# liulisixin/MLI-NeRF

Measured on AMD Instinct MI355X. Metric: rays/sec + PSNR, syn_hotdog 4096 rays x128 samples, 1/2/4/8 MI355X, higher is better.
Workload: dtype fp16; 1 GPU; syn_hotdog_b stage-b train step; rays_per_gpu=4096, samples_per_ray=128, global_rays=4096, parallelism=dp1, pipeline=geometry prefetch on a side stream, gate heads, 2 batch(es) ahead, output_layer_dw=forward partials (pq), tail=fused, reductions=ordered

## Files before the change

### include/mli_hip.h

```cpp
#ifndef MLI_HIP_H
#define MLI_HIP_H

#include <stdint.h>

#ifdef __cplusplus
extern "C" {
#endif

typedef struct ihipStream_t* mli_stream_t;

#define MLI_ABI_VERSION 18
#define MLI_HIDDEN 256
#define MLI_LEVELS 16
#define MLI_LEVEL_FEAT 8
#define MLI_HEAD_K0 304

typedef struct {
  float scale[MLI_LEVELS];
  uint32_t res[MLI_LEVELS];
  uint32_t size[MLI_LEVELS];
  uint32_t offset[MLI_LEVELS];
  uint64_t modmagic[MLI_LEVELS];
} mli_grid_levels;

int mli_abi_version(void);
const char* mli_error_string(int code);

typedef struct {
  const float* intr;
  const float* pose;
  const float* pose_light;
  const int64_t* ray_idx;
  int64_t first_pixel;
  int R, W;
  int bounding;
  float aabb[6];
  float* center;
  float* ray_unit;
  float* ray_norm;
  float* pts_light;
  float* near_;
  float* far_;
  uint8_t* outside;
} mli_rays_args;
int mli_rays(const mli_rays_args* a, mli_stream_t s);

typedef struct {
  const float* x01;
  const uint16_t* table;
  mli_grid_levels levels;
  int n;
  float* out;
} mli_hashgrid_args;
int mli_hashgrid_fwd(const mli_hashgrid_args* a, mli_stream_t s);

#define MLI_SDF_MODE_SDF 0
#define MLI_SDF_MODE_FIELD 1
#define MLI_SDF_MODE_SDF_LISTED 2
typedef struct {
  int mode;
  int R, n_per_ray;
  const float* center;
  const float* ray_unit;
  const float* dists;
  const uint8_t* outside;
  const uint16_t* table;
  mli_grid_levels levels;
  const void* wsdf;
  float eps;
  float grad_den;
  float hess_den;
  float outside_val;
  int with_hessian;
  float* sdf;
  float* grad;
  float* hess;
  uint16_t* h0;
  uint16_t* enc;
  int active_levels;
  const int32_t* inside_list;
  const int32_t* n_inside;
} mli_sdf_args;
int mli_sdf(const mli_sdf_args* a, mli_stream_t s);
int mli_sdf_workspace(const mli_sdf_args* a, int64_t* bytes);

struct mli_inside_list_args_s {
  int R, N;
  int n_pad;
  const uint8_t* outside;
  int32_t* inside_list;
  int32_t* n_inside;
  float outside_val;
  float* sdf;
  float* grad;
  float* hess;
  const float* near_;
  const float* far_;
  float* dists;
};
typedef struct mli_inside_list_args_s mli_inside_list_args;
int mli_inside_list(const mli_inside_list_args* a, mli_stream_t s);

typedef struct {
  const float* near_; const float* far_;
  const float* u;
  int R, Nc;
  float* dists;
} mli_sample_coarse_args;
int mli_sample_coarse(const mli_sample_coarse_args* a, mli_stream_t s);

typedef struct {
  int R;
  const float* dists_a; const float* sdf_a; int Na;
  const float* dists_b; const float* sdf_b; int Nb;
  float* dists_out; float* sdf_out;
  int Nf;
  float inv_s;
  const float* u_fine;
  float* fine_out;
  const int32_t* inside_list;
  const int32_t* n_inside;
} mli_sample_fine_args;
int mli_sample_fine(const mli_sample_fine_args* a, mli_stream_t s);

typedef struct {
  int R, N;
  const float* center; const float* ray_unit; const float* pts_light;
  const float* dists;
  const float* grad;
  const uint16_t* h0;
  const void* wfwd;
  float* y;
  uint16_t* feat_frag;
  uint16_t* xT;
  uint32_t* masks;
  int n_heads;
  const float* weights;
  float* q4;
  const int32_t* tile_list;
  const int32_t* n_live_tiles;
} mli_rgb_fwd_args;
#define MLI_Q4_SCALE 65536.0f
#define MLI_Q4_SEGS(N) ((256 % (N)) == 0 ? 256 / (N) : ((N) % 256 == 0 ? 1 : 256 / (N) + 2))
int mli_rgb_fwd(const mli_rgb_fwd_args* a, mli_stream_t s);
int mli_rgb_fwd_workspace(const mli_rgb_fwd_args* a, int64_t* bytes);

typedef struct {
  int R, N;
  const float* dists; const float* far_; const float* ray_unit; const float* ray_norm;
  const float* sdf; const float* grad; const float* y;
  const float* s_var;
  float anneal;
  int white_bg;
  float* weights;
  float* rgb; float* o_r; float* o_s; float* o_re;
  float* opacity; float* gradient; float* depth;
  float* blend_dist;
} mli_composite_args;
int mli_composite_fwd(const mli_composite_args* a, mli_stream_t s);

typedef struct {
  int R, N;
  const float* weights; const float* y;
  const float* o_r; const float* o_s;
  const float* d_rgb; const float* d_o_r; const float* d_o_s; const float* d_o_re;
  float grad_scale;
  float* dz4;
  float* dray;
} mli_composite_bwd_args;
int mli_composite_bwd(const mli_composite_bwd_args* a, mli_stream_t s);

typedef struct {
  int R, N;
  const float* dz4;
  const void* wbwd;
  const uint32_t* masks;
  uint16_t* dzT;
  uint16_t* dz4T;
  int skip_dz3;
  const int32_t* tile_list;
  const int32_t* n_live_tiles;
} mli_rgb_bwd_args;
int mli_rgb_bwd(const mli_rgb_bwd_args* a, mli_stream_t s);
int mli_rgb_bwd_workspace(const mli_rgb_bwd_args* a, int64_t* bytes);

typedef struct {
  const uint16_t* a_rows;
  const uint16_t* b_rows;
  int M, K;
  float* dw;
  float* db;
  int ldw;
  int a_tiled, b_tiled;
  int a_kst, b_kst;
  const uint16_t* b2_rows;
  int b2_q, b2_kst;
  const float* rb_dz4;
  const uint32_t* rb_mask;
  const void* rb_w4;
  int rb_col, rb_cnt;
  int rb_R, rb_N;
} mli_wgrad_job;
#define MLI_WGRAD_LAYOUT_ROWS 0
#define MLI_WGRAD_LAYOUT_TILED 1
#define MLI_WGRAD_LAYOUT_FRAG_ACC 2
#define MLI_WGRAD_LAYOUT_FRAG_NAT 3
#define MLI_WGRAD_BIG 1
#define MLI_WGRAD_WIDE 2
#define MLI_WGRAD_THIN 4
typedef struct {
  int S;
  int n_jobs;
  const mli_wgrad_job* jobs;
  int classes;
  int deterministic;
  float* workspace;
  const int32_t* tile_rank;
  const int32_t* tile_list;
  const int32_t* wtile_rank;
  const int32_t* wtile_list;
} mli_wgrad_args;
int mli_wgrad(const mli_wgrad_args* a, mli_stream_t s);
int mli_wgrad_workspace(const mli_wgrad_args* a, int64_t* bytes);

typedef struct {
  int R, N, n_heads;
  const float* q4;
  const float* dray;
  float scale;
  float* dw[3];
  float* db[3];
  int k_out[3];
  float* workspace;
  const int32_t* tile_rank;
} mli_dw4_args;
int mli_dw4(const mli_dw4_args* a, mli_stream_t s);
int mli_dw4_workspace(const mli_dw4_args* a, int64_t* bytes);

struct mli_live_rays_args_s {
  int R, N;
  const float* weights;
  float* y;
  int32_t* flags;
  int32_t* tile_list; int32_t* tile_rank; int32_t* n_live_tiles;
};
typedef struct mli_live_rays_args_s mli_live_rays_args;
int mli_live_rays(const mli_live_rays_args* a, mli_stream_t s);

struct mli_live_tiles_args_s {
  mli_composite_args comp;
  float* y;
  int32_t* flags;
  int32_t* tile_list; int32_t* tile_rank; int32_t* n_live_tiles;
  int32_t* wtile_list; int32_t* wtile_rank;
  int32_t* ticket;
  int scan_launch;
};
typedef struct mli_live_tiles_args_s mli_live_tiles_args;
int mli_live_tiles(const mli_live_tiles_args* a, mli_stream_t s);


typedef struct {
  int R, N;
  const float* dists; const float* far_; const float* ray_unit;
  const float* sdf; const float* grad; const float* y;
  const float* s_var;
  float anneal;
  int white_bg;
  const float* d_rgb;
  float grad_scale;
  float* dz4;
  float* d_sdf;
  float* d_grad;
  float* d_inv_s_part;
  float* d_s_var;
} mli_composite_bwd_geo_args;
int mli_composite_bwd_geo(const mli_composite_bwd_geo_args* a, mli_stream_t s);
int mli_composite_bwd_geo_workspace(const mli_composite_bwd_geo_args* a, int64_t* bytes);

typedef struct {
  int R, N;
  const float* dz4;
  const void* wgeo;
  const uint32_t* masks;
  const uint16_t* feat_frag;
  uint16_t* dzT;
  uint16_t* dz4T;
  float* d_nrm;
  uint16_t* dz1T;
  uint16_t* dh0_frag;
} mli_geo_bwd_args;
int mli_geo_bwd(const mli_geo_bwd_args* a, mli_stream_t s);
int mli_geo_bwd_workspace(const mli_geo_bwd_args* a, int64_t* bytes);

typedef struct {
  int R, N;
  const float* center; const float* ray_unit; const float* dists;
  const uint8_t* outside;
  const float* grad; const float* hess;
  const float* d_sdf; const float* d_grad;
  const float* d_nrm;
  const uint16_t* dh0_frag;
  const uint16_t* enc;
  const void* wsdf;
  const void* wsdf_t;
  float eps, grad_den, hess_den;
  float w_eikonal, w_curvature;
  float grad_scale;
  float* d_enc;
  uint16_t* dz0_frag;
  uint16_t* p_frag;
  float* dw_sdf;
  float* db_sdf;
  const float* d_grad_ext;
  const float* d_hess_ext;
  float* partials;
} mli_sdf_bwd_args;
int mli_sdf_bwd(const mli_sdf_bwd_args* a, mli_stream_t s);
int mli_sdf_bwd_workspace(const mli_sdf_bwd_args* a, int64_t* bytes);

typedef struct {
  const float* v0; const float* g0;
  uint8_t* dst;
} mli_pack_sdf_t_args;
#define MLI_SDF_T_PACK_BYTES 65536
int mli_pack_sdf_t(const mli_pack_sdf_t_args* a, mli_stream_t s);

typedef struct {
  int R, N;
  const float* center; const float* ray_unit; const float* dists;
  const float* d_enc;
  mli_grid_levels levels;
  float eps;
  int active_levels;
  float* d_table;
  int deterministic;
  int64_t* workspace;
  int64_t n_params;
} mli_hash_bwd_args;
int mli_hash_bwd(const mli_hash_bwd_args* a, mli_stream_t s);
int mli_hash_bwd_workspace(const mli_hash_bwd_args* a, int64_t* bytes);

typedef struct {
  const uint16_t* src;
  int64_t tile_stride;
  int tiles, k_steps, order;
  uint16_t* dst;
  int64_t ld;
  int64_t col0;
  int row0;
} mli_frag_rows_args;
int mli_frag_rows(const mli_frag_rows_args* a, mli_stream_t s);

typedef struct {
  int R;
  const float* center; const float* ray_unit; const float* pts_light;
  const float* near_; const float* far_;
  const float* blend_dist;
  const float* gradient;
  int camera_ray_type, iters;
  int vis_box;
  float vis_r2; float aabb[6];
  float gamma;
  const uint16_t* table; mli_grid_levels levels; int active_levels; const void* wsdf;
  float* light_unit; float* near_l; float* far_t; uint8_t* inside;
  float* inter_dist; uint8_t* inter_mask; float* inter_pts;
  uint8_t* visibility; float* normal_x_light; float* pseudo_shading;
} mli_light_visibility_args;
int mli_light_visibility(const mli_light_visibility_args* a, mli_stream_t s);
int mli_light_visibility_workspace(const mli_light_visibility_args* a, int64_t* bytes);

typedef struct {
  uint64_t seed;
  int64_t n_pixels;
  int R;
  const float* image;
  const float* ref;
  const float* sha;
  const float* cert;
  int64_t* ray_idx;
  float* image_sampled;
  float* ref_sampled;
  float* sha_sampled;
  float* cert_sampled;
} mli_ray_batch_args;
int mli_ray_batch(const mli_ray_batch_args* a, mli_stream_t s);

typedef struct {
  int R, N;
  const float* rgb; const float* o_r; const float* o_s; const float* o_re;
  const float* gt;
  const float* ref; const float* sha; const float* cert;
  const uint8_t* outside;
  const float* grad; const float* hess;
  float w_render, w_eikonal, w_curvature, w_intrinsic, w_re;
  float range_sha_lo, range_sha_hi, range_vis_lo, range_vis_hi, f_ref, f_sha;
  float f_neg, f_pos, e_pos;
  float* d_rgb; float* d_o_r; float* d_o_s; float* d_o_re;
  float* losses;
  float* scratch;
} mli_loss_args;
int mli_stage_b_loss(const mli_loss_args* a, mli_stream_t s);
int mli_stage_b_loss_workspace(const mli_loss_args* a, int64_t* bytes);

typedef struct {
  mli_composite_args comp;
  mli_loss_args loss;
  float grad_scale;
  float* dz4;
  int defer_finalize;
  float* dray;
} mli_composite_loss_args;
int mli_composite_loss(const mli_composite_loss_args* a, mli_stream_t s);
int mli_composite_loss_finalize(const mli_composite_loss_args* a, mli_stream_t s);
int mli_composite_loss_workspace(const mli_composite_loss_args* a, int64_t* bytes);

typedef struct {
  const float* v; const float* g; const float* bias;
  int n_out, k_ref;
  int transpose;
  int n_tiles, k_steps;
  const int16_t* kmap;
  const uint8_t* kmode;
  int64_t dst_offset;
  int chunk_stride;
  const int16_t* nmap;
} mli_pack_layer;
typedef struct {
  int n_layers;
  const mli_pack_layer* layers;
  uint8_t* dst;
  float* row_scale;
} mli_pack_args;
int mli_pack(const mli_pack_args* a, mli_stream_t s);
int mli_pack_workspace(const mli_pack_args* a, int64_t* bytes);

typedef struct {
  const float* v0; const float* g0; const float* b0;
  const float* w_sdf; const float* b_sdf;
  uint8_t* dst;
} mli_pack_sdf_args;
#define MLI_SDF_PACK_BYTES (65536 + 5 * 1024 + 16)
int mli_pack_sdf(const mli_pack_sdf_args* a, mli_stream_t s);

typedef struct {
  const float* dw; const float* db;
  const float* v; const float* g;
  int n_out, k_ref, k_pack;
  const int16_t* kinv;
  float* grad_v; float* grad_g; float* grad_b;
  const float* extra_db;
  int plain;
} mli_assemble_layer;
typedef struct {
  int n_layers;
  const mli_assemble_layer* layers;
  float inv_scale;
  int zero_dw;
} mli_assemble_args;
int mli_grad_assemble(const mli_assemble_args* a, mli_stream_t s);

typedef struct {
  float* p; float* g; float* m; float* v;
  int64_t n;
  double lr, beta1, beta2, eps, weight_decay;
  int step;
  uint16_t* p16;
  int zero_grad;
} mli_adamw_args;
int mli_adamw(const mli_adamw_args* a, mli_stream_t s);

typedef struct { const float* src; uint16_t* dst; int64_t n; } mli_cast_args;
int mli_cast_f16(const mli_cast_args* a, mli_stream_t s);

const char* mli_source_hash(void);

#ifdef __cplusplus
}
#endif
#endif
```

### mli_nerf_amd/_lib.py

```python
import ctypes as C
import os

HERE = os.path.dirname(os.path.abspath(__file__))
LIB_PATH = os.environ.get("MLI_HIP_LIB") or os.path.join(HERE, "libmli_hip.so")

P = C.c_void_p
I32 = C.c_int
I64 = C.c_int64
F32 = C.c_float
F64 = C.c_double


class GridLevels(C.Structure):
    _fields_ = [("scale", F32 * 16), ("res", C.c_uint32 * 16), ("size", C.c_uint32 * 16),
                ("offset", C.c_uint32 * 16), ("modmagic", C.c_uint64 * 16)]


class RaysArgs(C.Structure):
    _fields_ = [("intr", P), ("pose", P), ("pose_light", P), ("ray_idx", P), ("first_pixel", I64),
                ("R", I32), ("W", I32), ("bounding", I32), ("aabb", F32 * 6),
                ("center", P), ("ray_unit", P), ("ray_norm", P), ("pts_light", P),
                ("near_", P), ("far_", P), ("outside", P)]


class HashgridArgs(C.Structure):
    _fields_ = [("x01", P), ("table", P), ("levels", GridLevels), ("n", I32), ("out", P)]


class SdfArgs(C.Structure):
    _fields_ = [("mode", I32), ("R", I32), ("n_per_ray", I32), ("center", P), ("ray_unit", P),
                ("dists", P), ("outside", P), ("table", P), ("levels", GridLevels), ("wsdf", P),
                ("eps", F32), ("grad_den", F32), ("hess_den", F32), ("outside_val", F32),
                ("with_hessian", I32), ("sdf", P), ("grad", P), ("hess", P), ("h0", P),
                ("enc", P), ("active_levels", I32), ("inside_list", P), ("n_inside", P)]


class InsideListArgs(C.Structure):
    _fields_ = [("R", I32), ("N", I32), ("n_pad", I32), ("outside", P), ("inside_list", P), ("n_inside", P),
                ("outside_val", F32), ("sdf", P), ("grad", P), ("hess", P), ("near_", P), ("far_", P),
                ("dists", P)]


class SampleCoarseArgs(C.Structure):
    _fields_ = [("near_", P), ("far_", P), ("u", P), ("R", I32), ("Nc", I32), ("dists", P)]


class SampleFineArgs(C.Structure):
    _fields_ = [("R", I32), ("dists_a", P), ("sdf_a", P), ("Na", I32), ("dists_b", P), ("sdf_b", P),
                ("Nb", I32), ("dists_out", P), ("sdf_out", P), ("Nf", I32), ("inv_s", F32),
                ("u_fine", P), ("fine_out", P), ("inside_list", P), ("n_inside", P)]


class RgbFwdArgs(C.Structure):
    _fields_ = [("R", I32), ("N", I32), ("center", P), ("ray_unit", P), ("pts_light", P),
                ("dists", P), ("grad", P), ("h0", P), ("wfwd", P), ("y", P), ("feat_frag", P),
                ("xT", P), ("masks", P), ("n_heads", I32), ("weights", P), ("q4", P),
                ("tile_list", P), ("n_live_tiles", P)]


class CompositeArgs(C.Structure):
    _fields_ = [("R", I32), ("N", I32), ("dists", P), ("far_", P), ("ray_unit", P), ("ray_norm", P),
                ("sdf", P), ("grad", P), ("y", P), ("s_var", P), ("anneal", F32), ("white_bg", I32),
                ("weights", P), ("rgb", P), ("o_r", P), ("o_s", P), ("o_re", P), ("opacity", P),
                ("gradient", P), ("depth", P), ("blend_dist", P)]


class CompositeBwdArgs(C.Structure):
    _fields_ = [("R", I32), ("N", I32), ("weights", P), ("y", P), ("o_r", P), ("o_s", P),
                ("d_rgb", P), ("d_o_r", P), ("d_o_s", P), ("d_o_re", P), ("grad_scale", F32),
                ("dz4", P), ("dray", P)]


class RgbBwdArgs(C.Structure):
    _fields_ = [("R", I32), ("N", I32), ("dz4", P), ("wbwd", P), ("masks", P), ("dzT", P),
                ("dz4T", P), ("skip_dz3", I32), ("tile_list", P), ("n_live_tiles", P)]


class WgradJob(C.Structure):
    _fields_ = [("a_rows", P), ("b_rows", P), ("M", I32), ("K", I32), ("dw", P), ("db", P), ("ldw", I32),
                ("a_tiled", I32), ("b_tiled", I32), ("a_kst", I32), ("b_kst", I32), ("b2_rows", P),
                ("b2_q", I32), ("b2_kst", I32), ("rb_dz4", P), ("rb_mask", P), ("rb_w4", P), ("rb_col", I32),
                ("rb_cnt", I32), ("rb_R", I32), ("rb_N", I32)]


ROWS, TILED, FRAG_ACC, FRAG_NAT = 0, 1, 2, 3


def frag_job(a, b, M, K, dw, db, ldw, a_kst, b_kst, order=FRAG_ACC, b_order=None, b2=None, b2_q=0, b2_kst=0):
    return WgradJob(a, b, M, K, dw, db, ldw, order, order if b_order is None else b_order, a_kst, b_kst,
                    b2, b2_q, b2_kst)


class WgradArgs(C.Structure):
    _fields_ = [("S", I32), ("n_jobs", I32), ("jobs", P), ("classes", I32), ("deterministic", I32),
                ("workspace", P), ("tile_rank", P), ("tile_list", P), ("wtile_rank", P), ("wtile_list", P)]


class Dw4Args(C.Structure):
    _fields_ = [("R", I32), ("N", I32), ("n_heads", I32), ("q4", P), ("dray", P), ("scale", F32),
                ("dw", P * 3), ("db", P * 3), ("k_out", I32 * 3), ("workspace", P),
                ("tile_rank", P)]


class LiveRaysArgs(C.Structure):
    _fields_ = [("R", I32), ("N", I32), ("weights", P), ("y", P), ("flags", P), ("tile_list", P),
                ("tile_rank", P), ("n_live_tiles", P)]


class LiveTilesArgs(C.Structure):
    _fields_ = [("comp", CompositeArgs), ("y", P), ("flags", P), ("tile_list", P), ("tile_rank", P),
                ("n_live_tiles", P), ("wtile_list", P), ("wtile_rank", P), ("ticket", P), ("scan_launch", I32)]


Q4_SCALE = 65536.0


class LossArgs(C.Structure):
    _fields_ = [("R", I32), ("N", I32), ("rgb", P), ("o_r", P), ("o_s", P), ("o_re", P), ("gt", P),
                ("ref", P), ("sha", P), ("cert", P), ("outside", P), ("grad", P), ("hess", P),
                ("w_render", F32), ("w_eikonal", F32), ("w_curvature", F32), ("w_intrinsic", F32),
                ("w_re", F32), ("range_sha_lo", F32), ("range_sha_hi", F32), ("range_vis_lo", F32),
                ("range_vis_hi", F32), ("f_ref", F32), ("f_sha", F32), ("f_neg", F32), ("f_pos", F32),
                ("e_pos", F32), ("d_rgb", P), ("d_o_r", P), ("d_o_s", P), ("d_o_re", P), ("losses", P),
                ("scratch", P)]



class CompositeLossArgs(C.Structure):
    _fields_ = [("comp", CompositeArgs), ("loss", LossArgs), ("grad_scale", F32), ("dz4", P),
                ("defer_finalize", I32), ("dray", P)]

class PackLayer(C.Structure):
    _fields_ = [("v", P), ("g", P), ("bias", P), ("n_out", I32), ("k_ref", I32), ("transpose", I32),
                ("n_tiles", I32), ("k_steps", I32), ("kmap", P), ("kmode", P), ("dst_offset", I64),
                ("chunk_stride", I32), ("nmap", P)]


class PackArgs(C.Structure):
    _fields_ = [("n_layers", I32), ("layers", P), ("dst", P), ("row_scale", P)]


class PackSdfArgs(C.Structure):
    _fields_ = [("v0", P), ("g0", P), ("b0", P), ("w_sdf", P), ("b_sdf", P), ("dst", P)]


class AssembleLayer(C.Structure):
    _fields_ = [("dw", P), ("db", P), ("v", P), ("g", P), ("n_out", I32), ("k_ref", I32),
                ("k_pack", I32), ("kinv", P), ("grad_v", P), ("grad_g", P), ("grad_b", P),
                ("extra_db", P), ("plain", I32)]


class AssembleArgs(C.Structure):
    _fields_ = [("n_layers", I32), ("layers", P), ("inv_scale", F32), ("zero_dw", I32)]


class AdamwArgs(C.Structure):
    _fields_ = [("p", P), ("g", P), ("m", P), ("v", P), ("n", I64), ("lr", F64), ("beta1", F64),
                ("beta2", F64), ("eps", F64), ("weight_decay", F64), ("step", I32), ("p16", P),
                ("zero_grad", I32)]


class CastArgs(C.Structure):
    _fields_ = [("src", P), ("dst", P), ("n", I64)]


class CompositeBwdGeoArgs(C.Structure):
    _fields_ = [("R", I32), ("N", I32), ("dists", P), ("far_", P), ("ray_unit", P), ("sdf", P), ("grad", P),
                ("y", P), ("s_var", P), ("anneal", F32), ("white_bg", I32), ("d_rgb", P), ("grad_scale", F32),
                ("dz4", P), ("d_sdf", P), ("d_grad", P), ("d_inv_s_part", P), ("d_s_var", P)]


class GeoBwdArgs(C.Structure):
    _fields_ = [("R", I32), ("N", I32), ("dz4", P), ("wgeo", P), ("masks", P), ("feat_frag", P), ("dzT", P),
                ("dz4T", P), ("d_nrm", P), ("dz1T", P), ("dh0_frag", P)]


class SdfBwdArgs(C.Structure):
    _fields_ = [("R", I32), ("N", I32), ("center", P), ("ray_unit", P), ("dists", P), ("outside", P),
                ("grad", P), ("hess", P), ("d_sdf", P), ("d_grad", P), ("d_nrm", P), ("dh0_frag", P), ("enc", P),
                ("wsdf", P), ("wsdf_t", P), ("eps", F32), ("grad_den", F32), ("hess_den", F32),
                ("w_eikonal", F32), ("w_curvature", F32), ("grad_scale", F32), ("d_enc", P), ("dz0_frag", P),
                ("p_frag", P), ("dw_sdf", P), ("db_sdf", P), ("d_grad_ext", P), ("d_hess_ext", P),
                ("partials", P)]


class PackSdfTArgs(C.Structure):
    _fields_ = [("v0", P), ("g0", P), ("dst", P)]


class HashBwdArgs(C.Structure):
    _fields_ = [("R", I32), ("N", I32), ("center", P), ("ray_unit", P), ("dists", P), ("d_enc", P),
                ("levels", GridLevels), ("eps", F32), ("active_levels", I32), ("d_table", P),
                ("deterministic", I32), ("workspace", P), ("n_params", I64)]


class LightVisibilityArgs(C.Structure):
    _fields_ = [("R", I32), ("center", P), ("ray_unit", P), ("pts_light", P), ("near_", P), ("far_", P),
                ("blend_dist", P), ("gradient", P), ("camera_ray_type", I32), ("iters", I32), ("vis_box", I32),
                ("vis_r2", F32), ("aabb", F32 * 6), ("gamma", F32), ("table", P), ("levels", GridLevels),
                ("active_levels", I32), ("wsdf", P), ("light_unit", P), ("near_l", P), ("far_t", P),
                ("inside", P), ("inter_dist", P), ("inter_mask", P), ("inter_pts", P), ("visibility", P),
                ("normal_x_light", P), ("pseudo_shading", P)]


class RayBatchArgs(C.Structure):
    _fields_ = [("seed", C.c_uint64), ("n_pixels", I64), ("R", I32), ("image", P), ("ref", P), ("sha", P),
                ("cert", P), ("ray_idx", P), ("image_sampled", P), ("ref_sampled", P), ("sha_sampled", P),
                ("cert_sampled", P)]


class FragRowsArgs(C.Structure):
    _fields_ = [("src", P), ("tile_stride", I64), ("tiles", I32), ("k_steps", I32), ("order", I32), ("dst", P),
                ("ld", I64), ("col0", I64), ("row0", I32)]


ABI_VERSION = 18

ENTRY_POINTS = {
    "mli_rays": RaysArgs, "mli_hashgrid_fwd": HashgridArgs, "mli_sdf": SdfArgs,
    "mli_sample_coarse": SampleCoarseArgs, "mli_sample_fine": SampleFineArgs,
    "mli_rgb_fwd": RgbFwdArgs, "mli_composite_fwd": CompositeArgs,
    "mli_composite_bwd": CompositeBwdArgs, "mli_rgb_bwd": RgbBwdArgs,
    "mli_wgrad": WgradArgs, "mli_dw4": Dw4Args, "mli_live_rays": LiveRaysArgs,
    "mli_live_tiles": LiveTilesArgs, "mli_inside_list": InsideListArgs,
    "mli_pack": PackArgs, "mli_pack_sdf": PackSdfArgs, "mli_grad_assemble": AssembleArgs,
    "mli_adamw": AdamwArgs, "mli_cast_f16": CastArgs, "mli_stage_b_loss": LossArgs,
    "mli_composite_bwd_geo": CompositeBwdGeoArgs, "mli_geo_bwd": GeoBwdArgs, "mli_sdf_bwd": SdfBwdArgs,
    "mli_pack_sdf_t": PackSdfTArgs, "mli_hash_bwd": HashBwdArgs, "mli_frag_rows": FragRowsArgs,
    "mli_light_visibility": LightVisibilityArgs, "mli_ray_batch": RayBatchArgs,
    "mli_composite_loss": CompositeLossArgs, "mli_composite_loss_finalize": CompositeLossArgs,
}

WORKSPACE = {
    "mli_sdf": 1, "mli_rgb_fwd": 6, "mli_rgb_bwd": 2, "mli_wgrad": 1, "mli_composite_bwd_geo": 4,
    "mli_geo_bwd": 6, "mli_sdf_bwd": 4, "mli_hash_bwd": 1, "mli_light_visibility": 5, "mli_stage_b_loss": 5,
    "mli_pack": 1, "mli_dw4": 1, "mli_composite_loss": 2,
}


class McArgs(C.Structure):
    _fields_ = [("sdf", P), ("nx", I32), ("ny", I32), ("nz", I32), ("sx", I64), ("sy", I64), ("sz", I64),
                ("iso", F32), ("origin", F32 * 3), ("spacing", F32), ("off_x", I32), ("off_y", I32),
                ("off_z", I32), ("gx", I32), ("gy", I32), ("gz", I32), ("chunk_base", P), ("counts", P),
                ("edge_slot", P), ("max_vertices", I32), ("max_triangles", I32), ("verts", P),
                ("vert_keys", P), ("faces", P), ("face_keys", P)]


MESH_ABI_VERSION = 1
MC_CHUNK = 256

MESH_ENTRY_POINTS = {"mli_mc_count": McArgs, "mli_mc_emit": McArgs}
MESH_WORKSPACE = {"mli_mc_count": 2, "mli_mc_emit": 1}

class LabelMorphArgs(C.Structure):
    _fields_ = [("B", I32), ("H", I32), ("W", I32), ("erode_radius", I32), ("edge_step", I32),
                ("visibility", P), ("eroded", P), ("certainty", P), ("tile_max", P), ("normal_x_light", P),
                ("inter_mask", P), ("inv_gamma", F32), ("shading", P), ("shading_gamma", P)]


class LabelKmeansArgs(C.Structure):
    _fields_ = [("L", I32), ("K", I32), ("n_pixels", I32), ("max_iter", I32), ("image", P), ("labels", P),
                ("centers", P), ("passes", P)]


class LabelBestRefArgs(C.Structure):
    _fields_ = [("L", I32), ("K", I32), ("n_pixels", I32), ("threshold", F32), ("threshold_wrt_max", F32),
                ("image", P), ("shading", P), ("shading_gamma", P), ("labels", P), ("average_ref", P),
                ("keep_count", P), ("any_mask", P)]


class LabelFillArgs(C.Structure):
    _fields_ = [("H", I32), ("W", I32), ("K", I32), ("n_holes", I32), ("n_donors", I32), ("slices", I32),
                ("normal", P), ("centers", P), ("hole_idx", P), ("donor_idx", P), ("ref", P), ("hole_feat", P),
                ("donor_feat", P), ("partial", P)]


LABELS_ABI_VERSION = 1
LABELS_MAX_RADIUS = 15
LABELS_MAX_K = 4
LABELS_TILE = (32, 8)
LABELS_DONOR_TILE = 256
LABELS_MAX_SLICES = 64

LABELS_ENTRY_POINTS = {"mli_label_morph": LabelMorphArgs, "mli_label_kmeans": LabelKmeansArgs,
                       "mli_label_best_ref": LabelBestRefArgs, "mli_label_fill": LabelFillArgs}
LABELS_WORKSPACE = {"mli_label_morph": 1, "mli_label_fill": 3}

class MeshCcArgs(C.Structure):
    _fields_ = [("faces", P), ("n_faces", I64), ("verts", P), ("n_verts", C.c_int32), ("label", P), ("changed", P),
                ("max_rounds", C.c_int32), ("round", C.c_int32), ("comp_faces", P), ("comp_area", P), ("max_q", P),
                ("inv_unit", F64)]


MESH_CC_ABI_VERSION = 1
MESH_CC_MAX_ROUNDS = 4096

MESH_CC_ENTRY_POINTS = {"mli_cc_init": MeshCcArgs, "mli_cc_round": MeshCcArgs, "mli_cc_stats": MeshCcArgs}
MESH_CC_WORKSPACE = {"mli_cc_init": 4}

class MetricsArgs(C.Structure):
    _fields_ = [("B", I32), ("C", I32), ("H", I32), ("W", I32), ("quantize", I32), ("mask_pred", I32),
                ("gamma_target", I32), ("inv_gamma", F64), ("pred_f32", P), ("pred_u8", P), ("target_f32", P),
                ("target_u8", P), ("alpha_f32", P), ("alpha_u8", P), ("mse", P), ("psnr", P), ("ssim", P),
                ("ssim_channels", P), ("prep_pred", P), ("prep_target", P), ("partial", P)]


METRICS_ABI_VERSION = 1
METRICS_MAX_SIDE = 16384
METRICS_MAX_IMAGES = 16383
METRICS_MAX_CHANNELS = 4
METRICS_WINDOW = 7
METRICS_TILE = (32, 8)

METRICS_ENTRY_POINTS = {"mli_image_metrics": MetricsArgs}
METRICS_WORKSPACE = {"mli_image_metrics": 1}

class LightPointsArgs(C.Structure):
    _fields_ = [("L", I32), ("R", I32), ("pose_lights", P), ("pts_light", P)]


class CameraHitArgs(C.Structure):
    _fields_ = [("R", I32), ("center", P), ("ray_unit", P), ("near_", P), ("far_", P), ("blend_dist", P),
                ("camera_ray_type", I32), ("iters", I32), ("table", P), ("levels", GridLevels),
                ("active_levels", I32), ("wsdf", P), ("inter_dist", P), ("inter_mask", P), ("inter_pts", P)]


class LightShadowsArgs(C.Structure):
    _fields_ = [("L", I32), ("R", I32), ("pts_light", P), ("inter_pts", P), ("gradient", P), ("vis_box", I32),
                ("vis_r2", F32), ("aabb", F32 * 6), ("gamma", F32), ("iters", I32), ("table", P),
                ("levels", GridLevels), ("active_levels", I32), ("wsdf", P), ("visibility", P),
                ("normal_x_light", P), ("pseudo_shading", P)]


RELIGHT_ABI_VERSION = 1

RELIGHT_ENTRY_POINTS = {"mli_light_points": LightPointsArgs, "mli_camera_hit": CameraHitArgs,
                        "mli_light_shadows": LightShadowsArgs}
RELIGHT_WORKSPACE = {}

_lib = None


def lib():
    global _lib
    if _lib is None:
        if not os.path.exists(LIB_PATH):
            raise ImportError("libmli_hip.so is not built (%s); run mli_nerf_amd.build.build() -- "
                              "there is no CPU fallback for the hot path" % LIB_PATH)
        _lib = C.CDLL(LIB_PATH)
        for name, st in list(ENTRY_POINTS.items()) + list(MESH_ENTRY_POINTS.items()) + list(
                LABELS_ENTRY_POINTS.items()) + list(MESH_CC_ENTRY_POINTS.items()) + list(
                METRICS_ENTRY_POINTS.items()) + list(RELIGHT_ENTRY_POINTS.items()):
            fn = getattr(_lib, name)
            fn.argtypes = [C.POINTER(st), P]
            fn.restype = I32
        for table, points in ((WORKSPACE, ENTRY_POINTS), (MESH_WORKSPACE, MESH_ENTRY_POINTS),
                              (LABELS_WORKSPACE, LABELS_ENTRY_POINTS), (MESH_CC_WORKSPACE, MESH_CC_ENTRY_POINTS),
                              (METRICS_WORKSPACE, METRICS_ENTRY_POINTS)):
            for name in table:
                fn = getattr(_lib, name + "_workspace")
                fn.argtypes = [C.POINTER(points[name]), C.POINTER(I64)]
                fn.restype = I32
        _lib.mli_mesh_abi_version.restype = I32
        _lib.mli_labels_abi_version.restype = I32
        _lib.mli_mesh_cc_abi_version.restype = I32
        _lib.mli_metrics_abi_version.restype = I32
        _lib.mli_relight_abi_version.restype = I32
        _lib.mli_abi_version.restype = I32
        _lib.mli_error_string.restype = C.c_char_p
        _lib.mli_error_string.argtypes = [I32]
        _lib.mli_source_hash.restype = C.c_char_p
        if (_lib.mli_abi_version() != ABI_VERSION or _lib.mli_mesh_abi_version() != MESH_ABI_VERSION
                or _lib.mli_labels_abi_version() != LABELS_ABI_VERSION
                or _lib.mli_mesh_cc_abi_version() != MESH_CC_ABI_VERSION
                or _lib.mli_metrics_abi_version() != METRICS_ABI_VERSION
                or _lib.mli_relight_abi_version() != RELIGHT_ABI_VERSION):
            raise ImportError("libmli_hip.so ABI mismatch")
        from . import build as _build
        if all(os.path.exists(d) for d in _build._deps()):
            want, got = _build.source_hash(), _lib.mli_source_hash().decode()
            in_tree = os.path.realpath(LIB_PATH) == os.path.realpath(_build.OUT)
            if got != want and in_tree:
                raise ImportError("libmli_hip.so is stale (built from sources %s, the tree is %s); rebuild with "
                                  "mli_nerf_amd.build.build()" % (got, want))
            if got != want:
                import warnings
                warnings.warn("MLI_HIP_LIB=%s was built from sources %s, not this tree's %s (experiment build)"
                              % (LIB_PATH, got, want))
    return _lib


def _variant(name, args):
    if name == "mli_sdf":
        return ":field" if args.mode == 1 else ":sdf"
    if name == "mli_wgrad":
        return {1: ":big", 2: ":wide", 4: ":thin"}.get(args.classes, "")
    return ""


def workspace(name, args):
    out = (I64 * 8)()
    rc = getattr(lib(), name + "_workspace")(C.byref(args), out)
    if rc != 0:
        raise RuntimeError("%s_workspace failed: %s (%d)" % (name, lib().mli_error_string(rc).decode(), rc))
    return [int(out[i]) for i in range(WORKSPACE.get(name) or MESH_WORKSPACE.get(name) or LABELS_WORKSPACE.get(name)
                                         or MESH_CC_WORKSPACE.get(name) or METRICS_WORKSPACE[name])]


def ptr(t):
    return None if t is None else t.data_ptr()


PROFILE = None
PROFILE_NAMES = None
# ... 17 lines not shown
```

### mli_nerf_amd/csrc/mlp_bwd.hip

```cpp
#include "mlp_core.h"

namespace {

template <bool NODZ3>
__global__ __launch_bounds__(GBwd::THREADS) void rgb_bwd_kernel(mli_rgb_bwd_args a) {
  extern __shared__ __attribute__((aligned(16))) uint8_t lds[];
  if (a.n_live_tiles && (int)(blockIdx.x * GBwd::NW) >= *a.n_live_tiles) return;
  if (__builtin_amdgcn_readfirstlane(threadIdx.x >> 6) >= GBwd::NW / 2) rgb_bwd_body<GBwd, STORE, NODZ3>(a, lds);
  else rgb_bwd_body<GBwd, DMA, NODZ3>(a, lds);
}


}

extern "C" int mli_rgb_bwd(const mli_rgb_bwd_args* a, mli_stream_t s) {
  const int S = a->R * a->N;
  if (S % 256 != 0) return (int)hipErrorInvalidValue;
  if ((a->tile_list != nullptr) != (a->n_live_tiles != nullptr)) return (int)hipErrorInvalidValue;
  if (a->tile_list && (a->N <= 0 || 256 % a->N != 0 || a->N % 32 != 0)) return (int)hipErrorInvalidValue;
  if (a->skip_dz3)
    hipLaunchKernelGGL(rgb_bwd_kernel<true>, dim3(S / GBwd::SAMPLES), dim3(GBwd::THREADS), GBwd::LDS_BWD,
                       (hipStream_t)s, *a);
  else
    hipLaunchKernelGGL(rgb_bwd_kernel<false>, dim3(S / GBwd::SAMPLES), dim3(GBwd::THREADS), GBwd::LDS_BWD,
                       (hipStream_t)s, *a);
  MLI_LAUNCH_CHECK();
}

extern "C" int mli_rgb_bwd_workspace(const mli_rgb_bwd_args* a, int64_t* bytes) {
  const int64_t S = (int64_t)a->R * a->N;
  if (S <= 0 || S % 256 != 0) return (int)hipErrorInvalidValue;
  bytes[0] = 3 * 4 * 256 * S * 2;
  bytes[1] = 3 * S * 16 * 2;
  return 0;
}
```

### mli_nerf_amd/csrc/mlp_core.h

```cpp
#pragma once
#include "common.h"

#include <type_traits>

namespace {

constexpr int CH(int ks) { return ks * 1024 + 128; }
constexpr int FRAG_KS = 512;
constexpr int FRAG_TILE = 16 * FRAG_KS;
constexpr int X0_KS = MLI_HEAD_K0 / 16;
constexpr int X0_TILE = X0_KS * FRAG_KS;
constexpr int Q4_SLOT = 257 * 16;
constexpr int DIST = 2;
#ifndef MLI_HEADS_PAIR
#define MLI_HEADS_PAIR 1
#endif
constexpr bool HEADS_PAIR = MLI_HEADS_PAIR;
constexpr int NSLOT = HEADS_PAIR ? 4 : DIST + 1;

enum Role { ALL = 0, DMA = 1, STORE = 2 };

template <int NW_, int MAXP, bool SPLIT_, int PF_ = 0>
struct Geo {
  static constexpr int NW = NW_;
// ... 12 lines not shown
  static constexpr int QP_OFF = RING;
  static constexpr int PQ_WAVE = 2048 + 256;
  static constexpr int PQW_OFF = QP_OFF + (HEADS_PAIR ? 0 : NW * Q4_SLOT);
  static constexpr int LDS_FWD_PQ = PQW_OFF + NW * PQ_WAVE;
  static constexpr int FEAT_KS = 6;
  static_assert(FEAT_KS % 2 == 0, "whole 32-feature tiles of feat in LDS");
  static constexpr int LDS_FWD_PQF = LDS_FWD_PQ + NW * FEAT_KS * 1024;
  static constexpr int FEAT_KS_EVAL = 8;
  static_assert(FEAT_KS_EVAL % 2 == 0, "whole 32-feature tiles of feat in LDS");
  static constexpr int LDS_FWD_F = LDS_FWD + NW * FEAT_KS_EVAL * 1024;
  template <int ROLE> static constexpr int ring_ops() { return ROLE == STORE ? 0 : RND; }
};

struct Ring {
  const uint8_t* src;
  const uint8_t* last;
  int next, n, cur;
};

template <class G, int ROLE>
MLI_FI void ring_pieces(const uint8_t* s, int nb, uint8_t* slot) {
  const int wave = threadIdx.x >> 6, lane = threadIdx.x & 63;
  if (ROLE != STORE) {
#pragma unroll
    for (int u = 0; u < G::RND; ++u)
      glds16(s + min((u * G::ND + wave) * 1024 + lane * 16, nb - 16), slot + (u * G::ND + wave) * 1024);
  }
}

template <class G, int ROLE, class Bytes>
MLI_FI void ring_issue(Ring& r, uint8_t* lds, Bytes&& bytes) {
  const bool real = r.next < r.n;
  const int nb = bytes(real ? r.next : r.n - 1);
  ring_pieces<G, ROLE>(real ? r.src : r.last, nb, lds + (r.next % NSLOT) * G::SLOT);
  if (real) r.src += nb;
  r.next++;
}

struct ChunkAt {
  const uint8_t* image;
  int head_bytes;
  int first;
  MLI_FI const uint8_t* src(int c) const { return image + (size_t)(c >> 3) * head_bytes + first + (c & 7) * CH(16); }
  MLI_FI int operator()(int) const { return CH(16); }
};

template <class G, int ROLE>
MLI_FI void ring_issue(Ring& r, uint8_t* lds, ChunkAt& at) {
  ring_pieces<G, ROLE>(at.src(min(r.next, r.n - 1)), CH(16), lds + (r.next % NSLOT) * G::SLOT);
  r.next++;
}

template <class Bytes>
MLI_FI void ring_start(Ring& r, const void* base, int n, Bytes&& bytes) {
  r.src = reinterpret_cast<const uint8_t*>(base);
  size_t total = 0;
  for (int c = 0; c + 1 < n; ++c) total += bytes(c);
  r.last = r.src + total;
  r.next = 0;
  r.n = n;
  r.cur = 0;
}

MLI_FI void frag_store2(uint16_t* tile_img, int t, half8 f0, half8 f1, int lane) {
  half8* d = reinterpret_cast<half8*>(tile_img) + (2 * t) * 64 + lane;
  gstore_nt(d, f0);
  gstore_nt(d + 64, f1);
}

MLI_FI float relu1(float x) {
  return __builtin_bit_cast(float, max(__builtin_bit_cast(int, x), 0));
}
MLI_FI int f32_bits(float x) { return __builtin_bit_cast(int, x); }
MLI_FI uint32_t relu_bits16(const f32x16& r) {
  uint32_t b = 0;
#pragma unroll
  for (int i = 15; i >= 0; --i)
    asm("v_cmp_lt_i32 vcc, 0, %1\n\tv_addc_co_u32 %0, vcc, %0, %0, vcc" : "+v"(b) : "v"(f32_bits(r[i])) : "vcc");
  return b;
}
template <int KS, int PF = 0>
MLI_FI f32x16 chunk_mma(const uint8_t* chunk, const half8* X, int lane) {
  const int h = lane >> 5;
  f32x16 acc;
  const f32x4* bias = reinterpret_cast<const f32x4*>(chunk + KS * 1024 + h * 64);
#pragma unroll
  for (int u = 0; u < 4; ++u) {
    const f32x4 b = bias[u];
    acc[4 * u] = b[0]; acc[4 * u + 1] = b[1]; acc[4 * u + 2] = b[2]; acc[4 * u + 3] = b[3];
  }
  const half8* w = reinterpret_cast<const half8*>(chunk) + lane;
  if constexpr (PF == 0) {
#pragma unroll
    for (int q = 0; q < KS; ++q) acc = mfma32(w[q * 64], X[q], acc);
  } else {
    constexpr int D = PF < KS ? PF : KS;
    half8 wr[D];
#pragma unroll
    for (int q = 0; q < D; ++q) wr[q] = w[q * 64];
#pragma unroll
    for (int q = 0; q < KS; ++q) {
      acc = mfma32(wr[q % D], X[q], acc);
      if (q + D < KS) wr[q % D] = w[(q + D) * 64];
    }
#pragma unroll
    for (int q = 0; q < D; ++q) __builtin_amdgcn_sched_group_barrier(0x100, 1, 0);
#pragma unroll
    for (int q = 0; q < KS; ++q) {
      __builtin_amdgcn_sched_group_barrier(0x008, 1, 0);
      if (q + D < KS) __builtin_amdgcn_sched_group_barrier(0x100, 1, 0);
    }
  }
  return acc;
}

template <class G, int ROLE, int KS, int NT, int EPI, bool MASKED, class Bytes, class Pre, class Epi>
MLI_FI void run_layer(Ring& rg, uint8_t* lds, const half8* X, int lane, Bytes&& bytes, Pre&& pre, Epi&& epi) {
  auto stores = [](int t) MLI_LAMBDA_FI { return EPI + ((MASKED && t == NT - 1) ? 1 : 0); };
#pragma unroll
  for (int t = 0; t < NT; ++t) {
    pre.issue(t);
    ring_issue<G, ROLE>(rg, lds, bytes);
    const f32x16 acc = chunk_mma<KS, G::PF>(lds + (rg.cur % NSLOT) * G::SLOT, X, lane);
    epi(t, acc);
    if (ROLE != STORE) {
      int n = (DIST - 1) * G::template ring_ops<ROLE>() + pre.count(t) + stores(t);
#pragma unroll
      for (int b = 1; b < DIST; ++b) {
        if (t - b < 0) break;
        n += stores(t - b) + (b < DIST - 1 ? pre.count(t - b) : 0);
      }
      vm_wait(n);
    }
    block_sync();
    rg.cur++;
  }
}

struct NoPre {
  MLI_FI int count(int) const { return 0; }
  MLI_FI void issue(int) const {}
};

template <class G, int ROLE, int KS, int NT, int EPI, int MASKN, int PREVN, bool DEFER, int LASTN = 0, class Bytes,
          class Pre, class Prev, class Epi>
MLI_FI void run_layer_d(Ring& rg, uint8_t* lds, const half8* X, int lane, Bytes&& bytes, Pre&& pre, Prev&& prev,
                        Epi&& epi, f32x16& pacc) {
  static_assert(ROLE != ALL, "split wave roles only");
  auto stores = [](int t) MLI_LAMBDA_FI {
    if (t < 0) return LASTN;
    const int pv = t == 0 ? PREVN : 0;
    if (DEFER) return pv + (t >= 1 ? EPI : 0);
    return pv + EPI + (t == NT - 1 ? MASKN : 0);
  };
#pragma unroll
  for (int t = 0; t < NT; ++t) {
    pre.issue(t);
    ring_issue<G, ROLE>(rg, lds, bytes);
    if (t == 0) prev(pacc);
    const f32x16 acc = chunk_mma<KS, G::PF>(lds + (rg.cur % NSLOT) * G::SLOT, X, lane);
    if (DEFER) {
      if (t > 0) epi(t - 1, pacc);
      pacc = acc;
    } else {
      epi(t, acc);
    }
    if (ROLE != STORE) vm_wait((DIST - 1) * G::template ring_ops<ROLE>() + pre.count(t) + stores(t) + stores(t - 1));
    block_sync();
    rg.cur++;
  }
}

template <class G, int ROLE, int KS, int NT, int EPI, int MASKN, int PREVN, bool DEFER, int NEXTN, class Bytes,
          class Pre, class Prev, class Epi>
MLI_FI void run_layer_p(Ring& rg, uint8_t* lds, const half8* X, int lane, Bytes&& bytes, Pre&& pre, Prev&& prev,
                        Epi&& epi, f32x16& pacc) {
  static_assert(ROLE != ALL, "split wave roles only");
  static_assert(NSLOT == 4, "two segments of two chunks in the ring");
  auto stores = [](int t) MLI_LAMBDA_FI {
    const int pv = t == 0 ? PREVN : 0;
    if (DEFER) return pv + (t >= 1 ? EPI : 0);
    return pv + EPI + (t == NT - 1 ? MASKN : 0);
  };
#pragma unroll
  for (int s = 0; s < NT; s += 2) {
    const int n_this = NT - s < 2 ? NT - s : 2;
    const int n_next = s + 2 < NT ? (NT - s - 2 < 2 ? NT - s - 2 : 2) : NEXTN;
#pragma unroll
    for (int t = s; t < s + n_this; ++t) pre.issue(t);
#pragma unroll
    for (int k = 0; k < n_next; ++k) ring_issue<G, ROLE>(rg, lds, bytes);
    int n = 0;
#pragma unroll
    for (int t = s; t < s + n_this; ++t) {
      if (t == 0) prev(pacc);
      const f32x16 acc = chunk_mma<KS, G::PF>(lds + (rg.cur % NSLOT) * G::SLOT, X, lane);
      if (DEFER) {
        if (t > 0) epi(t - 1, pacc);
        pacc = acc;
      } else {
        epi(t, acc);
      }
      n += stores(t);
      rg.cur++;
    }
    if (ROLE != STORE) vm_wait(n);
    block_sync();
  }
}

template <class G, int ROLE, int KS, int NT, int EPI, int MASKN, int PREVN, bool DEFER, int LASTN, int NEXTN,
          class Bytes, class Pre, class Prev, class Epi>
MLI_FI void heads_layer(Ring& rg, uint8_t* lds, const half8* X, int lane, Bytes&& bytes, Pre&& pre, Prev&& prev,
                        Epi&& epi, f32x16& pacc) {
  if constexpr (HEADS_PAIR)
    run_layer_p<G, ROLE, KS, NT, EPI, MASKN, PREVN, DEFER, NEXTN>(rg, lds, X, lane, bytes, pre, prev, epi, pacc);
  else
    run_layer_d<G, ROLE, KS, NT, EPI, MASKN, PREVN, DEFER, LASTN>(rg, lds, X, lane, bytes, pre, prev, epi, pacc);
}

constexpr int PROLOGUE_CHUNKS = HEADS_PAIR ? 2 : DIST;

constexpr bool HEADS_DEFER = true;

constexpr float Q4_SCALE = MLI_Q4_SCALE;

template <class G, int ROLE>
MLI_FI void q4_tile(const mli_rgb_fwd_args& a, uint8_t* lds, const half8 (&X)[19], const float (&gq)[3], int hd,
                   int lane, const Ring& rg) {
  const int wave = threadIdx.x >> 6, c = lane & 31, h = lane >> 5;
  uint8_t* xr = lds + G::PQW_OFF + wave * G::PQ_WAVE;
  uint8_t* gr = xr + 2048;
  auto q4_park = [&](int w) MLI_LAMBDA_FI {
    if constexpr (HEADS_PAIR) {
      static_assert(4 * Q4_SLOT <= G::SLOT && G::NW == 8, "Q park in two ring slots");
      const int slot = (rg.cur - (w < 4 ? 2 : 1)) % NSLOT;
      return lds + slot * G::SLOT + (w & 3) * Q4_SLOT;
    } else {
      return lds + G::QP_OFF + w * Q4_SLOT;
    }
  };
  uint8_t* qs = q4_park(wave);
  if (h == 0) {
#pragma unroll
    for (int i = 0; i < 4; ++i)
      ds_write_u16(lds_addr(gr + i * 64 + c * 2), __builtin_bit_cast(uint16_t, (f16)(i < 3 ? gq[i] : 0.f)));
  }
  asm volatile("" ::: "memory");
  half8 gf[2];
  {
    const int gi = min(c, 3);
#pragma unroll
    for (int ks = 0; ks < 2; ++ks) gf[ks] = *reinterpret_cast<const half8*>(gr + gi * 64 + (16 * ks + 8 * h) * 2);
  }
  const int g16 = (lane >> 4) & 3, q = (lane & 15) >> 2, p = lane & 3;
  const int chunk = 4 * (g16 & 1) + p;
#pragma unroll
  for (int b = 0; b < 8; ++b) {
#pragma unroll
    for (int u = 0; u < 2; ++u) {
      const u32x4 w = __builtin_bit_cast(u32x4, X[2 * b + u]);
#pragma unroll
      for (int jj = 0; jj < 2; ++jj) {
        const int ch = (4 * u + 2 * jj + h) ^ ((c >> 1) & 7);
        ds_write_u64(lds_addr(xr + c * 64 + ch * 8), u32x2{w[2 * jj], w[2 * jj + 1]});
      }
    }
    f32x16 acc;
#pragma unroll
    for (int e = 0; e < 16; ++e) acc[e] = 0.f;
    half8 xf[2];
#pragma unroll
    for (int ks = 0; ks < 2; ++ks) {
      const int s0 = 16 * ks + 8 * h + q, s1 = s0 + 4;
      const half4 lo = ds_tr16_at<0>(lds_addr(xr + s0 * 64 + (chunk ^ ((s0 >> 1) & 7)) * 8));
      const half4 hi = ds_tr16_at<0>(lds_addr(xr + s1 * 64 + (chunk ^ ((s1 >> 1) & 7)) * 8));
      xf[ks] = half8{lo[0], lo[1], lo[2], lo[3], hi[0], hi[1], hi[2], hi[3]};
    }
    lgkm_wait<0>();
    tie(xf[0]);
    tie(xf[1]);
#pragma unroll
    for (int ks = 0; ks < 2; ++ks) acc = mfma32(gf[ks], xf[ks], acc);
    if (h == 0) ds_write_f128(lds_addr(qs + (32 * b + c) * 16), f32x4{acc[0], acc[1], acc[2], acc[3]});
  }
  float sb[3];
#pragma unroll
  for (int i = 0; i < 3; ++i) {
    float v = gq[i];
#pragma unroll
    for (int o = 32; o > 0; o >>= 1) v += __shfl_xor(v, o);
    sb[i] = v;
  }
  if (lane == 0) ds_write_f128(lds_addr(qs + 256 * 16), f32x4{sb[0], sb[1], sb[2], 0.f});
  block_sync();
  if (ROLE != DMA) {
    const int N = a.N, t0 = blockIdx.x * G::NW;
    const int r_first = t0 * 32 / N;
    const int nseg = ((t0 + G::NW) * 32 - 1) / N - r_first + 1;
    const int segs = MLI_Q4_SEGS(N);
    const int nthr = ROLE == STORE ? G::THREADS / 2 : G::THREADS;
    const int tid = ROLE == STORE ? threadIdx.x - G::THREADS / 2 : threadIdx.x;
    f32x4* qb = reinterpret_cast<f32x4*>(a.q4);
    for (int it = tid; it < nseg * 257; it += nthr) {
      const int seg = it / 257, row = it - seg * 257;
      size_t item = (size_t)blockIdx.x * segs + seg;
      if (a.tile_list) item = (size_t)(a.tile_list[t0 + seg * (N / 32)] * 32 / N);
      f32x4* qo = qb + item * a.n_heads * 257;
      f32x4 v = {0.f, 0.f, 0.f, 0.f};
#pragma unroll
      for (int w = 0; w < G::NW; ++w)
        if ((t0 + w) * 32 / N - r_first == seg) v += *reinterpret_cast<const f32x4*>(q4_park(w) + row * 16);
      gstore_nt(qo + (size_t)hd * 257 + row, v);
    }
  }
  block_sync();
}

MLI_FI int fwd_bytes(int c) { return (c >= 8 && (c - 8) % 33 < 8) ? CH(19) : CH(16); }

template <class G, bool TRAIN, bool PQ, int ROLE>
MLI_FI void rgb_fwd_body(const mli_rgb_fwd_args& a, uint8_t* lds) {
  const int lane = threadIdx.x & 63, wave = threadIdx.x >> 6;
  const int c = lane & 31, h = lane >> 5;
  const int S = a.R * a.N;
  const int tile = blockIdx.x * G::NW + wave;
  const int tile_o = (PQ && a.tile_list) ? __builtin_amdgcn_readfirstlane(a.tile_list[tile]) : tile;
  const int m = tile_o * 32 + c;
  const int r = m / a.N, k = m - r * a.N;
  const size_t slot = (size_t)k * a.R + r;
  auto bytes = [](int cc) MLI_LAMBDA_FI { return fwd_bytes(cc); };
  constexpr int XL = PQ ? 3 : 4;
  constexpr int FKS = PQ ? G::FEAT_KS : (!TRAIN ? G::FEAT_KS_EVAL : 0);
  constexpr int FOFF = PQ ? G::LDS_FWD_PQ : G::LDS_FWD;
  const float wgt = PQ ? a.weights[slot] : 0.f;

  Ring rg;
  ring_start(rg, a.wfwd, 8 + a.n_heads * 33, bytes);

  half8 A[16], B[19];
  {
    const half8* src = reinterpret_cast<const half8*>(a.h0 + (size_t)tile_o * FRAG_TILE) + lane;
#pragma unroll
    for (int q = 0; q < 16; ++q) B[q] = gload16(src + q * 64);
  }
  half8 xe[3];
  {
    const float d = a.dists[slot];
    const float* cr = a.center + 3 * r;
    const float* vr = a.ray_unit + 3 * r;
    float p[3], nrm[3], g[3];
#pragma unroll
    for (int i = 0; i < 3; ++i) {
      p[i] = __fadd_rn(cr[i], __fmul_rn(vr[i], d));
      g[i] = a.grad[3 * slot + i];
    }
    const float gn = fmaxf(sqrtf((g[0] * g[0] + g[1] * g[1]) + g[2] * g[2]), 1e-12f);
#pragma unroll
    for (int i = 0; i < 3; ++i) nrm[i] = g[i] / gn;
    float shl[16], shv[16];
    sh16(a.pts_light[3 * r], a.pts_light[3 * r + 1], a.pts_light[3 * r + 2], shl);
    sh16(vr[0], vr[1], vr[2], shv);
    const float e16[8] = {p[0], p[1], p[2], nrm[0], nrm[1], nrm[2], 0.f, 0.f};
    const uint32_t hm = opaque_v(h) ? ~0u : 0u;
#pragma unroll
    for (int j = 0; j < 8; ++j) {
      const float v16 = sel_mask(hm, 0.f, e16[j]);
      const float v17 = sel_mask(hm, shl[8 + j], shl[j]);
      const float v18 = sel_mask(hm, shv[8 + j], shv[j]);
      B[16][j] = (f16)v16;
      B[17][j] = (f16)v17;
      B[18][j] = (f16)v18;
      if (TRAIN) {
        const int lo = j < 4 ? j : 4 + j, hi = j < 4 ? 4 + j : 8 + j;
        xe[0][j] = (f16)sel_mask(hm, hi < 8 ? e16[hi & 7] : 0.f, lo < 8 ? e16[lo & 7] : 0.f);
        xe[1][j] = (f16)sel_mask(hm, shl[hi], shl[lo]);
        xe[2][j] = (f16)sel_mask(hm, shv[hi], shv[lo]);
      }
    }
  }
  uint16_t* ftile = a.feat_frag + (size_t)tile * X0_TILE;
#pragma unroll
  for (int d = 0; d < PROLOGUE_CHUNKS; ++d) ring_issue<G, ROLE>(rg, lds, bytes);
  if (TRAIN) {
    half8* xd = reinterpret_cast<half8*>(ftile + 16 * FRAG_KS) + lane;
#pragma unroll
    for (int i = 0; i < 3; ++i) gstore_nt(xd + i * 64, xe[i]);
  }
  vm_wait((HEADS_PAIR || ROLE == STORE ? 0 : (DIST - 1) * G::template ring_ops<ROLE>()) + (TRAIN ? 3 : 0));
#pragma unroll
  for (int q = 0; q < 16; ++q) tie(B[q]);
  block_sync();

  f32x16 pacc;
  auto none = [](f32x16&) MLI_LAMBDA_FI {};
  auto feat_epi = [&](int t, const f32x16& acc) MLI_LAMBDA_FI {
    f32x16 v;
#pragma unroll
    for (int i = 0; i < 16; i += 2) {
      const f32x2 sp = softplus100x2((f32x2){acc[i], acc[i + 1]});
      v[i] = sp.x;
      v[i + 1] = sp.y;
    }
    A[2 * t] = acc_to_frag(v, 0);
    A[2 * t + 1] = acc_to_frag(v, 1);
    half8* dst = reinterpret_cast<half8*>(ftile) + (2 * t) * 64 + lane;
    gstore(dst, A[2 * t]);
    gstore(dst + 64, A[2 * t + 1]);
    if (2 * t + 1 < FKS) {
      half8* fl = reinterpret_cast<half8*>(lds + FOFF + wave * FKS * 1024) + (2 * t) * 64 + lane;
      fl[0] = A[2 * t];
      fl[64] = A[2 * t + 1];
    }
  };
  heads_layer<G, ROLE, 16, 8, 2, 0, 0, HEADS_DEFER, TRAIN ? 3 : 0, 2>(rg, lds, B, lane, bytes, NoPre{}, none, feat_epi,
                                                                      pacc);
  if (HEADS_DEFER) feat_epi(7, pacc);

  for (int hd = 0; hd < a.n_heads; ++hd) {
    const int S = opaque_s(a.R * a.N);
    if (hd == 0) {
#pragma unroll
      for (int q = 0; q < 16; ++q) B[q] = A[q];
    } else {
      const half8* src = reinterpret_cast<const half8*>(ftile) + opaque_v(lane);
      const half8* fl = reinterpret_cast<const half8*>(lds + FOFF + wave * (FKS > 0 ? FKS : 1) * 1024) + lane;
#pragma unroll
      for (int q = 0; q < 16; ++q) B[q] = q < FKS ? fl[q * 64] : gload16(src + q * 64);
    }
    auto l0_wait = [&](f32x16&) MLI_LAMBDA_FI {
      if (hd > 0) {
        vm_wait((HEADS_PAIR ? 2 : 1) * G::template ring_ops<ROLE>());
#pragma unroll
        for (int q = FKS; q < 16; ++q) tie(B[q]);
      }
    };
    uint32_t mbits[4];
    auto relu_epi = [&](half8* out, int layer, bool stg) MLI_LAMBDA_FI {
      return [&, out, layer, stg](int t, const f32x16& acc) MLI_LAMBDA_FI {
        f32x16 v;
#pragma unroll
        for (int i = 0; i < 16; ++i) v[i] = relu1(acc[i]);
        out[2 * t] = acc_to_frag(v, 0);
        out[2 * t + 1] = acc_to_frag(v, 1);
        if (TRAIN) {
          const uint32_t bits = relu_bits16(v);
          if (t & 1) mbits[t >> 1] |= bits << 16; else mbits[t >> 1] = bits;
          if (stg) frag_store2(a.xT + ((size_t)(hd * XL + layer) * (S / 32) + tile) * FRAG_TILE, t, out[2 * t],
                               out[2 * t + 1], lane);
          if (t == 7) {
            u32x4* mp = reinterpret_cast<u32x4*>(a.masks) +
                        ((size_t)(hd * 4 + layer) * (S / 32) + tile) * 64 + lane;
            gstore_nt(mp, u32x4{mbits[0], mbits[1], mbits[2], mbits[3]});
          }
        }
      };
    };
    auto e0 = relu_epi(A, 0, true);
    auto e1 = relu_epi(B, 1, true);
    auto e2 = relu_epi(A, 2, true);
    auto e3 = relu_epi(B, 3, !PQ);
    auto fin = [&](auto& e) MLI_LAMBDA_FI {
      return [&](f32x16& p) MLI_LAMBDA_FI {
        if (HEADS_DEFER) e(7, p);
      };
    };
    constexpr int MN = TRAIN ? 1 : 0, PN = TRAIN && HEADS_DEFER ? 1 : 0;
    constexpr int X = TRAIN ? 2 : 0, X3 = PQ ? 0 : X;
    constexpr int LN = HEADS_DEFER ? X : X + MN;
    heads_layer<G, ROLE, 19, 8, X, MN, 0, HEADS_DEFER, 0, 2>(rg, lds, B, lane, bytes, NoPre{}, l0_wait, e0, pacc);
    heads_layer<G, ROLE, 16, 8, X, MN, PN + X, HEADS_DEFER, LN, 2>(rg, lds, A, lane, bytes, NoPre{}, fin(e0), e1, pacc);
    heads_layer<G, ROLE, 16, 8, X, MN, PN + X, HEADS_DEFER, LN, 2>(rg, lds, B, lane, bytes, NoPre{}, fin(e1), e2, pacc);
    heads_layer<G, ROLE, 16, 8, X3, MN, PN + X, HEADS_DEFER, LN, 1>(rg, lds, A, lane, bytes, NoPre{}, fin(e2), e3,
                                                                    pacc);
    const int no = hd == 2 ? 1 : 3;
    const int off = hd * 3;
    float gq[3] = {0.f, 0.f, 0.f};
    heads_layer<G, ROLE, 16, 1, 0, 0, PN + X3, false, HEADS_DEFER ? X3 : X3 + MN, 2>(rg, lds, B, lane, bytes, NoPre{},
                                                                                fin(e3),
                                          [&](int, const f32x16& acc) MLI_LAMBDA_FI {
      if (h == 0) {
#pragma unroll
        for (int i = 0; i < 3; ++i)
          if (i < no) {
            const float y = sigmoidf_acc(acc[i]);
            gstore_f32(a.y + 8 * slot + off + i, y);
            if (PQ) gq[i] = Q4_SCALE * wgt * (y * (1.0f - y));
          }
      }
    }, pacc);
    if (PQ) q4_tile<G, ROLE>(a, lds, B, gq, hd, lane, rg);
  }
  vm_wait(0);
}

#ifndef MLI_HEADS_PF
#define MLI_HEADS_PF 4
#endif
constexpr int HEADS_PF = MLI_HEADS_PF;
typedef Geo<8, 20, true, HEADS_PF> GFwd;
typedef Geo<8, 20, true, HEADS_PF> GFwdT;
typedef Geo<8, 17, true, HEADS_PF> GBwd;

template <bool TRAIN, bool PQ>
__global__ __launch_bounds__(GFwd::THREADS) void rgb_fwd_kernel(mli_rgb_fwd_args a) {
  extern __shared__ __attribute__((aligned(16))) uint8_t lds[];
  typedef typename std::conditional<TRAIN, GFwdT, GFwd>::type G;
  if (PQ && a.n_live_tiles && (int)(blockIdx.x * G::NW) >= *a.n_live_tiles) return;
  if (__builtin_amdgcn_readfirstlane(threadIdx.x >> 6) >= G::NW / 2) rgb_fwd_body<G, TRAIN, PQ, STORE>(a, lds);
  else rgb_fwd_body<G, TRAIN, PQ, DMA>(a, lds);
}

MLI_FI int bwd_bytes(int c) { return (c % 32) < 8 ? CH(1) : CH(16); }
constexpr int BWD_CHUNKS = 3 * 32;

template <class G, int ROLE, bool NODZ3 = false>
MLI_FI void rgb_bwd_body(const mli_rgb_bwd_args& a, uint8_t* lds) {
  const int lane = threadIdx.x & 63, wave = threadIdx.x >> 6;
  const int c = lane & 31, h = lane >> 5;
  const int S = a.R * a.N;
  const int tiles = S / 32;
  const int tile = blockIdx.x * G::NW + wave;
  const int tile_o = a.tile_list ? __builtin_amdgcn_readfirstlane(a.tile_list[tile]) : tile;
  const int m = tile_o * 32 + c;
  const int r = m / a.N, k = m - r * a.N;
  const size_t slot = (size_t)k * a.R + r;
  auto bytes = [](int cc) MLI_LAMBDA_FI { return bwd_bytes(cc); };
  constexpr int MASK_OPS = ROLE == DMA ? 2 : ROLE == ALL ? 1 : 0;
  auto mask_dma = [&](int L) MLI_LAMBDA_FI {
    const int Lc = min(L, 11);
    const int hd = Lc >> 2, ml = 3 - (Lc & 3);
    const uint8_t* src = reinterpret_cast<const uint8_t*>(a.masks) +
                         (((size_t)(hd * 4 + ml) * tiles + (size_t)blockIdx.x * G::NW) * 64) * 16;
#pragma unroll
    for (int u = 0; u < MASK_OPS; ++u)
      glds16(src + u * (G::MASKB / 2) + threadIdx.x * 16,
             lds + G::MASK_OFF + (L & 1) * G::MASKB + u * (G::MASKB / 2) + wave * 1024);
  };

  f32x4 dzv0, dzv1;
  {
    const f32x4* p = reinterpret_cast<const f32x4*>(a.dz4 + 8 * slot);
    dzv0 = p[0];
    dzv1 = p[1];
  }
  Ring rg;
  ring_start(rg, a.wbwd, BWD_CHUNKS, bytes);
  mask_dma(0);
#pragma unroll
  for (int d = 0; d < PROLOGUE_CHUNKS; ++d) ring_issue<G, ROLE>(rg, lds, bytes);
  if (ROLE != STORE) vm_wait(HEADS_PAIR ? 0 : (DIST - 1) * G::template ring_ops<ROLE>());
  block_sync();

  half8 A[16], B[16];
  for (int hd = 0; hd < 3; ++hd) {
    const int S = opaque_s(a.R * a.N);
    const int no = hd == 2 ? 1 : 3;
    half8 z4;
    {
      const float d0 = hd == 0 ? dzv0[0] : hd == 1 ? dzv0[3] : dzv1[2];
      const float d1 = hd == 0 ? dzv0[1] : dzv1[0];
      const float d2 = hd == 0 ? dzv0[2] : dzv1[1];
#pragma unroll
      for (int j = 0; j < 8; ++j) z4[j] = (f16)0.f;
      if (h == 0) {
        z4[0] = (f16)d0;
        if (no > 1) {
          z4[1] = (f16)d1;
          z4[2] = (f16)d2;
        }
      }
      if (a.dz4T)
        gstore_nt(reinterpret_cast<half8*>(a.dz4T + ((size_t)hd * (S / 32) + tile) * FRAG_KS) + lane, z4);
    }
    struct MaskPre {
      decltype(mask_dma)& dma;
      int next_layer;
      MLI_FI int count(int t) const { return t == 8 - DIST ? MASK_OPS : 0; }
      MLI_FI void issue(int t) const {
        if (t == 8 - DIST) dma(next_layer);
      }
    };
    auto pre = [&](int li) MLI_LAMBDA_FI { return MaskPre{mask_dma, hd * 4 + li + 1}; };
    auto mask_epi = [&](half8* out, int layer , int li, auto stc ) MLI_LAMBDA_FI {
      return [&, out, layer, li, stc](int t, const f32x16& acc) MLI_LAMBDA_FI {
        const u32x4 mv =
            *reinterpret_cast<const u32x4*>(lds + G::MASK_OFF + (li & 1) * G::MASKB + wave * 1024 + lane * 16);
        const int wi = t >> 1;
        const uint32_t word = wi == 0 ? mv[0] : wi == 1 ? mv[1] : wi == 2 ? mv[2] : mv[3];
        f32x16 v;
#pragma unroll
        for (int i = 0; i < 16; ++i) v[i] = mask_bit(acc[i], word, (t & 1) * 16 + i);
        out[2 * t] = acc_to_frag(v, 0);
        out[2 * t + 1] = acc_to_frag(v, 1);
        if (decltype(stc)::value)
          frag_store2(a.dzT + ((size_t)(hd * 4 + layer) * (S / 32) + tile) * FRAG_TILE, t, out[2 * t],
                      out[2 * t + 1], lane);
      };
    };
    const std::true_type store{};
    auto e3 = mask_epi(A, 3, 0, std::integral_constant<bool, !NODZ3>{});
    auto e2 = mask_epi(B, 2, 1, store);
    auto e1 = mask_epi(A, 1, 2, store);
    auto e0 = mask_epi(B, 0, 3, store);
    auto none = [](f32x16&) MLI_LAMBDA_FI {};
    auto fin = [&](auto& e) MLI_LAMBDA_FI {
      return [&](f32x16& p) MLI_LAMBDA_FI {
        if (HEADS_DEFER) e(7, p);
      };
    };
    f32x16 pacc;
    constexpr int X = 2, LN = X, X3 = NODZ3 ? 0 : X;
    heads_layer<G, ROLE, 1, 8, X3, 0, 0, HEADS_DEFER, 0, 2>(rg, lds, &z4, lane, bytes, pre(0), none, e3, pacc);
    heads_layer<G, ROLE, 16, 8, X, 0, X3, HEADS_DEFER, X3, 2>(rg, lds, A, lane, bytes, pre(1), fin(e3), e2, pacc);
    heads_layer<G, ROLE, 16, 8, X, 0, X, HEADS_DEFER, LN, 2>(rg, lds, B, lane, bytes, pre(2), fin(e2), e1, pacc);
    heads_layer<G, ROLE, 16, 8, X, 0, X, HEADS_DEFER, LN, 2>(rg, lds, A, lane, bytes, pre(3), fin(e1), e0, pacc);
    if (HEADS_DEFER) e0(7, pacc);
  }
  vm_wait(0);
}

}

__attribute__((visibility("hidden"))) int mli_launch_rgb_fwd_pq(const mli_rgb_fwd_args* a, hipStream_t s);
__attribute__((visibility("hidden"))) int mli_launch_rgb_fwd_train(const mli_rgb_fwd_args* a, hipStream_t s);
```

### mli_nerf_amd/csrc/mlp_fwd.hip

```cpp
#include "mlp_core.h"

extern "C" int mli_rgb_fwd(const mli_rgb_fwd_args* a, mli_stream_t s) {
  const int S = a->R * a->N;
  if (S % 256 != 0) return (int)hipErrorInvalidValue;
  const bool train = a->xT != nullptr;
  if (a->feat_frag == nullptr || (train && a->masks == nullptr)) return (int)hipErrorInvalidValue;
  if (a->n_heads != 1 && a->n_heads != 3) return (int)hipErrorInvalidValue;
  const bool pq = a->weights != nullptr;
  if (pq && (!train || a->q4 == nullptr || a->N % 32 != 0)) return (int)hipErrorInvalidValue;
  if (!pq && a->q4 != nullptr) return (int)hipErrorInvalidValue;
  if ((a->tile_list != nullptr) != (a->n_live_tiles != nullptr)) return (int)hipErrorInvalidValue;
  if (a->tile_list && (!pq || 256 % a->N != 0)) return (int)hipErrorInvalidValue;
  const dim3 grid(S / GFwd::SAMPLES), block(GFwd::THREADS);
  if (pq) return mli_launch_rgb_fwd_pq(a, (hipStream_t)s);
  if (train) return mli_launch_rgb_fwd_train(a, (hipStream_t)s);
  static_assert(GFwd::LDS_FWD_F <= 163840, "LDS per workgroup");
  hipLaunchKernelGGL((rgb_fwd_kernel<false, false>), grid, block, GFwd::LDS_FWD_F, (hipStream_t)s, *a);
  MLI_LAUNCH_CHECK();
}

extern "C" int mli_rgb_fwd_workspace(const mli_rgb_fwd_args* a, int64_t* bytes) {
  const int64_t S = (int64_t)a->R * a->N;
  if (S <= 0 || S % 256 != 0 || (a->n_heads != 1 && a->n_heads != 3)) return (int)hipErrorInvalidValue;
  const bool pq = a->weights != nullptr;
  if (pq && a->N % 32 != 0) return (int)hipErrorInvalidValue;
  bytes[0] = S * 8 * 4;
  bytes[1] = (int64_t)MLI_HEAD_K0 * S * 2;
  bytes[2] = 0;
  bytes[3] = (int64_t)a->n_heads * (pq ? 3 : 4) * 256 * S * 2;
  bytes[4] = (int64_t)a->n_heads * 4 * (S / 32) * 64 * 16;
  bytes[5] = pq ? (S / 256) * MLI_Q4_SEGS(a->N) * a->n_heads * 257 * 4 * 4 : 0;
  return 0;
}
```

### mli_nerf_amd/csrc/rays.hip

```cpp
#include "common.h"
#include "loss.h"
#include "mli_relight.h"

namespace {

MLI_FI float light_pos(const float* Q, int i) {
  return -((Q[4 * 0 + i] * Q[3] + Q[4 * 1 + i] * Q[7]) + Q[4 * 2 + i] * Q[11]);
}

__global__ __launch_bounds__(256) void rays_kernel(mli_rays_args a) {
  const int r = blockIdx.x * blockDim.x + threadIdx.x;
  if (r >= a.R) return;
  const int64_t pix = a.ray_idx ? a.ray_idx[r] : a.first_pixel + r;
  const float py = (float)(pix / a.W) + 0.5f;
  const float px = (float)(pix % a.W) + 0.5f;
  float K[9], T[12], TL[3];
  {
    const float* M = a.intr;
    const float c00 = M[4] * M[8] - M[5] * M[7], c01 = M[5] * M[6] - M[3] * M[8], c02 = M[3] * M[7] - M[4] * M[6];
    const float det = (M[0] * c00 + M[1] * c01) + M[2] * c02;
    const float id = 1.0f / det;
    K[0] = c00 * id; K[1] = (M[2] * M[7] - M[1] * M[8]) * id; K[2] = (M[1] * M[5] - M[2] * M[4]) * id;
    K[3] = c01 * id; K[4] = (M[0] * M[8] - M[2] * M[6]) * id; K[5] = (M[2] * M[3] - M[0] * M[5]) * id;
    K[6] = c02 * id; K[7] = (M[1] * M[6] - M[0] * M[7]) * id; K[8] = (M[0] * M[4] - M[1] * M[3]) * id;
// ... 610 lines not shown
  return (L << lb) | Rr;
}

__global__ __launch_bounds__(256) void ray_batch_kernel(mli_ray_batch_args a) {
  const int r = blockIdx.x * blockDim.x + threadIdx.x;
  if (r >= a.R) return;
  int bits = 1;
  while ((1ll << bits) < a.n_pixels) ++bits;
  uint64_t x = (uint64_t)r;
  do {
    x = feistel(x, bits, a.seed);
  } while (x >= (uint64_t)a.n_pixels);
  const int64_t p = (int64_t)x, n = a.n_pixels;
  a.ray_idx[r] = p;
  if (a.image)
    for (int c = 0; c < 3; ++c) a.image_sampled[3 * r + c] = a.image[c * n + p];
  if (a.ref)
    for (int c = 0; c < 3; ++c) a.ref_sampled[3 * r + c] = a.ref[c * n + p];
  if (a.sha) a.sha_sampled[r] = a.sha[p];
  if (a.cert) a.cert_sampled[r] = a.cert[p];
}

}

extern "C" int mli_rays(const mli_rays_args* a, mli_stream_t s) {
  if (a->R <= 0) return 0;
  hipLaunchKernelGGL(rays_kernel, dim3((a->R + 255) / 256), dim3(256), 0, (hipStream_t)s, *a);
  MLI_LAUNCH_CHECK();
}

extern "C" int mli_light_points(const mli_light_points_args* a, mli_stream_t s) {
  if (a->L <= 0 || a->R <= 0) return 0;
  if (!a->pose_lights || !a->pts_light) return (int)hipErrorInvalidValue;
  if ((int64_t)a->L * a->R > INT32_MAX) return (int)hipErrorInvalidValue;
  const int64_t n = (int64_t)a->L * a->R * 3;
  hipLaunchKernelGGL(light_points_kernel, dim3((unsigned)((n + 255) / 256)), dim3(256), 0, (hipStream_t)s, *a);
  MLI_LAUNCH_CHECK();
}

extern "C" int mli_sample_coarse(const mli_sample_coarse_args* a, mli_stream_t s) {
  const int n = a->R * a->Nc;
  if (n <= 0) return 0;
  hipLaunchKernelGGL(sample_coarse_kernel, dim3((n + 255) / 256), dim3(256), 0, (hipStream_t)s, *a);
  MLI_LAUNCH_CHECK();
}

extern "C" int mli_sample_fine(const mli_sample_fine_args* a, mli_stream_t s) {
  if (a->R <= 0) return 0;
  if (a->Nf > FBMAX || a->Nb > FBMAX || a->Na < 1 || a->Na + a->Nb > FMAX) return (int)hipErrorInvalidValue;
  if (a->Nf > 0 && a->sdf_out == nullptr) return (int)hipErrorInvalidValue;
  if ((a->inside_list == nullptr) != (a->n_inside == nullptr)) return (int)hipErrorInvalidValue;
  FineArgs fa;
  fa.a = *a;
  for (int j = 0; j < 64; ++j) fa.u[j] = (j < a->Nf && a->u_fine) ? a->u_fine[j] : 2.0f;
  hipLaunchKernelGGL(sample_fine_kernel, dim3((a->R + FW - 1) / FW), dim3(FW * 64), 0, (hipStream_t)s, fa);
  MLI_LAUNCH_CHECK();
}

extern "C" int mli_composite_fwd(const mli_composite_args* a, mli_stream_t s) {
  if (a->R <= 0) return 0;
  if (a->N > 256) return (int)hipErrorInvalidValue;
  if (a->N <= 32 * CE)
    hipLaunchKernelGGL(composite_fwd_kernel<32>, dim3((a->R + 2 * CW - 1) / (2 * CW)), dim3(CW * 64), 0,
                       (hipStream_t)s, *a);
  else
    hipLaunchKernelGGL(composite_fwd_kernel<64>, dim3((a->R + CW - 1) / CW), dim3(CW * 64), 0, (hipStream_t)s, *a);
  MLI_LAUNCH_CHECK();
}

extern "C" int mli_composite_bwd(const mli_composite_bwd_args* a, mli_stream_t s) {
  if (a->R <= 0) return 0;
  const size_t S = (size_t)a->R * a->N;
  hipLaunchKernelGGL(composite_bwd_kernel, dim3((unsigned)((S + 255) / 256)), dim3(256), 0, (hipStream_t)s, *a);
  MLI_LAUNCH_CHECK();
}

extern "C" int mli_composite_bwd_geo(const mli_composite_bwd_geo_args* a, mli_stream_t s) {
  if (a->R <= 0) return 0;
  if (a->N > 256) return (int)hipErrorInvalidValue;
  if (a->d_inv_s_part == nullptr) return (int)hipErrorInvalidValue;
  hipLaunchKernelGGL(composite_bwd_geo_kernel, dim3((a->R + CW - 1) / CW), dim3(CW * 64), 0, (hipStream_t)s, *a);
  hipLaunchKernelGGL(svar_grad_kernel, dim3(1), dim3(256), 0, (hipStream_t)s, *a);
  MLI_LAUNCH_CHECK();
}

extern "C" int mli_composite_bwd_geo_workspace(const mli_composite_bwd_geo_args* a, int64_t* bytes) {
  if (a->R <= 0 || a->N <= 0) return (int)hipErrorInvalidValue;
  const int64_t S = (int64_t)a->R * a->N;
  bytes[0] = S * 8 * 4;
  bytes[1] = S * 4;
  bytes[2] = S * 3 * 4;
  bytes[3] = (int64_t)a->R * 4;
  return 0;
}

extern "C" int mli_ray_batch(const mli_ray_batch_args* a, mli_stream_t s) {
  if (a->R <= 0) return 0;
  if (a->n_pixels < a->R || a->n_pixels > (1ll << 40) || !a->ray_idx) return (int)hipErrorInvalidValue;
  hipLaunchKernelGGL(ray_batch_kernel, dim3((a->R + 255) / 256), dim3(256), 0, (hipStream_t)s, *a);
  MLI_LAUNCH_CHECK();
}

struct CLGeo {
  int rpb, nb;
};
static CLGeo cl_geo(int R, int N) {
  const int rpb = N <= 32 * CE ? 2 * CW : CW;
  return CLGeo{rpb, (R + rpb - 1) / rpb};
}
static bool cl_valid(const mli_composite_loss_args* a) {
  const mli_composite_args& c = a->comp;
  const mli_loss_args& l = a->loss;
  if (c.R <= 0 || c.N <= 0 || c.N > 256 || l.R != c.R || l.N != c.N) return false;
  if (!c.weights || !c.rgb || !c.o_r || !c.o_s || !c.o_re || !a->dz4 || !l.scratch || !l.losses || !l.gt ||
      !l.outside || !c.y)
    return false;
  return !(l.w_intrinsic != 0.f && (l.sha == nullptr || l.cert == nullptr || l.ref == nullptr));
}

extern "C" int mli_composite_loss(const mli_composite_loss_args* a, mli_stream_t s) {
  if (!cl_valid(a)) return (int)hipErrorInvalidValue;
  const CLGeo g = cl_geo(a->comp.R, a->comp.N);
  if (g.rpb == 2 * CW)
    hipLaunchKernelGGL(composite_loss_kernel<32>, dim3(g.nb), dim3(CW * 64), 0, (hipStream_t)s, *a);
  else
    hipLaunchKernelGGL(composite_loss_kernel<64>, dim3(g.nb), dim3(CW * 64), 0, (hipStream_t)s, *a);
  if (!a->defer_finalize)
    hipLaunchKernelGGL(composite_loss_finalize, dim3(1), dim3(256), 0, (hipStream_t)s, a->loss, g.nb);
  MLI_LAUNCH_CHECK();
}

extern "C" int mli_composite_loss_finalize(const mli_composite_loss_args* a, mli_stream_t s) {
  if (!cl_valid(a)) return (int)hipErrorInvalidValue;
  hipLaunchKernelGGL(composite_loss_finalize, dim3(1), dim3(256), 0, (hipStream_t)s, a->loss,
                     cl_geo(a->comp.R, a->comp.N).nb);
  MLI_LAUNCH_CHECK();
}

extern "C" int mli_composite_loss_workspace(const mli_composite_loss_args* a, int64_t* bytes) {
  const int R = a->comp.R;
  if (R <= 0 || a->comp.N <= 0) return (int)hipErrorInvalidValue;
  bytes[0] = (int64_t)mli_loss::ACC_N * cl_geo(R, a->comp.N).nb * 4;
  bytes[1] = (int64_t)R * a->comp.N * 8 * 4;
  return 0;
}

namespace {

constexpr int LR_RAYS = 64, LR_SCAN = 1024;

__global__ __launch_bounds__(4 * LR_RAYS) void live_flags_kernel(mli_live_rays_args a) {
  __shared__ int any[4][LR_RAYS];
  const int rl = threadIdx.x % LR_RAYS, j = threadIdx.x / LR_RAYS;
  const int r = blockIdx.x * LR_RAYS + rl;
  int live = 0;
  if (r < a.R)
    for (int k = j; k < a.N; k += 4)
      live |= (__builtin_bit_cast(uint32_t, a.weights[(size_t)k * a.R + r]) & 0x7fffffffu) != 0;
  any[j][rl] = live;
  __syncthreads();
  live = any[0][rl] | any[1][rl] | any[2][rl] | any[3][rl];
  if (r >= a.R) return;
  if (j == 0) a.flags[r] = live;
  if (!live && a.y != nullptr) {
    const f32x4 z = {0.f, 0.f, 0.f, 0.f};
    for (int k = j; k < a.N; k += 4) {
      f32x4* row = reinterpret_cast<f32x4*>(a.y + ((size_t)k * a.R + r) * 8);
      row[0] = z;
      row[1] = z;
    }
  }
}

template <bool TILES, class Flag, class Emit>
MLI_FI void compact_scan(int n, Flag flag, Emit emit, int& kept, int& bits) {
  __shared__ int sums[1 + TILES][LR_SCAN];
  const int t = threadIdx.x;
  const int per = (n + LR_SCAN - 1) / LR_SCAN;
  const int r0 = min(t * per, n), r1 = min(r0 + per, n);
  int cnt = 0, wcnt = 0;
  for (int r = r0; r < r1; ++r) {
    const uint32_t f = flag(r);
    cnt += f != 0;
    if (TILES) wcnt += __popc(f);
  }
  sums[0][t] = cnt;
  if (TILES) sums[TILES][t] = wcnt;
  __syncthreads();
  for (int o = 1; o < LR_SCAN; o <<= 1) {
    const int v = t >= o ? sums[0][t - o] : 0, wv = TILES && t >= o ? sums[TILES][t - o] : 0;
    __syncthreads();
    sums[0][t] += v;
    if (TILES) sums[TILES][t] += wv;
    __syncthreads();
  }
  kept = sums[0][LR_SCAN - 1];
  bits = TILES ? sums[TILES][LR_SCAN - 1] : 0;
  int before = sums[0][t] - cnt;
  int wbefore = TILES ? sums[TILES][t] - wcnt : 0;
  for (int r = r0; r < r1; ++r) {
    const uint32_t f = flag(r);
    emit(r, f, f != 0 ? before : kept + (r - before), before, wbefore);
    before += f != 0;
    if (TILES) wbefore += __popc(f);
  }
}

__global__ __launch_bounds__(LR_SCAN) void live_scan_kernel(mli_live_rays_args a) {
  const int T = a.N / 32, G = 256 / a.N;
  int L, none;
  compact_scan<false>(
      a.R, [&](int r) MLI_LAMBDA_FI { return (uint32_t)a.flags[r]; },
      [&](int r, uint32_t live, int pos, int before, int) MLI_LAMBDA_FI {
        for (int i = 0; i < T; ++i) {
          a.tile_list[pos * T + i] = r * T + i;
          a.tile_rank[r * T + i] = before * T + (live ? i : 0);
        }
      },
      L, none);
  if (threadIdx.x == 0) {
    a.tile_rank[a.R * T] = L * T;
    a.n_live_tiles[0] = (L + G - 1) / G * G * T;
  }
}

}

extern "C" int mli_live_rays(const mli_live_rays_args* a, mli_stream_t s) {
  if (a->R <= 0 || a->N <= 0 || a->N % 32 != 0 || 256 % a->N != 0 || a->R % (256 / a->N) != 0)
    return (int)hipErrorInvalidValue;
  if (!a->weights || !a->flags || !a->tile_list || !a->tile_rank || !a->n_live_tiles) return (int)hipErrorInvalidValue;
  hipLaunchKernelGGL(live_flags_kernel, dim3((a->R + LR_RAYS - 1) / LR_RAYS), dim3(4 * LR_RAYS), 0, (hipStream_t)s, *a);
  hipLaunchKernelGGL(live_scan_kernel, dim3(1), dim3(LR_SCAN), 0, (hipStream_t)s, *a);
  MLI_LAUNCH_CHECK();
}

namespace {

__global__ __launch_bounds__(LR_SCAN) void inside_list_kernel(mli_inside_list_args a, int fill_blocks) {
  const int t = threadIdx.x;
  if ((int)blockIdx.x < fill_blocks) {
    const size_t i = (size_t)blockIdx.x * LR_SCAN + t;
    if (i >= (size_t)a.R * a.N) return;
    const int r = (int)(i % a.R);
    if (!a.outside[r]) return;
    if (a.dists != nullptr) {
      const float near = a.near_[r], far = a.far_[r];
      const float d = near + (((float)(i / a.R) + 0.5f) / (float)a.N) * (far - near);
      a.dists[i] = fminf(fmaxf(d, near), far);
    }
    if (a.sdf == nullptr) return;
    a.sdf[i] = a.outside_val;
    a.grad[3 * i] = 0.0f;
    a.grad[3 * i + 1] = 0.0f;
    a.grad[3 * i + 2] = 0.0f;
    if (a.hess != nullptr) {
      a.hess[3 * i] = 0.0f;
      a.hess[3 * i + 1] = 0.0f;
      a.hess[3 * i + 2] = 0.0f;
    }
    return;
  }
  int n_in, none;
  compact_scan<false>(
      a.R, [&](int r) MLI_LAMBDA_FI { return (uint32_t)(a.outside[r] == 0); },
      [&](int r, uint32_t, int pos, int, int) MLI_LAMBDA_FI { a.inside_list[pos] = r; }, n_in, none);
  if (t == 0) a.n_inside[0] = min(n_in + a.n_pad, a.R);
}

}

extern "C" int mli_inside_list(const mli_inside_list_args* a, mli_stream_t s) {
  if (a->R <= 0 || a->N <= 0 || a->n_pad < 0 || !a->outside || !a->inside_list || !a->n_inside)
    return (int)hipErrorInvalidValue;
  if ((a->sdf == nullptr) != (a->grad == nullptr) || (a->hess != nullptr && a->sdf == nullptr))
    return (int)hipErrorInvalidValue;
  if ((a->dists == nullptr) != (a->near_ == nullptr) || (a->dists == nullptr) != (a->far_ == nullptr))
    return (int)hipErrorInvalidValue;
  const int64_t S = (int64_t)a->R * a->N;
  const int fill_blocks = (a->sdf || a->dists) ? (int)((S + LR_SCAN - 1) / LR_SCAN) : 0;
  hipLaunchKernelGGL(inside_list_kernel, dim3(fill_blocks + 1), dim3(LR_SCAN), 0, (hipStream_t)s, *a, fill_blocks);
  MLI_LAUNCH_CHECK();
}

namespace {

constexpr int LT_WAVES = LR_SCAN / 64;

MLI_FI void live_tiles_scan(const mli_live_tiles_args& a) {
  const int R = a.comp.R, N = a.comp.N;
  const int T = N / 32, G = 256 / N;
  int L, W;
  compact_scan<true>(
      R,
      [&](int r) MLI_LAMBDA_FI {
        return (uint32_t)__hip_atomic_load(a.flags + r, __ATOMIC_RELAXED, __HIP_MEMORY_SCOPE_AGENT);
      },
      [&](int r, uint32_t f, int pos, int before, int wbefore) MLI_LAMBDA_FI {
        for (int i = 0; i < T; ++i) {
          const int below = wbefore + __popc(f & ((1u << i) - 1u));
          a.tile_list[pos * T + i] = r * T + i;
          a.tile_rank[r * T + i] = before * T + (f != 0 ? i : 0);
          a.wtile_rank[pos * T + i] = f != 0 ? below : W;
          if ((f >> i) & 1u) a.wtile_list[below] = pos * T + i;
        }
      },
      L, W);
  if (threadIdx.x == 0) {
    a.tile_rank[R * T] = L * T;
    a.wtile_rank[R * T] = W;
    a.n_live_tiles[0] = (L + G - 1) / G * G * T;
  }
}

template <int L>
__global__ __launch_bounds__(LR_SCAN) void live_tiles_kernel(mli_live_tiles_args a) {
  __shared__ int last;
  const int lane = threadIdx.x & 63, w = threadIdx.x >> 6;
  const int sub = lane % L;
  const int r = (blockIdx.x * LT_WAVES + w) * (64 / L) + lane / L;
  const int R = a.comp.R, N = a.comp.N;
  if (r < R) {
    float wv[CE], yk[CE][7], acc[12];
    composite_ray<L>(a.comp, r, sub, wv, yk, acc);
    int nz = 0;
#pragma unroll
    for (int e = 0; e < CE; ++e)
      if (CE * sub + e < N) nz |= (__builtin_bit_cast(uint32_t, wv[e]) & 0x7fffffffu) != 0;
    const uint64_t seg = __ballot(nz) >> (lane / L * L);
    uint32_t f = 0;
#pragma unroll
    for (int j = 0; j < L * CE / 32; ++j)
      if (j * 32 < N && ((seg >> (j * (32 / CE))) & ((1u << (32 / CE)) - 1u)) != 0) f |= 1u << j;
    if (sub == 0) a.flags[r] = (int)f;
    if (f == 0 && a.y != nullptr) {
      const f32x4 z = {0.f, 0.f, 0.f, 0.f};
#pragma unroll
      for (int e = 0; e < CE; ++e) {
        const int k = CE * sub + e;
        if (k < N) {
          f32x4* row = reinterpret_cast<f32x4*>(a.y + ((size_t)k * R + r) * 8);
          row[0] = z;
          row[1] = z;
        }
      }
    }
  }
  if (a.scan_launch) return;
  __threadfence();
  __syncthreads();
  if (threadIdx.x == 0) last = atomicAdd(a.ticket, 1) == (int)gridDim.x - 1;
  __syncthreads();
  if (!last) return;
  __threadfence();
  live_tiles_scan(a);
  if (threadIdx.x == 0) atomicExch(a.ticket, 0);
}

__global__ __launch_bounds__(LR_SCAN) void live_tiles_scan_kernel(mli_live_tiles_args a) { live_tiles_scan(a); }

}

extern "C" int mli_live_tiles(const mli_live_tiles_args* a, mli_stream_t s) {
  const int R = a->comp.R, N = a->comp.N;
  if (R <= 0 || N <= 0 || N % 32 != 0 || 256 % N != 0 || R % (256 / N) != 0) return (int)hipErrorInvalidValue;
  if (a->comp.y != nullptr || !a->comp.weights || !a->flags || !a->tile_list || !a->tile_rank || !a->n_live_tiles ||
      !a->wtile_list || !a->wtile_rank || (!a->scan_launch && !a->ticket))
    return (int)hipErrorInvalidValue;
  if (N <= 32 * CE) {
    const int rpb = 2 * LT_WAVES;
    hipLaunchKernelGGL(live_tiles_kernel<32>, dim3((R + rpb - 1) / rpb), dim3(LR_SCAN), 0, (hipStream_t)s, *a);
  } else {
    hipLaunchKernelGGL(live_tiles_kernel<64>, dim3((R + LT_WAVES - 1) / LT_WAVES), dim3(LR_SCAN), 0, (hipStream_t)s, *a);
  }
  if (a->scan_launch) hipLaunchKernelGGL(live_tiles_scan_kernel, dim3(1), dim3(LR_SCAN), 0, (hipStream_t)s, *a);
  MLI_LAUNCH_CHECK();
}
```

### mli_nerf_amd/csrc/wgrad.hip

```cpp
#include "common.h"

#include <algorithm>

namespace {

constexpr int MAXJOBS = 16;
constexpr int BK = 64;
constexpr int ROWB = BK * 2 + 16;

struct Job {
  const uint16_t* a; const uint16_t* b;
  int M, K, ldw;
  float* dw; float* db;
  int tiles_n, tile_base;
  int a_tiled, b_tiled;
  int a_kst, b_kst;
  const uint16_t* b2;
  int b2_q, b2_kst;
  const float* rb_dz4; const uint8_t* rb_mask; const uint8_t* rb_w4;
  int rb_col, rb_cnt, rb_R, rb_N;
};

MLI_FI const uint16_t* operand_at(const uint16_t* base, bool tiled, int n_rows, int row, size_t S, int k) {
  return tiled ? base + (size_t)(k >> 8) * n_rows * 256 + (size_t)row * 256 + (k & 255) : base + (size_t)row * S + k;
// ... 372 lines not shown
    tstride[u] = kst * 1024;
    sbase[u] = reinterpret_cast<const uint8_t*>(in_a ? J.a : sec ? J.b2 : J.b) + (size_t)tl * tstride[u] +
               (sec ? qg - J.b2_q : qg) * 1024;
    odd[u] = (q & 1) << 7;
  }
  const uint32_t voff = (32 * (lane >> 5) + ((lane & 31) ^ ((lane >> 5) << 2))) * 16;
  auto tile_of = [&](int s) MLI_LAMBDA_FI {
    const int sc = min(s, n_st - 1);
    return wl != nullptr ? sload_i32(wl + to_sgpr(sc)) : t0 + sc * TPS;
  };
  auto issue = [&](auto RBc, int s, int buf) MLI_LAMBDA_FI {
    constexpr int U0 = decltype(RBc)::value ? A_PPW : 0;
    const int tile = tile_of(s);
#pragma unroll
    for (int u = U0; u < PPW; ++u) {
      const uint8_t* sp = sbase[u] + (size_t)tile * tstride[u];
      glds16(sp + (voff ^ (uint32_t)odd[u]), lds + buf * STAGE + piece_of(u) * 1024);
    }
  };
  const bool a_nat = J.a_tiled == 3, b_nat = J.b_tiled == 3;
  uint32_t ba[2][2], bb[2][2];
  {
    const uint32_t l0 = lds_addr(lds);
#pragma unroll
    for (int hf = 0; hf < 2; ++hf)
#pragma unroll
      for (int r = 0; r < 2; ++r) {
        ba[hf][r] = l0 + 2 * wm * TM * 1024 + frag_read_off(lane, hf, r, a_nat);
        bb[hf][r] = l0 + B_OFF + 2 * wn * TN * 1024 + frag_read_off(lane, hf, r, b_nat);
      }
  }

  f32x16 acc[TM][TN];
#pragma unroll
  for (int i = 0; i < TM; ++i)
#pragma unroll
    for (int j = 0; j < TN; ++j)
#pragma unroll
      for (int e = 0; e < 16; ++e) acc[i][j][e] = 0.f;
  const bool do_bias = (J.db != nullptr) && tn == 0 && wn == 0;
  float bsum[TM];
#pragma unroll
  for (int i = 0; i < TM; ++i) bsum[i] = 0.f;
  const half2 ones = {(f16)1.f, (f16)1.f};

  auto consume = [&](int st) MLI_LAMBDA_FI {
    const uint32_t so = (st % NBUF) * STAGE;
    auto read_a = [&](auto KSc, half8 (&ra)[TM]) MLI_LAMBDA_FI {
      constexpr int ks = decltype(KSc)::value, tl = ks >> 1, hf = ks & 1;
      static_for<TM>([&](auto Ic) MLI_LAMBDA_FI {
        constexpr int o = (tl * KA + 2 * decltype(Ic)::value) * 1024;
        const half4 lo = ds_tr16_at<o>(ba[hf][0] + so), hi = ds_tr16_at<o>(ba[hf][1] + so);
        ra[decltype(Ic)::value] = half8{lo[0], lo[1], lo[2], lo[3], hi[0], hi[1], hi[2], hi[3]};
      });
    };
    auto read_b = [&](auto KSc, auto Jc, half8& rb) MLI_LAMBDA_FI {
      constexpr int ks = decltype(KSc)::value, tl = ks >> 1, hf = ks & 1;
      constexpr int o = (tl * KB + 2 * decltype(Jc)::value) * 1024;
      const half4 lo = ds_tr16_at<o>(bb[hf][0] + so), hi = ds_tr16_at<o>(bb[hf][1] + so);
      rb = half8{lo[0], lo[1], lo[2], lo[3], hi[0], hi[1], hi[2], hi[3]};
    };
    half8 fa[2][TM], fb[TN];
    read_a(std::integral_constant<int, 0>{}, fa[0]);
    static_for<TN>([&](auto Jc) MLI_LAMBDA_FI { read_b(std::integral_constant<int, 0>{}, Jc, fb[decltype(Jc)::value]); });
    static_for<2 * TPS>([&](auto KSc) MLI_LAMBDA_FI {
      constexpr int ks = decltype(KSc)::value, cb = ks & 1;
      constexpr bool next = ks + 1 < 2 * TPS;
      if constexpr (next) read_a(std::integral_constant<int, ks + 1>{}, fa[cb ^ 1]);
      static_for<TN>([&](auto Jc) MLI_LAMBDA_FI {
        constexpr int j = decltype(Jc)::value;
        lgkm_wait<next ? 2 * (TN - 1 + TM) : 2 * (TN - 1 - j)>();
        if constexpr (j == 0) {
#pragma unroll
          for (int i = 0; i < TM; ++i) tie(fa[cb][i]);
        }
        tie(fb[j]);
#pragma unroll
        for (int i = 0; i < TM; ++i) acc[i][j] = mfma32(fa[cb][i], fb[j], acc[i][j]);
        if constexpr (next) read_b(std::integral_constant<int, ks + 1>{}, Jc, fb[j]);
      });
      if (do_bias) {
#pragma unroll
        for (int i = 0; i < TM; ++i)
#pragma unroll
          for (int e = 0; e < 8; e += 2)
            bsum[i] = __builtin_amdgcn_fdot2(half2{fa[cb][i][e], fa[cb][i][e + 1]}, ones, bsum[i], false);
      }
    });
  };
  auto stream = [&]() MLI_LAMBDA_FI {
    const std::false_type img{};
#pragma unroll
    for (int d = 0; d < NBUF - 1; ++d) issue(img, d, d);
    for (int st = 0; st < n_st; ++st) {
      vm_wait((NBUF - 2) * PPW);
      block_sync();
      issue(img, st + NBUF - 1, (st + NBUF - 1) % NBUF);
      consume(st);
    }
  };
  if (n_st <= 0) {
  } else if constexpr (CAN_RB) {
    if (J.rb_dz4 != nullptr) {
      const std::true_type rb{};
      constexpr int B_PPW = PPW - A_PPW;
      const int c = lane & 31;
      const uint32_t l0 = lds_addr(lds);
      const uint8_t* wc = J.rb_w4 + wv * W4_CHUNK;
      half8 wf = *reinterpret_cast<const half8*>(wc + lane * 16);
      f32x16 bias;
#pragma unroll
      for (int u = 0; u < 4; ++u) {
        const f32x4 b = *reinterpret_cast<const f32x4*>(wc + 1024 + h * 64 + u * 16);
        bias[4 * u] = b[0]; bias[4 * u + 1] = b[1]; bias[4 * u + 2] = b[2]; bias[4 * u + 3] = b[3];
      }
      tie(wf);
      tie(bias);
      auto issue_e = [&](int s) MLI_LAMBDA_FI {
        if (wv < 2) {
          const int tile = tile_of(s);
          const uint8_t* p;
          if (wv == 0) {
            const int m = (ka.tile_list ? sload_i32(ka.tile_list + tile) : tile) * 32 + c;
            const int r = m / J.rb_N, k = m - r * J.rb_N;
            p = reinterpret_cast<const uint8_t*>(J.rb_dz4) + ((size_t)k * J.rb_R + r) * 32 + h * 16;
          } else {
            p = J.rb_mask + (size_t)tile * 1024 + lane * 16;
          }
          glds16(p, lds + E_OFF + (s % NBUF) * E_SLOT + wv * 1024);
        }
      };
      auto rebuild = [&](int s) MLI_LAMBDA_FI {
        const uint32_t e = l0 + E_OFF + (s % NBUF) * E_SLOT;
        uint32_t d[3];
#pragma unroll
        for (int i = 0; i < 3; ++i) {
          const int f = min(J.rb_col + i, 7);
          d[i] = ds_read_u32(e + ((f >> 2) * 32 + c) * 16 + (f & 3) * 4);
        }
        uint32_t word = ds_read_u32(e + 1024 + lane * 16 + (wv >> 1) * 4);
        lgkm_wait<0>();
#pragma unroll
        for (int i = 0; i < 3; ++i) tie(d[i]);
        tie(word);
        half8 z4;
#pragma unroll
        for (int j = 0; j < 8; ++j) z4[j] = (f16)0.f;
        if (h == 0) {
          z4[0] = (f16)__builtin_bit_cast(float, d[0]);
          if (J.rb_cnt > 1) {
            z4[1] = (f16)__builtin_bit_cast(float, d[1]);
            z4[2] = (f16)__builtin_bit_cast(float, d[2]);
          }
        }
        const f32x16 a = mfma32(wf, z4, bias);
        f32x16 v;
#pragma unroll
        for (int i = 0; i < 16; ++i) v[i] = mask_bit(a[i], word, (wv & 1) * 16 + i);
        const uint32_t dst = l0 + (s % NBUF) * STAGE + 2 * wv * 1024;
        ds_write_f128(dst + frag_chunk(c, h, 0) * 16, __builtin_bit_cast(f32x4, acc_to_frag(v, 0)));
        ds_write_f128(dst + 1024 + frag_chunk(c, h, 1) * 16, __builtin_bit_cast(f32x4, acc_to_frag(v, 1)));
      };
      issue_e(0);
#pragma unroll
      for (int d = 0; d < NBUF - 1; ++d) {
        issue_e(d + 1);
        issue(rb, d, d);
      }
      if (wv < 2) vm_wait((NBUF - 1) * (B_PPW + 1));
      block_sync();
      rebuild(0);
      for (int st = 0; st < n_st; ++st) {
        if (wv < 2) vm_wait((NBUF - 2) * (B_PPW + 1));
        else vm_wait((NBUF - 2) * B_PPW);
        block_sync();
        issue_e(st + NBUF);
        issue(rb, st + NBUF - 1, (st + NBUF - 1) % NBUF);
        consume(st);
        rebuild(st + 1);
      }
    } else {
      stream();
    }
  } else {
    stream();
  }
  vm_wait(0);
  float* slab = nullptr;
  if (ka.part != nullptr) {
    int jx = 0;
#pragma unroll
    for (int j = 1; j < MAXJOBS; ++j)
      if (j < ka.n_jobs && bid >= ka.jobs[j].tile_base) jx = j;
    slab = ka.part + ka.part_base[jx] + (int64_t)split * ((int64_t)J.M * J.K + J.M);
  }
#pragma unroll
  for (int i = 0; i < TM; ++i)
#pragma unroll
    for (int j = 0; j < TN; ++j)
#pragma unroll
      for (int e = 0; e < 16; ++e) {
        const int row = tm * BM + wm * TM * 32 + i * 32 + acc_row(e, h);
        const int col = tn * BN + wn * TN * 32 + j * 32 + rl;
        if (row < J.M && col < J.K) {
          if (slab) slab[(size_t)row * J.K + col] = acc[i][j][e];
          else atomicAdd(J.dw + (size_t)row * J.ldw + col, acc[i][j][e]);
        }
      }
  if (do_bias) {
#pragma unroll
    for (int i = 0; i < TM; ++i) {
      const float v = bsum[i] + __shfl_xor(bsum[i], 32);
      const int row = tm * BM + wm * TM * 32 + i * 32 + rl;
      if (h == 0 && row < J.M) {
        if (slab) slab[(size_t)J.M * J.K + row] = v;
        else atomicAdd(J.db + row, v);
      }
    }
  }
}

struct RArgs {
  const float* part;
  int64_t base[MAXJOBS], first[MAXJOBS + 1];
  float* dw[MAXJOBS];
  float* db[MAXJOBS];
  int M[MAXJOBS], K[MAXJOBS], ldw[MAXJOBS];
  int n_jobs, n_split;
};

__global__ __launch_bounds__(256) void wgrad_reduce_kernel(RArgs r) {
  const int64_t e = (int64_t)blockIdx.x * 256 + threadIdx.x;
  if (e >= r.first[r.n_jobs]) return;
  int j = 0;
#pragma unroll
  for (int q = 1; q < MAXJOBS; ++q)
    if (q < r.n_jobs && e >= r.first[q]) j = q;
  const int64_t loc = e - r.first[j];
  const int64_t MK = (int64_t)r.M[j] * r.K[j], stride = MK + r.M[j];
  if (loc >= MK && r.db[j] == nullptr) return;
  const float* p = r.part + r.base[j] + loc;
  float acc = 0.f;
  int sp = 0;
  for (; sp + 16 <= r.n_split; sp += 16) {
    float v[16];
#pragma unroll
    for (int q = 0; q < 16; ++q) v[q] = p[(int64_t)(sp + q) * stride];
#pragma unroll
    for (int q = 0; q < 16; ++q) acc += v[q];
  }
  for (; sp < r.n_split; ++sp) acc += p[(int64_t)sp * stride];
  if (loc < MK) {
    const int row = (int)(loc / r.K[j]), col = (int)(loc - (int64_t)row * r.K[j]);
    r.dw[j][(size_t)row * r.ldw[j] + col] = acc;
  } else {
    r.db[j][loc - MK] = acc;
  }
}


constexpr int FR_ROW = 256 * 2 + 16;
__global__ __launch_bounds__(512) void frag_rows_kernel(mli_frag_rows_args a) {
  __shared__ __attribute__((aligned(16))) uint8_t st[16 * FR_ROW];
  const int lane = threadIdx.x & 63, wave = threadIdx.x >> 6, tid = threadIdx.x;
  const int c = lane & 31, h = lane >> 5;
  const int tile = blockIdx.x * 8 + wave;
  const bool have = tile < a.tiles;
  const half8* src = reinterpret_cast<const half8*>(a.src + (size_t)(have ? tile : 0) * a.tile_stride) + lane;
  for (int q = 0; q < a.k_steps; ++q) {
    half8 v = src[q * 64];
#pragma unroll
    for (int j = 0; j < 8; ++j) {
      const int kk = a.order ? (8 * (j >> 2) + 4 * h + (j & 3)) : (8 * h + j);
      *reinterpret_cast<f16*>(st + kk * FR_ROW + (wave * 32 + c) * 2) = v[j];
    }
    __syncthreads();
    const int row = tid >> 5, col = (tid & 31) * 8;
    const int64_t s0 = (int64_t)blockIdx.x * 256 + col;
    if (s0 < (int64_t)a.tiles * 32) {
      const u32x4 x = *reinterpret_cast<const u32x4*>(st + row * FR_ROW + col * 2);
      __builtin_nontemporal_store(x, reinterpret_cast<u32x4*>(a.dst + (a.row0 + 16 * q + row) * a.ld + a.col0 + s0));
    }
    __syncthreads();
  }
}

constexpr int DW4_SLICES = 256;

__global__ __launch_bounds__(256) void dw4_partial_kernel(mli_dw4_args a) {
  const int N = a.N, nh = a.n_heads, segs = MLI_Q4_SEGS(N);
  const int wgs = a.R * N / 256;
  const int g0 = (int)((int64_t)wgs * blockIdx.x / gridDim.x);
  const int g1 = (int)((int64_t)wgs * (blockIdx.x + 1) / gridDim.x);
  const int f = threadIdx.x;
  f32x4 acc[3], accb[3];
#pragma unroll
  for (int h = 0; h < 3; ++h) acc[h] = accb[h] = f32x4{0.f, 0.f, 0.f, 0.f};
  for (int g = g0; g < g1; ++g) {
    const int r0 = g * 256 / N, nseg = (g * 256 + 255) / N - r0 + 1;
    for (int sg = 0; sg < nseg; ++sg) {
      if (a.tile_rank != nullptr && a.tile_rank[(r0 + sg + 1) * (N / 32)] == a.tile_rank[(r0 + sg) * (N / 32)]) continue;
      const float* d = a.dray + 8 * (r0 + sg);
      const f32x4* q = reinterpret_cast<const f32x4*>(a.q4) + ((size_t)g * segs + sg) * nh * 257;
#pragma unroll
      for (int h = 0; h < 3; ++h) {
        if (h >= nh) break;
        f32x4 dv;
#pragma unroll
        for (int c = 0; c < 4; ++c) dv[c] = c < a.k_out[h] ? d[3 * h + c] : 0.f;
        acc[h] += dv * __builtin_nontemporal_load(q + h * 257 + f);
        if (f == 0) accb[h] += dv * __builtin_nontemporal_load(q + h * 257 + 256);
      }
    }
  }
  f32x4* ws = reinterpret_cast<f32x4*>(a.workspace) + (size_t)blockIdx.x * nh * 257;
#pragma unroll
  for (int h = 0; h < 3; ++h) {
    if (h >= nh) break;
    ws[h * 257 + f] = acc[h];
    if (f == 0) ws[h * 257 + 256] = accb[h];
  }
}

__global__ __launch_bounds__(256) void dw4_reduce_kernel(mli_dw4_args a, int slices) {
  __shared__ f32x4 red[256];
  const int nh = a.n_heads, e = blockIdx.x;
  const int h = e / 257, row = e - h * 257, j = threadIdx.x;
  const f32x4* ws = reinterpret_cast<const f32x4*>(a.workspace);
  red[j] = j < slices ? ws[(size_t)j * nh * 257 + e] : f32x4{0.f, 0.f, 0.f, 0.f};
  __syncthreads();
  for (int o = 128; o > 0; o >>= 1) {
    if (j < o) red[j] += red[j + o];
    __syncthreads();
  }
  if (j < a.k_out[h]) {
    const float s = red[0][j] * a.scale;
    if (row < 256) a.dw[h][j * 256 + row] = s;
    else a.db[h][j] = s;
  }
}

enum { CLS_BIG = 1, CLS_WIDE = 2, CLS_THIN = 4 };

constexpr bool WIDE_SHARE = true;
constexpr int WIDE_DMA = 2, WIDE_BKD = 64;
constexpr int BIG_DMA = 2;
#ifndef MLI_FRAG_TPS
#define MLI_FRAG_TPS 1
#endif
#ifndef MLI_FRAG_NBUF
#define MLI_FRAG_NBUF 4
#endif
constexpr int FRAG_TPS = MLI_FRAG_TPS, FRAG_NBUF = MLI_FRAG_NBUF;

inline int job_class(const mli_wgrad_job& j) {
  return j.M <= 32 ? CLS_THIN : (j.K <= 256 ? CLS_BIG : CLS_WIDE);
}

inline bool is_frag(int layout) { return layout == MLI_WGRAD_LAYOUT_FRAG_ACC || layout == MLI_WGRAD_LAYOUT_FRAG_NAT; }

inline bool job_valid(const mli_wgrad_job& j, int S) {
  if (j.a_tiled < 0 || j.a_tiled > 3 || j.b_tiled < 0 || j.b_tiled > 3) return false;
  const bool fa = is_frag(j.a_tiled), fb = is_frag(j.b_tiled);
  if (fa != fb) return false;
  if (j.b2_rows && (!fb || j.b2_q <= 0 || j.b2_q > j.b_kst || j.b2_kst <= 0 ||
                    j.b2_q + j.b2_kst < (j.K + 15) / 16))
    return false;
  if (fa && (j.a_kst < (j.M + 15) / 16 || (!j.b2_rows && j.b_kst < (j.K + 15) / 16))) return false;
  if ((j.a_tiled == MLI_WGRAD_LAYOUT_TILED || j.b_tiled == MLI_WGRAD_LAYOUT_TILED) && S % 256 != 0) return false;
  if (j.rb_dz4 && (!fa || j.M != 256 || job_class(j) != CLS_BIG || !j.rb_mask || !j.rb_w4 ||
                   (j.rb_cnt != 1 && j.rb_cnt != 3) || j.rb_col < 0 || j.rb_col + j.rb_cnt > 8 || j.rb_N <= 0 ||
                   (int64_t)j.rb_R * j.rb_N != S))
    return false;
  return true;
}

template <int BM, int BN, int OCC, bool SHARE = false>
int64_t plan(const mli_wgrad_args* a, int cls, bool frag, KArgs& ka) {
  ka.S = a->S;
  int n = 0, tiles = 0;
  for (int i = 0; i < a->n_jobs; ++i) {
    const mli_wgrad_job& j = a->jobs[i];
    if (!job_valid(j, a->S)) return -1;
    if (job_class(j) != cls || is_frag(j.a_tiled) != frag) continue;
    if (n == MAXJOBS || j.ldw < j.K || j.M <= 0 || j.K <= 0) return -1;
    Job& J = ka.jobs[n++];
    J.a = j.a_rows; J.b = j.b_rows; J.M = j.M; J.K = j.K; J.ldw = j.ldw; J.dw = j.dw; J.db = j.db;
    J.a_tiled = j.a_tiled; J.b_tiled = j.b_tiled;
    J.a_kst = j.a_kst; J.b_kst = j.b_kst;
    J.b2 = j.b2_rows; J.b2_q = j.b2_q; J.b2_kst = j.b2_kst;
    J.rb_dz4 = j.rb_dz4;
    J.rb_mask = reinterpret_cast<const uint8_t*>(j.rb_mask);
    J.rb_w4 = reinterpret_cast<const uint8_t*>(j.rb_w4);
    J.rb_col = j.rb_col; J.rb_cnt = j.rb_cnt; J.rb_R = j.rb_R; J.rb_N = j.rb_N;
    J.tiles_n = (j.K + BN - 1) / BN;
    tiles += ((j.M + BM - 1) / BM) * J.tiles_n;
  }
  ka.n_jobs = n;
  ka.part = nullptr;
  ka.tile_rank = ka.tile_list = ka.wtile_rank = ka.wtile_list = nullptr;
  if (n == 0) return 0;
  ka.share = 0;
  if (SHARE) {
    bool ok = n > 1;
    for (int i = 0; ok && i < n; ++i) ok = ka.jobs[i].b == ka.jobs[0].b && ka.jobs[i].M <= BM && ka.jobs[i].tiles_n == 1;
    ka.share = ok ? 1 : 0;
  }
  const int want = ka.share ? 8 * std::max(1, 32 * OCC / n) : std::max(1, 256 * OCC / tiles);
  const int steps = a->S / BK;
  ka.k_split = ((steps + want - 1) / want) * BK;
  ka.n_split = (a->S + ka.k_split - 1) / ka.k_split;
  int base = 0;
  int64_t floats = 0;
  for (int i = 0; i < n; ++i) {
    ka.jobs[i].tile_base = base;
    base += ((ka.jobs[i].M + BM - 1) / BM) * ka.jobs[i].tiles_n * ka.n_split;
    ka.part_base[i] = floats;
    floats += (int64_t)ka.n_split * ((int64_t)ka.jobs[i].M * ka.jobs[i].K + ka.jobs[i].M);
  }
  return floats;
}

template <int BM, int BN, int WM, int WN, int OCC, int DEPTH, bool SHARE_B = false, int DMA_NBUF = 0, int DMA_BKD = 32>
int launch(const mli_wgrad_args* a, int cls, bool frag, hipStream_t s) {
  KArgs ka;
  const int64_t floats = plan<BM, BN, OCC, SHARE_B>(a, cls, frag, ka);
  if (floats < 0) return (int)hipErrorInvalidValue;
  if (ka.n_jobs == 0) return 0;
  if (a->deterministic) {
    if (a->workspace == nullptr) return (int)hipErrorInvalidValue;
    ka.part = a->workspace;
  }
  int grid = 0;
  for (int i = 0; i < ka.n_jobs; ++i) grid += ((ka.jobs[i].M + BM - 1) / BM) * ka.jobs[i].tiles_n * ka.n_split;
  if (a->tile_rank != nullptr) {
    if (!frag || FRAG_TPS != 1 || a->tile_list == nullptr) return (int)hipErrorInvalidValue;
    ka.tile_rank = a->tile_rank;
    ka.tile_list = a->tile_list;
  }
  if (a->wtile_rank != nullptr || a->wtile_list != nullptr) {
    if (a->tile_rank == nullptr || a->wtile_rank == nullptr || a->wtile_list == nullptr) return (int)hipErrorInvalidValue;
    ka.wtile_rank = a->wtile_rank;
    ka.wtile_list = a->wtile_list;
  }
  if (frag) {
    constexpr int LDS = FRAG_NBUF * FRAG_TPS * (BM / 16 + BN / 16) * 1024;
    constexpr int LDS_RB = rebuild_ok(BM, BN, false, FRAG_TPS) ? FRAG_NBUF * E_SLOT : 0;
    static_assert(LDS + LDS_RB <= 160 * 1024, "LDS");
    bool any_rb = false;
    for (int i = 0; i < ka.n_jobs; ++i) any_rb = any_rb || ka.jobs[i].rb_dz4 != nullptr;
    if (SHARE_B && ka.share)
      hipLaunchKernelGGL((wgrad_frag_kernel<BM, BN, WM, WN, FRAG_NBUF, SHARE_B, FRAG_TPS>),
                         dim3(8 * ka.n_jobs * ((ka.n_split + 7) / 8)), dim3(512), LDS, s, ka);
    else
      hipLaunchKernelGGL((wgrad_frag_kernel<BM, BN, WM, WN, FRAG_NBUF, false, FRAG_TPS>), dim3(grid), dim3(512),
                         LDS + (any_rb ? LDS_RB : 0), s, ka);
  } else if (SHARE_B && ka.share) {
    grid = 8 * ka.n_jobs * ((ka.n_split + 7) / 8);
    if constexpr (SHARE_B && DMA_NBUF > 0)
      hipLaunchKernelGGL((wgrad_dma_kernel<BM, BN, WM, WN, DMA_NBUF, true, DMA_BKD>), dim3(grid), dim3(512),
                         DMA_NBUF * (BM + BN) * DMA_BKD * 2, s, ka);
    else if constexpr (SHARE_B)
      hipLaunchKernelGGL((wgrad_kernel<BM, BN, WM, WN, DEPTH, true>), dim3(grid), dim3(512), (BM + BN) * ROWB, s, ka);
  } else if constexpr (DMA_NBUF > 0) {
    hipLaunchKernelGGL((wgrad_dma_kernel<BM, BN, WM, WN, DMA_NBUF, false, DMA_BKD>), dim3(grid), dim3(512),
                       DMA_NBUF * (BM + BN) * DMA_BKD * 2, s, ka);
  } else {
    hipLaunchKernelGGL((wgrad_kernel<BM, BN, WM, WN, DEPTH>), dim3(grid), dim3(512), (BM + BN) * ROWB, s, ka);
  }
  if (!a->deterministic) return (int)hipGetLastError();
  RArgs r;
  r.part = a->workspace;
  r.n_jobs = ka.n_jobs;
  r.n_split = ka.n_split;
  int64_t first = 0;
  for (int i = 0; i < ka.n_jobs; ++i) {
    const Job& J = ka.jobs[i];
    r.base[i] = ka.part_base[i];
    r.first[i] = first;
    r.dw[i] = J.dw; r.db[i] = J.db; r.M[i] = J.M; r.K[i] = J.K; r.ldw[i] = J.ldw;
    first += (int64_t)J.M * J.K + J.M;
  }
  r.first[ka.n_jobs] = first;
  hipLaunchKernelGGL(wgrad_reduce_kernel, dim3((unsigned)((first + 255) / 256)), dim3(256), 0, s, r);
  return (int)hipGetLastError();
}

}

extern "C" int mli_wgrad(const mli_wgrad_args* a, mli_stream_t s) {
  if (a->S <= 0 || a->S % BK != 0) return (int)hipErrorInvalidValue;
  int e = 0;
  for (int frag = 0; frag < 2 && !e; ++frag) {
    if (a->classes & CLS_BIG) e = launch<256, 256, 4, 2, 1, 2, false, BIG_DMA, 64>(a, CLS_BIG, frag, (hipStream_t)s);
    if (!e && (a->classes & CLS_WIDE))
      e = launch<256, 320, 4, 2, 1, 1, WIDE_SHARE, WIDE_DMA, WIDE_BKD>(a, CLS_WIDE, frag, (hipStream_t)s);
    if (!e && (a->classes & CLS_THIN)) e = launch<32, 256, 1, 8, 2, 2>(a, CLS_THIN, frag, (hipStream_t)s);
  }
  return e;
}

extern "C" int mli_wgrad_workspace(const mli_wgrad_args* a, int64_t* bytes) {
  bytes[0] = 0;
  if (a->S <= 0 || a->S % BK != 0) return (int)hipErrorInvalidValue;
  if (!a->deterministic) return 0;
  KArgs ka;
  int64_t mx = 0, f;
  for (int frag = 0; frag < 2; ++frag) {
    if (a->classes & CLS_BIG) { if ((f = plan<256, 256, 1>(a, CLS_BIG, frag, ka)) < 0) return (int)hipErrorInvalidValue; mx = std::max(mx, f); }
    if (a->classes & CLS_WIDE) { if ((f = plan<256, 320, 1, WIDE_SHARE>(a, CLS_WIDE, frag, ka)) < 0) return (int)hipErrorInvalidValue; mx = std::max(mx, f); }
    if (a->classes & CLS_THIN) { if ((f = plan<32, 256, 2>(a, CLS_THIN, frag, ka)) < 0) return (int)hipErrorInvalidValue; mx = std::max(mx, f); }
  }
  bytes[0] = mx * 4;
  return 0;
}

extern "C" int mli_frag_rows(const mli_frag_rows_args* a, mli_stream_t s) {
  if (a->tiles <= 0 || a->k_steps <= 0) return 0;
  if (a->tiles % 8 != 0 || (a->ld % 8) != 0 || (a->col0 % 8) != 0) return (int)hipErrorInvalidValue;
  hipLaunchKernelGGL(frag_rows_kernel, dim3(a->tiles / 8), dim3(512), 0, (hipStream_t)s, *a);
  MLI_LAUNCH_CHECK();
}

static bool dw4_valid(const mli_dw4_args* a) {
  if (a->R <= 0 || a->N <= 0 || a->N % 32 != 0 || (int64_t)a->R * a->N % 256 != 0 || a->n_heads < 1 ||
      a->n_heads > 3)
    return false;
  for (int h = 0; h < a->n_heads; ++h)
    if (a->k_out[h] < 1 || a->k_out[h] > 3 || 3 * h + a->k_out[h] > 8) return false;
  return true;
}

static int dw4_slices(const mli_dw4_args* a) { return std::min(DW4_SLICES, a->R * a->N / 256); }

extern "C" int mli_dw4(const mli_dw4_args* a, mli_stream_t s) {
  if (!dw4_valid(a) || !a->q4 || !a->dray || !a->workspace) return (int)hipErrorInvalidValue;
  if (a->tile_rank && 256 % a->N != 0) return (int)hipErrorInvalidValue;
  for (int h = 0; h < a->n_heads; ++h)
    if (!a->dw[h] || !a->db[h]) return (int)hipErrorInvalidValue;
  const int slices = dw4_slices(a);
  hipLaunchKernelGGL(dw4_partial_kernel, dim3(slices), dim3(256), 0, (hipStream_t)s, *a);
  hipLaunchKernelGGL(dw4_reduce_kernel, dim3(a->n_heads * 257), dim3(256), 0, (hipStream_t)s, *a, slices);
  MLI_LAUNCH_CHECK();
}

extern "C" int mli_dw4_workspace(const mli_dw4_args* a, int64_t* bytes) {
  if (!dw4_valid(a)) return (int)hipErrorInvalidValue;
  bytes[0] = (int64_t)dw4_slices(a) * a->n_heads * 257 * 4 * 4;
  return 0;
}
```

### mli_nerf_amd/engine.py

```python
import contextlib
import ctypes as C
import math
import os
import types

import numpy as np
import torch

from . import _lib as L
from . import layout
from .hashgrid import level_table, normal_eps


class PathConfig:

    def __init__(self, n_coarse=64, n_fine=16, n_hier=4, white_bg=True, bounding="sphere",
                 aabb=(-1, -1, -1, 1, 1, 1), outside_val=1000.0, anneal_end=0.1, log2T=22,
                 levels=16, min_logres=5, max_logres=11, light_visibility=None, scale_rule="fp32"):
        self.n_coarse, self.n_fine, self.n_hier = n_coarse, n_fine, n_hier
        self.scale_rule = scale_rule
        self.white_bg, self.bounding, self.aabb = white_bg, bounding, tuple(float(x) for x in aabb)
        self.outside_val, self.anneal_end = outside_val, anneal_end
        self.log2T, self.levels, self.min_logres, self.max_logres = log2T, levels, min_logres, max_logres
        self.light_visibility = light_visibility

    @property
    def n_samples(self):
        return self.n_coarse + self.n_fine * self.n_hier


def _grid_levels(cfg):
    table, total = level_table(cfg.levels, cfg.log2T, cfg.min_logres, cfg.max_logres, cfg.scale_rule)
    g = L.GridLevels()
    for i, (scale, res, size, off) in enumerate(table):
        g.scale[i], g.res[i], g.size[i], g.offset[i] = scale, res, size, off
        g.modmagic[i] = layout.fastmod_magic(size)
    return g, total


GEOMETRY_BUFS = frozenset(["center", "ray_unit", "ray_norm", "pts_light", "near", "far", "outside",
                           "d_coarse", "s_coarse", "d_m0", "d_m1", "s_m0", "s_m1", "d_f0", "d_f1", "s_f0",
                           "s_f1", "dists", "sdf", "grad", "hess", "h0", "enc5", "inside_list", "n_inside"])


class _Lane:

    def __init__(self, shared=None):
        self.own = {}
        self.step = self.own if shared is None else shared

    def of(self, name):
        return self.own if name in GEOMETRY_BUFS else self.step


class _Lanes:

    def __init__(self):
        self._lanes = {0: _Lane()}
        self._lane = self._lanes[0]
        self._shared_step = {}

    def _lane_named(self, lane, geometry_only):
        if lane not in self._lanes:
            self._lanes[lane] = _Lane(self._shared_step if geometry_only else None)
        found = self._lanes[lane]
        if geometry_only != (found.step is not found.own):
            raise RuntimeError("engine lane %r was created with geometry_only=%s" % (lane, not geometry_only))
        return found

    def use_lane(self, lane, geometry_only=False):
        self._lane = self._lane_named(lane, geometry_only)

    @contextlib.contextmanager
    def lane(self, lane, geometry_only=False):
        prev = self._lane
        self._lane = lane if isinstance(lane, _Lane) else self._lane_named(lane, geometry_only)
        try:
            yield
        finally:
            self._lane = prev

    def _buf(self, name, shape, dtype=torch.float32):
        bufs = self._lane.of(name)
        t = bufs.get(name)
        n = math.prod(shape)
        if t is None or t.numel() < n or t.dtype != dtype:
            t = bufs[name] = torch.empty(n, dtype=dtype, device=self.device)
        return t[:n].view(*shape)

    @property
    def _bufs(self):
        lane = self._lane
        return types.MappingProxyType(lane.own if lane.step is lane.own else {**lane.step, **lane.own})


SWITCHES = (
    ("wgrad_slab_classes", "MLI_WGRAD_SLABS", 2, int),
    ("dz3_rebuild", "MLI_DZ3_REBUILD", True, bool),
    ("elide_dead_rays", "MLI_ELIDE_DEAD", True, bool),
    ("live_tiles_pass", "MLI_LIVE_TILES_PASS", 1, int),
    ("skip_zero_tiles", "MLI_SKIP_ZERO_TILES", True, bool),
    ("elide_outside", "MLI_ELIDE_OUTSIDE", True, bool),
    ("elide_outside_sampling", "MLI_ELIDE_OUTSIDE_SAMPLING", True, bool),
)


GRAD_CLASSES = ("out", "big", "wide")
GRAD_CLASS_LAYERS = {"out": (4,), "big": (1, 2, 3), "wide": (0,)}


def _head_dw_sizes(k_out):
    return [(256, layout.K0)] + [(256, 256)] * 3 + [(k_out, 256)]


def _dw_numel(sizes):
    return sum(m * k + m for m, k in sizes)


def _to_device_structs(structs, device):
    raw = b"".join(bytes(s) for s in structs)
    return torch.frombuffer(bytearray(raw), dtype=torch.uint8).to(device)


class RenderEngine(_Lanes):

    def __init__(self, cfg, device, stage="b"):
        if torch.device(device).type != "cuda":
            raise RuntimeError("RenderEngine runs on the MI355X (libmli_hip.so); the model is on %s" % device)
        self.cfg = cfg
        self.stage = stage
        self.head_specs = layout.HEADS_A if stage == "a" else layout.HEADS
        self.device = torch.device(device)
        self.levels, self.table_entries = _grid_levels(cfg)
        self.set_normal_eps(normal_eps(cfg.levels, cfg.min_logres, cfg.max_logres))
        self.active_levels = cfg.levels
        self.table16 = None
        self.table_grad_clean = None
        self._dw_zero = None
        self._y_zeroed = None
        self.wsdf = torch.empty(65536 + 5 * 1024 + 16, dtype=torch.uint8, device=self.device)
        self.fplan, fbytes = layout.fwd_plan(self.head_specs)
        self.bplan, bbytes = layout.geo_plan() if stage == "a" else layout.bwd_plan()
        self._bwd_off = (fbytes + 255) // 256 * 256
        self._wimg = torch.empty(self._bwd_off + bbytes, dtype=torch.uint8, device=self.device)
        self.wfwd = self._wimg[:fbytes]
        self.wbwd = self._wimg[self._bwd_off:]
        self.wsdf_t = torch.empty(65536, dtype=torch.uint8, device=self.device) if stage == "a" else None
        self._kmaps = []
        self.tlayout, self.n_train = layout.trainable_layout(stage)
        self.toff = {name: (off, shape) for name, shape, off in self.tlayout}
        _Lanes.__init__(self)
        self.gate_wgrad, self.gate_event = False, None
        self.u_fine = (C.c_float * 64)(*(layout.u_fine(cfg.n_fine) + [2.0] * (64 - cfg.n_fine)))
        self._pack_descs = None
        self.trace = None
        self.deterministic = False
        for name, env, default, kind in SWITCHES:
            v = os.environ.get(env)
            setattr(self, name, default if v is None else int(v) if kind is int else v != "0")
        self.pq = True
        self._wplans = {}
        self._kinv = {(name, li): torch.from_numpy((layout.head_kinv(name, k_in) if li == 0 else
                                                    np.arange(256)).astype(np.int16)).to(self.device)
                      for name, k_in, _ in layout.HEADS for li in range(5)}

    def set_normal_eps(self, normal_eps_value):
        eps64 = float(normal_eps_value) / np.sqrt(3)
        self.eps = float(np.float32(eps64))
        self.grad_den = float(np.float32(4.0 * eps64))
        self.hess_den = float(np.float32(eps64 ** 2))

    def load_table(self, params_flat):
        assert params_flat.numel() == self.table_entries * 8, (params_flat.numel(), self.table_entries)
        if self.table16 is None or self.table16.numel() != params_flat.numel():
            self.table16 = torch.empty(params_flat.numel(), dtype=torch.float16, device=self.device)
        L.call("mli_cast_f16", L.CastArgs(L.ptr(params_flat), L.ptr(self.table16), params_flat.numel()))

    def pack_sdf(self, v0, g0, b0, w_sdf, b_sdf):
        L.call("mli_pack_sdf", L.PackSdfArgs(L.ptr(v0), L.ptr(g0), L.ptr(b0), L.ptr(w_sdf), L.ptr(b_sdf),
                                             L.ptr(self.wsdf)))
        if self.wsdf_t is not None:
            L.call("mli_pack_sdf_t", L.PackSdfTArgs(L.ptr(v0), L.ptr(g0), L.ptr(self.wsdf_t)))

    def load_sdf(self, params_flat, v0, g0, b0, w_sdf, b_sdf):
        self.load_table(params_flat)
        self.pack_sdf(v0, g0, b0, w_sdf, b_sdf)

    def _descs(self, plan, tensors, base=0):
        descs = []
        for p in plan:
            km = torch.from_numpy(p["kmap"].astype(np.int16)).to(self.device)
            kmode = torch.from_numpy(p["kmode"].astype(np.uint8)).to(self.device)
            nm = None
            if p.get("nmap") is not None:
                nm = torch.from_numpy(p["nmap"].astype(np.int16)).to(self.device)
            self._kmaps += [km, kmode, nm]
            v, g, b = tensors(p["prefix"])
            descs.append(L.PackLayer(L.ptr(v), L.ptr(g), L.ptr(b), p["n_out"], p["k_ref"], p["transpose"],
                                     p["n_tiles"], p["k_steps"], L.ptr(km), L.ptr(kmode), base + p["dst_offset"],
                                     p["chunk_stride"], L.ptr(nm)))
        return descs

    def pack_heads(self, flat, sdf_l1):
        def tensors(prefix):
            if prefix == "neural_sdf.mlp.linears.1" and sdf_l1 is not None:
                return sdf_l1
            return tuple(self.param_view(flat, prefix + s) for s in (".weight_v", ".weight_g", ".bias"))
        key = (flat.data_ptr(), None if sdf_l1 is None else sdf_l1[0].data_ptr())
        if self._pack_descs is None or self._pack_descs[0] != key:
            self._kmaps = []
            descs = self._descs(self.fplan, tensors) + self._descs(self.bplan, tensors, self._bwd_off)
            self._pack_descs = (key, _to_device_structs(descs, self.device), len(descs))
        _, d, n = self._pack_descs
        L.call("mli_pack", L.PackArgs(n, L.ptr(d), L.ptr(self._wimg), L.ptr(self._buf("pack_scale", (n, 256)))))

    def param_view(self, flat, name):
        off, shape = self.toff[name]
        n = int(np.prod(shape))
        return flat[off:off + n].reshape(shape)

    @torch.no_grad()
    def rays(self, pose, intr, pose_light, ray_idx, W, R=None, first_pixel=0):
        w2c, w2l, K = pose[0].contiguous(), pose_light[0].contiguous(), intr[0].contiguous()
        R = R if ray_idx is None else ray_idx.shape[-1]
        ridx = None if ray_idx is None else ray_idx.reshape(-1).to(torch.int64).contiguous()
        out = dict(center=self._buf("center", (R, 3)), ray_unit=self._buf("ray_unit", (R, 3)),
                   ray_norm=self._buf("ray_norm", (R,)), pts_light=self._buf("pts_light", (R, 3)),
                   near=self._buf("near", (R,)), far=self._buf("far", (R,)),
                   outside=self._buf("outside", (R,), torch.uint8))
        aabb = (C.c_float * 6)(*self.cfg.aabb)
        L.call("mli_rays", L.RaysArgs(L.ptr(K), L.ptr(w2c), L.ptr(w2l), L.ptr(ridx), first_pixel, R, W,
                                      1 if self.cfg.bounding == "box" else 0, aabb,
                                      L.ptr(out["center"]), L.ptr(out["ray_unit"]), L.ptr(out["ray_norm"]),
                                      L.ptr(out["pts_light"]), L.ptr(out["near"]), L.ptr(out["far"]),
                                      L.ptr(out["outside"])))
        out["_keep"] = (w2c, w2l, K, ridx)
        return out

    def _sdf(self, rays, dists, n_per_ray, out, mode=0, grad=None, hess=None, h0=None, inside=(None, None)):
        R = rays["center"].shape[0]
        enc = None
        if mode == 1:
            tiles = (R * n_per_ray + 31) // 32
            enc = self._buf("enc5", (tiles * 32 * 640,), torch.float16)
        L.call("mli_sdf", L.SdfArgs(mode, R, n_per_ray, L.ptr(rays["center"]), L.ptr(rays["ray_unit"]),
                                    L.ptr(dists), L.ptr(rays["outside"]), L.ptr(self.table16), self.levels,
                                    L.ptr(self.wsdf), self.eps, self.grad_den, self.hess_den,
                                    self.cfg.outside_val, 1 if hess is not None else 0, L.ptr(out),
                                    L.ptr(grad), L.ptr(hess), L.ptr(h0), L.ptr(enc), int(self.active_levels),
                                    L.ptr(inside[0]), L.ptr(inside[1])))
        return enc

    @torch.no_grad()
    def inside_rays(self, rays, training, elide=True):
        N = self.cfg.n_samples
        if not (elide and self.elide_outside and self.elides(N, training)):
            return None
        R, sampling = rays["center"].shape[0], bool(self.elide_outside_sampling)
        lst, n = self._buf("inside_list", (R,), torch.int32), self._buf("n_inside", (1,), torch.int32)
        hess = self._buf("hess", (N, R, 3)) if training else None
        sdf, grad = self._buf("sdf", (N, R)), self._buf("grad", (N, R, 3))
        fill = (rays["near"], rays["far"], self._buf("dists", (N, R))) if sampling else ()
        L.call("mli_inside_list", L.InsideListArgs(
            R, N, 256 // N - 1, L.ptr(rays["outside"]), L.ptr(lst), L.ptr(n), self.cfg.outside_val, L.ptr(sdf),
            L.ptr(grad), L.ptr(hess), *[L.ptr(t) for t in fill]))
        return lst, n, sampling

    @torch.no_grad()
    def sample(self, rays, u=None, inside=None):
        cfg = self.cfg
        R = rays["center"].shape[0]
        Nc, Nf, H, N = cfg.n_coarse, cfg.n_fine, cfg.n_hier, cfg.n_samples
        inside = inside[:2] if inside is not None and inside[2] else (None, None)
        lst = (L.ptr(inside[0]), L.ptr(inside[1]))
        mode = 0 if inside[0] is None else 2
        d0 = self._buf("d_coarse", (Nc, R))
        uu = None if u is None else u.reshape(R, Nc).contiguous()
        L.call("mli_sample_coarse", L.SampleCoarseArgs(L.ptr(rays["near"]), L.ptr(rays["far"]), L.ptr(uu),
                                                       R, Nc, L.ptr(d0)))
        s0 = self._buf("s_coarse", (Nc, R))
        self._sdf(rays, d0, Nc, s0, mode=mode, inside=inside)
        da, sa, na, db, sb, nb = d0, s0, Nc, None, None, 0
        for h in range(H):
            dm = self._buf("d_m%d" % (h & 1), (na + nb, R))
            sm = self._buf("s_m%d" % (h & 1), (na + nb, R))
            f = self._buf("d_f%d" % (h & 1), (Nf, R))
            L.call("mli_sample_fine", L.SampleFineArgs(R, L.ptr(da), L.ptr(sa), na, L.ptr(db), L.ptr(sb), nb,
                                                       L.ptr(dm), L.ptr(sm), Nf, float(64 * 2 ** h),
                                                       C.cast(self.u_fine, C.c_void_p), L.ptr(f), *lst))
            sf = None
            if h < H - 1:
                sf = self._buf("s_f%d" % (h & 1), (Nf, R))
                self._sdf(rays, f, Nf, sf, mode=mode, inside=inside)
            if self.trace is not None:
                self.trace.append(dict(merged=dm.clone(), merged_sdf=sm.clone(), fine=f.clone(),
                                       fine_sdf=None if sf is None else sf.clone()))
            da, sa, na, db, sb, nb = dm, sm, na + nb, f, sf, Nf
        dists = self._buf("dists", (N, R))
        L.call("mli_sample_fine", L.SampleFineArgs(R, L.ptr(da), None, na, L.ptr(db), None, nb, L.ptr(dists),
                                                   None, 0, 0.0, None, None, *lst))
        return dists

    @torch.no_grad()
    def field(self, rays, dists, training, inside=None, u=None):
        N, R = dists.shape
        sdf, grad = self._buf("sdf", (N, R)), self._buf("grad", (N, R, 3))
        hess = self._buf("hess", (N, R, 3)) if training else None
        h0 = self._buf("h0", (N * R * 256,), torch.float16)
        elided = inside is not None
        sampled = elided and inside[2]
        enc = self._sdf(rays, dists, N, sdf, mode=1, grad=grad, hess=hess, h0=h0,
                        inside=inside[:2] if elided else (None, None))
        return dict(sdf=sdf, grad=grad, hess=hess, h0=h0, enc=enc, elided=elided,
                    lane=self._lane if elided else None, sampling_elided=sampled, u=u if sampled else None)

    def geometry(self, data, W, training, u=None, elide=False):
        rays = self.rays(data["pose"], data["intr"], data["pose_light"], data["ray_idx"], W)
        inside = self.inside_rays(rays, training, elide)
        dists = self.sample(rays, u, inside)
        return rays, dists, self.field(rays, dists, training, inside, u)

    @torch.no_grad()
    def densify(self, st):
        rays, dists, fld = st[0], st[1], st[2]
        if not fld.get("elided"):
            return st
        with self.lane(fld["lane"]):
            dense = dict(dists=dists)
            if fld.get("sampling_elided"):
                u = fld["u"]
                if u is not None:
                    u.record_stream(torch.cuda.current_stream(u.device))
                dense["dists"] = self.sample(rays, u)
            dense.update(self.field(rays, dists, fld["hess"] is not None))
        for k in ("dists", "sdf", "grad", "hess", "h0", "enc"):
            have = dists if k == "dists" else fld[k]
            if (dense[k] is None) != (have is None) or (dense[k] is not None
                                                        and dense[k].data_ptr() != have.data_ptr()):
                raise RuntimeError("densify: the state's lane no longer holds its %s buffer" % k)
        fld.update(elided=False, lane=None, sampling_elided=False, u=None)
        return st

    def pq_mode(self, N, training):
        return bool(self.pq and training and self.stage == "b" and N % 32 == 0)

    @torch.no_grad()
    def weights(self, rays, dists, fld, s_var, progress):
        out = self._composite_out(dists, outputs=False)
        L.call("mli_composite_fwd", self._composite_args(rays, dists, fld, dict(y=None), s_var, progress, out))
        return out["weights"]

    @torch.no_grad()
    def elides(self, N, training):
        return bool(self.elide_dead_rays and self.pq_mode(N, training) and 256 % N == 0)

    @torch.no_grad()
    def heads(self, rays, dists, fld, training, s_var=None, progress=0.0, elide=False):
        N, R = dists.shape
        S = N * R
        if S % 256:
            raise ValueError("heads: rays x samples = %d x %d is not a whole number of 256-sample tiles (the "
                             "reference configs' batches are: 4096 / 8192 rays x 128 / 192 samples)" % (R, N))
        nh = len(self.head_specs)
        y = self._buf("y", (N, R, 8))
        if nh == 1 and self._y_zeroed != y.data_ptr():
            y.zero_()
            self._y_zeroed = y.data_ptr()
        feat = self._buf("feat", (S * layout.K0,), torch.float16)
        xT = masks = w = tl = tr = nl = wl = wr = None
        pq = s_var is not None and self.pq_mode(N, training)
        if training and self.stage == "b" and not self.deterministic:
            self._zero_once(self._buf("dw", (_dw_numel(self._dw_sizes()),)))
        if training:
            xT = self._buf("xT", (nh, 3 if pq else 4, S * 256), torch.float16)
            masks = self._buf("masks", (nh, 4, S // 32, 64, 4), torch.int32)
        if pq and elide and self.elides(N, training):
            w, tl, tr, nl, wl, wr = self._live_lists(rays, dists, fld, y, s_var, progress)
        else:
            self.densify((rays, dists, fld))
            if pq:
                w = self.weights(rays, dists, fld, s_var, progress)
        q4 = self._buf("q4", (S // 256, layout.q4_segs(N), nh, 257, 4)) if pq else None
        L.call("mli_rgb_fwd", L.RgbFwdArgs(R, N, L.ptr(rays["center"]), L.ptr(rays["ray_unit"]),
                                           L.ptr(rays["pts_light"]), L.ptr(dists), L.ptr(fld["grad"]),
                                           L.ptr(fld["h0"]), L.ptr(self.wfwd), L.ptr(y), L.ptr(feat),
                                           L.ptr(xT), L.ptr(masks), nh, L.ptr(w), L.ptr(q4), L.ptr(tl), L.ptr(nl)))
        return dict(y=y, x0T=feat if training else None, xT=xT, masks=masks, feat=feat, q4=q4,
                    tile_list=tl, tile_rank=tr, n_live_tiles=nl, wtile_list=wl, wtile_rank=wr)

    def _live_lists(self, rays, dists, fld, y, s_var, progress):
        N, R = dists.shape
        T = N * R // 32
        tl = self._buf("tile_list", (T,), torch.int32)
        tr = self._buf("tile_rank", (T + 1,), torch.int32)
        nl = self._buf("n_live_tiles", (1,), torch.int32)
        flags = self._buf("live_flags", (R,), torch.int32)
        if not self.live_tiles_pass:
            w = self.weights(rays, dists, fld, s_var, progress)
            L.call("mli_live_rays", L.LiveRaysArgs(R, N, L.ptr(w), L.ptr(y), L.ptr(flags), L.ptr(tl), L.ptr(tr),
                                                   L.ptr(nl)))
            return w, tl, tr, nl, None, None
        out = self._composite_out(dists, outputs=False)
        w, comp = out["weights"], self._composite_args(rays, dists, fld, dict(y=None), s_var, progress, out)
        wl = self._buf("wtile_list", (T,), torch.int32)
        wr = self._buf("wtile_rank", (T + 1,), torch.int32)
        step = self._lane.step
        if "live_ticket" not in step:
            step["live_ticket"] = torch.zeros(1, dtype=torch.int32, device=self.device)
        L.call("mli_live_tiles", L.LiveTilesArgs(comp, L.ptr(y), L.ptr(flags), L.ptr(tl), L.ptr(tr), L.ptr(nl),
                                                 L.ptr(wl), L.ptr(wr), L.ptr(step["live_ticket"]),
                                                 0 if self.live_tiles_pass == 2 else 1))
        return (w, tl, tr, nl, wl, wr) if self.skip_zero_tiles else (w, tl, tr, nl, None, None)

    def _composite_out(self, dists, outputs=True, extras=False):
        N, R = dists.shape
        new = lambda c: torch.empty(R, c, device=self.device) if outputs else None
        out = dict(weights=self._buf("weights", (N, R)), rgb=new(3), o_r=new(3), o_s=new(1), o_re=new(3))
        if extras:
            out.update(opacity=new(1), gradient=new(3), depth=new(1))
            if self.cfg.light_visibility:
                out["blend_dist"] = new(1)
        return out

    @torch.no_grad()
    def composite(self, rays, dists, fld, hd, s_var, progress, training):
        out = self._composite_out(dists, extras=not training)
        L.call("mli_composite_fwd", self._composite_args(rays, dists, fld, hd, s_var, progress, out))
        return out

    def _composite_args(self, rays, dists, fld, hd, s_var, progress, out):
        N, R = dists.shape
        anneal = min(progress / self.cfg.anneal_end, 1.0)
        return L.CompositeArgs(R, N, L.ptr(dists), L.ptr(rays["far"]), L.ptr(rays["ray_unit"]),
                               L.ptr(rays["ray_norm"]), L.ptr(fld["sdf"]), L.ptr(fld["grad"]), L.ptr(hd["y"]),
                               L.ptr(s_var), float(anneal), 1 if self.cfg.white_bg else 0, L.ptr(out["weights"]),
                               L.ptr(out["rgb"]), L.ptr(out["o_r"]), L.ptr(out["o_s"]), L.ptr(out["o_re"]),
                               L.ptr(out.get("opacity")), L.ptr(out.get("gradient")), L.ptr(out.get("depth")),
                               L.ptr(out.get("blend_dist")))

    @staticmethod
    def grad_scale(R):
        return float(2.0 ** round(math.log2(max(R, 1)) + 2))

    @torch.no_grad()
    def composite_loss(self, rays, dists, fld, hd, s_var, progress, loss, defer=False):
        N, R = dists.shape
        out = self._composite_out(dists)
        dz4 = self._buf("dz4", (N, R, 8))
        dray = self._buf("dray", (R, 8)) if hd.get("q4") is not None else None
        args = L.CompositeLossArgs(self._composite_args(rays, dists, fld, hd, s_var, progress, out), loss,
                                   self.grad_scale(R), L.ptr(dz4), 1 if defer else 0, L.ptr(dray))
        n = L.workspace("mli_composite_loss", args)[0] // 4
        args.loss.scratch = L.ptr(self._buf("cl_scratch", (n,)))
        L.call("mli_composite_loss", args)
        if defer:
            if self._lane.step.get("cl_deferred") is not None:
                raise RuntimeError("composite_loss(defer=True): the previous deferred loss values on this "
                                   "lane were never finished (finish_losses)")
            self._lane.step["cl_deferred"] = args
        return out, dz4

    def finish_losses(self):
        args = self._lane.step.pop("cl_deferred", None)
        if args is not None:
            L.call("mli_composite_loss_finalize", args)

    def drop_deferred(self):
        self._lane.step.pop("cl_deferred", None)

    def _vis_config(self):
        vis = self.cfg.light_visibility
        if vis.get("type", "sphere_tracing") != "sphere_tracing":
            raise NotImplementedError("light visibility type %r (only 'sphere_tracing', the configs' choice, "
                                      "is built)" % vis.get("type"))
        kind = {"blend_z_sphere_tracing": 0, "blend_z": 1, "sphere_tracing": 2}[vis["camera_ray_type"]]
        box = vis.get("bounding", "sphere") == "box"
        r2 = float(np.float32(float(vis.get("radius", 1.0)) ** 2))
        return kind, box, r2, float(vis.get("gamma") or 0.0)

    @torch.no_grad()
    def light_visibility(self, rays, comp, iters=20):
        kind, box, r2, gamma = self._vis_config()
        R = rays["center"].shape[0]
        f = lambda *shape: torch.empty(*shape, device=self.device)
        u8 = lambda n: torch.empty(n, 1, dtype=torch.uint8, device=self.device)
        o = dict(inter_dist=f(R, 1), inter_mask=u8(R), visibility=u8(R), normal_x_light=f(R, 1),
                 pseudo_shading=f(R, 1))
        scratch = dict(light_unit=f(R, 3), near_l=f(R), far_t=f(R), inside=u8(R), inter_pts=f(R, 3))
        L.call("mli_light_visibility", L.LightVisibilityArgs(
            R, L.ptr(rays["center"]), L.ptr(rays["ray_unit"]), L.ptr(rays["pts_light"]), L.ptr(rays["near"]),
            L.ptr(rays["far"]), L.ptr(comp["blend_dist"]), L.ptr(comp["gradient"]), kind, iters, 1 if box else 0,
            r2, (C.c_float * 6)(*self.cfg.aabb), gamma, L.ptr(self.table16), self.levels,
            int(self.active_levels), L.ptr(self.wsdf), L.ptr(scratch["light_unit"]), L.ptr(scratch["near_l"]),
            L.ptr(scratch["far_t"]), L.ptr(scratch["inside"]), L.ptr(o["inter_dist"]), L.ptr(o["inter_mask"]),
            L.ptr(scratch["inter_pts"]), L.ptr(o["visibility"]), L.ptr(o["normal_x_light"]),
            L.ptr(o["pseudo_shading"])))
        o["visibility"] = o["visibility"].bool()
        o["inter_mask"] = o["inter_mask"].bool()
        comp.update(o)
        return comp

    def stamp(self):
        return (id(self._lane), self._lane.step.get("__gen", 0))

    def check_stamp(self, stamp):
        lane = next((ln for ln in self._lanes.values() if id(ln) == stamp[0]), None)
        if lane is None:
            raise RuntimeError("render state of an unknown engine lane")
        if lane.step.get("__gen", 0) != stamp[1]:
            raise RuntimeError("render state overwritten: another render ran on the same engine lane "
                               "between this forward and its backward")

    def render(self, data, s_var, progress, training, u=None, W=512, composite=True, elide=False):
        step = self._lane.step
        step["__gen"] = step.get("__gen", 0) + 1
        rays, dists, fld = self.geometry(data, W, training, u, elide and s_var is not None)
        hd = self.heads(rays, dists, fld, training, s_var, progress, elide=elide)
        if not composite:
            return rays, dists, fld, hd, None
        comp = self.composite(rays, dists, fld, hd, s_var, progress, training)
        if self.cfg.light_visibility and not training:
            self.light_visibility(rays, comp)
        return rays, dists, fld, hd, comp

    @torch.no_grad()
    def light_points(self, pose_lights, R):
        w2l = pose_lights.to(self.device, torch.float32).contiguous()
        n = w2l.shape[0]
        pl = self._buf("pts_lights", (n, R, 3))
        L.call("mli_light_points", L.LightPointsArgs(n, R, L.ptr(w2l), L.ptr(pl)))
        return pl

    @torch.no_grad()
    def lights_visibility(self, rays, pts_lights, comps, iters=20):
        kind, box, r2, gamma = self._vis_config()
        n, R = pts_lights.shape[0], rays["center"].shape[0]
        f = lambda *shape: torch.empty(*shape, device=self.device)
        u8 = lambda *shape: torch.empty(*shape, dtype=torch.uint8, device=self.device)
        inter_dist, inter_mask, inter_pts = f(R, 1), u8(R, 1), f(R, 3)
        L.call("mli_camera_hit", L.CameraHitArgs(
            R, L.ptr(rays["center"]), L.ptr(rays["ray_unit"]), L.ptr(rays["near"]), L.ptr(rays["far"]),
            L.ptr(comps[0]["blend_dist"]), kind, iters, L.ptr(self.table16), self.levels, int(self.active_levels),
            L.ptr(self.wsdf), L.ptr(inter_dist), L.ptr(inter_mask), L.ptr(inter_pts)))
        vis, nxl, sh = u8(n, R, 1), f(n, R, 1), f(n, R, 1)
        L.call("mli_light_shadows", L.LightShadowsArgs(
            n, R, L.ptr(pts_lights), L.ptr(inter_pts), L.ptr(comps[0]["gradient"]), 1 if box else 0, r2,
            (C.c_float * 6)(*self.cfg.aabb), gamma, iters, L.ptr(self.table16), self.levels,
            int(self.active_levels), L.ptr(self.wsdf), L.ptr(vis), L.ptr(nxl), L.ptr(sh)))
        vis, inter_mask = vis.bool(), inter_mask.bool()
        for l, comp in enumerate(comps):
            comp.update(inter_dist=inter_dist, inter_mask=inter_mask, visibility=vis[l], normal_x_light=nxl[l],
                        pseudo_shading=sh[l])
        return comps

    SHARED_MAPS = ("opacity", "gradient", "depth", "blend_dist")

    def render_lights(self, data, pose_lights, s_var, progress, W=512):
        step = self._lane.step
        step["__gen"] = step.get("__gen", 0) + 1
        rays, dists, fld = self.geometry(dict(data, pose_light=pose_lights[:1]), W, False)
        pl = self.light_points(pose_lights, rays["center"].shape[0])
        comps = []
        for l in range(pl.shape[0]):
            rl = dict(rays, pts_light=pl[l])
            hd = self.heads(rl, dists, fld, False, s_var, progress)
            out = self._composite_out(dists, extras=l == 0)
            L.call("mli_composite_fwd", self._composite_args(rl, dists, fld, hd, s_var, progress, out))
            if l:
                out.update({k: comps[0][k] for k in self.SHARED_MAPS if k in comps[0]})
            comps.append(out)
        if self.cfg.light_visibility:
            self.lights_visibility(rays, pl, comps)
        return rays, dists, fld, comps

    @staticmethod
    def _dw_sizes():
        return [mk for _, _, k_out in layout.HEADS for mk in _head_dw_sizes(k_out)]

    def _wgrad_plan(self, dzT, dz4T, hd, dwbuf, flat, grad_out, S, rebuild=None):
        pq = hd.get("q4") is not None
        key = (dzT.data_ptr(), None if dz4T is None else dz4T.data_ptr(), hd["x0T"].data_ptr(),
               hd["xT"].data_ptr(), dwbuf.data_ptr(), flat.data_ptr(), grad_out.data_ptr(), S, pq,
               None if rebuild is None else (rebuild[0].data_ptr(), hd["masks"].data_ptr()) + tuple(rebuild[1:]))
        hit = self._wplans.get(key)
        if hit is not None:
            return hit
        if len(self._wplans) >= 8:
            self._wplans.clear()
        sizes = self._dw_sizes()
        jobs, assemble, off = [], [], 0
        dw4, db4, k4 = [None] * 3, [None] * 3, [0] * 3
        for hdx, (name, k_in, k_out) in enumerate(layout.HEADS):
            for li in range(5):
                m, k = sizes[hdx * 5 + li]
                dw = dwbuf[off:off + m * k]
                db = dwbuf[off + m * k:off + m * k + m]
                off += m * k + m
                if li == 0:
                    jobs.append(L.frag_job(L.ptr(dzT[hdx, 0]), L.ptr(hd["x0T"]), m, k, L.ptr(dw), L.ptr(db), k, 16,
                                           layout.K0 // 16))
                elif li < 4:
                    jobs.append(L.frag_job(L.ptr(dzT[hdx, li]), L.ptr(hd["xT"][hdx, li - 1]), m, k, L.ptr(dw),
                                           L.ptr(db), k, 16, 16))
                    if li == 3 and rebuild is not None:
                        j, (dz4, R, N) = jobs[-1], rebuild
                        j.rb_dz4, j.rb_mask = L.ptr(dz4), L.ptr(hd["masks"][hdx, 3])
                        j.rb_w4 = L.ptr(self.wbwd) + self.bplan[4 * hdx]["dst_offset"]
                        j.rb_col, j.rb_cnt, j.rb_R, j.rb_N = 3 * hdx, k_out, R, N
                elif pq:
                    dw4[hdx], db4[hdx], k4[hdx] = L.ptr(dw), L.ptr(db), m
                else:
                    jobs.append(L.frag_job(L.ptr(dz4T[hdx]), L.ptr(hd["xT"][hdx, 3]), m, k, L.ptr(dw), L.ptr(db), k,
                                           1, 16))
                pre = layout.param_prefix(name, li)
                v = self.param_view(flat, pre + ".weight_v")
                g = self.param_view(flat, pre + ".weight_g")
                k_ref = v.shape[1]
                kinv_t = self._kinv[(name, li)]
                assemble.append(L.AssembleLayer(L.ptr(dw), L.ptr(db), L.ptr(v), L.ptr(g), m, k_ref, k,
                                                L.ptr(kinv_t), L.ptr(self.param_view(grad_out, pre + ".weight_v")),
                                                L.ptr(self.param_view(grad_out, pre + ".weight_g")),
                                                L.ptr(self.param_view(grad_out, pre + ".bias")), None))
        job_arr = (L.WgradJob * len(jobs))(*jobs)
        order = [h * 5 + li for cls in GRAD_CLASSES for li in GRAD_CLASS_LAYERS[cls] for h in range(len(layout.HEADS))]
        ad = _to_device_structs([assemble[i] for i in order], self.device)
        plan = (job_arr, ad, (dw4, db4, k4))
        self._wplans[key] = plan
        return plan

    def _wgrad(self, S, jobs, classes, hd=None):
        tr, tl, wr, wl = (None,) * 4 if hd is None else [hd.get(k) for k in ("tile_rank", "tile_list", "wtile_rank",
                                                                             "wtile_list")]
        slab = 7 if self.deterministic else self.wgrad_slab_classes
        need = sum(classes) & slab
        ws = None
        if need:
            q = L.WgradArgs(S, len(jobs), C.cast(jobs, C.c_void_p), need, 1, None)
            nbytes = L.workspace("mli_wgrad", q)[0]
            ws = self._buf("wgrad_ws", (max(nbytes, 4) // 4,))
        for cls in classes:
            for part, det in ((cls & ~slab, 0), (cls & slab, 1)):
                if part:
                    L.call("mli_wgrad", L.WgradArgs(S, len(jobs), C.cast(jobs, C.c_void_p), part, det, L.ptr(ws),
                                                    L.ptr(tr), L.ptr(tl), L.ptr(wr), L.ptr(wl)))

    @torch.no_grad()
    def backward(self, st, d_rgb, d_o_r, d_o_s, d_o_re, flat, sdf_l1, grad_out, dz4=None, on_class=None):
        rays, dists, fld, hd, comp = st
        N, R = dists.shape
        S = N * R
        scale = self.grad_scale(R)
        pq = hd.get("q4") is not None
        rebuild = self.dz3_rebuild and dz4 is not None
        if dz4 is None and hd.get("tile_list") is not None:
            raise RuntimeError("backward: the heads ran with elide=True (the fused train step's mode); the "
                               "three-call tail needs the dense images")
        if dz4 is None:
            dz4 = self._buf("dz4", (N, R, 8))
            c = lambda t: None if t is None else t.contiguous()
            L.call("mli_composite_bwd", L.CompositeBwdArgs(R, N, L.ptr(comp["weights"]), L.ptr(hd["y"]),
                                                           L.ptr(comp["o_r"]), L.ptr(comp["o_s"]), L.ptr(c(d_rgb)),
                                                           L.ptr(c(d_o_r)), L.ptr(c(d_o_s)), L.ptr(c(d_o_re)),
                                                           scale, L.ptr(dz4),
                                                           L.ptr(self._buf("dray", (R, 8)) if pq else None)))
        dz4T = None if pq else self._buf("dz4T", (3, S * 16), torch.float16)
        dwbuf = self._buf("dw", (_dw_numel(self._dw_sizes()),))
        zero_dw = 0 if self.deterministic else 1
        if zero_dw:
            self._zero_once(dwbuf)
            self._dw_zero = None
        dzT = self._buf("dzT", (3, 4, S * 256), torch.float16)
        L.call("mli_rgb_bwd", L.RgbBwdArgs(R, N, L.ptr(dz4), L.ptr(self.wbwd), L.ptr(hd["masks"]), L.ptr(dzT),
                                           L.ptr(dz4T), 1 if rebuild else 0, L.ptr(hd.get("tile_list")),
                                           L.ptr(hd.get("n_live_tiles"))))
        jobs, ad, (dw4, db4, k4) = self._wgrad_plan(dzT, dz4T, hd, dwbuf, flat, grad_out, S,
                                                    (dz4, R, N) if rebuild else None)
        if self.gate_wgrad:
            self.gate_event = torch.cuda.Event()
            self.gate_event.record()
        if on_class is None:
            if pq:
                self._dw4(R, N, hd, scale, dw4, db4, k4)
                self._wgrad(S, jobs, (1, 2), hd)
            else:
                self._wgrad(S, jobs, (1, 2, 4), hd)
            L.call("mli_grad_assemble", L.AssembleArgs(15, L.ptr(ad), 1.0 / scale, zero_dw))
            self._dw_zero = dwbuf.data_ptr() if zero_dw else None
            return grad_out
        nh, sz = len(layout.HEADS), C.sizeof(L.AssembleLayer)
        first = 0
        for cls in GRAD_CLASSES:
            if cls == "out":
                if pq:
                    self._dw4(R, N, hd, scale, dw4, db4, k4)
                else:
                    self._wgrad(S, jobs, (4,), hd)
            else:
                self._wgrad(S, jobs, (1,) if cls == "big" else (2,), hd)
            n = nh * len(GRAD_CLASS_LAYERS[cls])
            L.call("mli_grad_assemble", L.AssembleArgs(n, L.ptr(ad) + first * sz, 1.0 / scale, zero_dw))
            first += n
            on_class(cls)
        self._dw_zero = dwbuf.data_ptr() if zero_dw else None
        return grad_out

    def _zero_once(self, buf):
        if self._dw_zero != buf.data_ptr():
            buf.zero_()
            self._dw_zero = buf.data_ptr()

    def _dw4(self, R, N, hd, scale, dw4, db4, k4):
        args = L.Dw4Args(R, N, 3, L.ptr(hd["q4"]), L.ptr(self._lane.step["dray"]), scale / L.Q4_SCALE,
                         (C.c_void_p * 3)(*dw4), (C.c_void_p * 3)(*db4), (C.c_int * 3)(*k4), None,
                         L.ptr(hd.get("tile_rank")))
        args.workspace = L.ptr(self._buf("dw4_ws", (L.workspace("mli_dw4", args)[0] // 4,)))
        L.call("mli_dw4", args)

    def _assemble_desc(self, dw, db, v, g, n_out, k_ref, k_pack, kinv, gv, gg, gb, plain=0):
        kinv_t = torch.from_numpy(np.asarray(kinv).astype(np.int16)).to(self.device)
        return L.AssembleLayer(L.ptr(dw), L.ptr(db), L.ptr(v), L.ptr(g), n_out, k_ref, k_pack, L.ptr(kinv_t),
                               L.ptr(gv), L.ptr(gg), L.ptr(gb), None, plain), kinv_t

    def _plan_a(self, bufs, flat, grad_flat, S):
        key = tuple(t.data_ptr() for t in bufs.values()) + (flat.data_ptr(), grad_flat.data_ptr(), S)
        if getattr(self, "_aplan", None) is not None and self._aplan[0] == key:
            return self._aplan[1:]
        head = layout.HEADS_A[0][0]
        sizes = _head_dw_sizes(3)
        dw, off = bufs["dw"], 0
        jobs_s, jobs_5s, descs, keep = [], [], [], []

        def take(m, k):
            nonlocal off
            w, b = dw[off:off + m * k], dw[off + m * k:off + m * k + m]
            off += m * k + m
            return w, b
        pv = lambda n: self.param_view(flat, n)
        gv = lambda n: self.param_view(grad_flat, n)
        for li, (m, k) in enumerate(sizes):
            w, b = take(m, k)
            a_rows = bufs["dzT"][li] if li < 4 else bufs["dz4T"]
            b_rows = bufs["x0T"] if li == 0 else bufs["xT"][0, li - 1]
            jobs_s.append(L.frag_job(L.ptr(a_rows), L.ptr(b_rows), m, k, L.ptr(w), L.ptr(b), k, 16 if li < 4 else 1,
                                     layout.K0 // 16 if li == 0 else 16))
            pre = layout.param_prefix(head, li)
            k_ref = pv(pre + ".weight_v").shape[1]
            kinv = layout.head_kinv(head, k_ref) if li == 0 else np.arange(k_ref)
            d, kt = self._assemble_desc(w, b, pv(pre + ".weight_v"), pv(pre + ".weight_g"), m, k_ref, k, kinv,
                                        gv(pre + ".weight_v"), gv(pre + ".weight_g"), gv(pre + ".bias"))
            descs.append(d)
            keep.append(kt)
        w, b = take(256, 256)
        jobs_s.append(L.frag_job(L.ptr(bufs["dz1T"]), L.ptr(bufs["h0"]), 256, 256, L.ptr(w), L.ptr(b), 256, 16, 16))
        pre = "neural_sdf.mlp.linears.1"
        d, kt = self._assemble_desc(w, b, pv(pre + ".weight_v"), pv(pre + ".weight_g"), 256, 256, 256,
                                    np.arange(256), gv(pre + ".weight_v"), gv(pre + ".weight_g"), gv(pre + ".bias"))
        descs.append(d)
        keep.append(kt)
        w, b = take(256, layout.SDF_K0)
        jobs_5s.append(L.frag_job(L.ptr(bufs["dz0_frag"]), L.ptr(bufs["enc"]), 256, layout.SDF_K0, L.ptr(w), L.ptr(b),
                                  layout.SDF_K0, 16, 8, order=L.FRAG_ACC, b_order=L.FRAG_NAT,
                                  b2=L.ptr(bufs["p_frag"]), b2_q=8, b2_kst=1))
        pre = "neural_sdf.mlp.linears.0"
        kinv0 = np.concatenate([128 + np.arange(3), np.arange(128)])
        d, kt = self._assemble_desc(w, b, pv(pre + ".weight_v"), pv(pre + ".weight_g"), 256, layout.SDF_K0,
                                    layout.SDF_K0, kinv0, gv(pre + ".weight_v"),
                                    gv(pre + ".weight_g"), gv(pre + ".bias"))
        descs.append(d)
        keep.append(kt)
        dws = bufs["dws"]
        d, kt = self._assemble_desc(dws[:256], dws[256:257], None, None, 1, 256, 256, np.arange(256),
                                    gv("neural_sdf.mlp.linear_sdf.weight"), None,
                                    gv("neural_sdf.mlp.linear_sdf.bias"), plain=1)
        descs.append(d)
        keep.append(kt)
        js = (L.WgradJob * len(jobs_s))(*jobs_s)
        j5 = (L.WgradJob * len(jobs_5s))(*jobs_5s)
        ad = _to_device_structs(descs, self.device)
        self._aplan = (key, js, j5, ad, len(descs), keep, off)
        return self._aplan[1:]

    def _table_grad_target(self, grad_table):
        if self.deterministic:
            return self._buf("hash_ws", (grad_table.numel(),), torch.int64)
        self._lane.step.pop("hash_ws", None)
        return grad_table

    @torch.no_grad()
    def backward_a(self, st, d_rgb, flat, grad_flat, grad_table, w_eikonal, w_curvature, progress,
                   d_grad_ext=None, d_hess_ext=None):
        rays, dists, fld, hd, comp = st
        N, R = dists.shape
        S = N * R
        scale = self.grad_scale(R)
        f16 = torch.float16
        dz4, d_sdf, d_grad = self._buf("dz4", (N, R, 8)), self._buf("d_sdf", (N, R)), self._buf("d_grad", (N, R, 3))
        dinv = self._buf("d_inv_s_part", (R,))
        anneal = min(progress / self.cfg.anneal_end, 1.0)
        s_var = self.param_view(flat, "s_var")
        L.call("mli_composite_bwd_geo", L.CompositeBwdGeoArgs(
            R, N, L.ptr(dists), L.ptr(rays["far"]), L.ptr(rays["ray_unit"]), L.ptr(fld["sdf"]), L.ptr(fld["grad"]),
            L.ptr(hd["y"]), L.ptr(s_var), float(anneal), 1 if self.cfg.white_bg else 0, L.ptr(d_rgb.contiguous()),
            scale, L.ptr(dz4), L.ptr(d_sdf), L.ptr(d_grad), L.ptr(dinv), L.ptr(self.param_view(grad_flat, "s_var"))))
        b = dict(dzT=self._buf("dzT", (4, 256 * S), f16), dz4T=self._buf("dz4T", (16 * S,), f16),
                 x0T=hd["x0T"], xT=hd["xT"], dz1T=self._buf("dz1T", (256 * S,), f16),
                 h0=fld["h0"], enc=fld["enc"], dz0_frag=self._buf("dz0_frag", (5 * S * 256,), f16),
                 p_frag=self._buf("p_frag", (5 * S * 16,), f16), dws=self._buf("dws", (257,)))
        d_nrm = self._buf("d_nrm", (N, R, 4))
        dh0 = self._buf("dh0", (S * 256,), f16)
        L.call("mli_geo_bwd", L.GeoBwdArgs(R, N, L.ptr(dz4), L.ptr(self.wbwd), L.ptr(hd["masks"]), L.ptr(hd["feat"]),
                                           L.ptr(b["dzT"]), L.ptr(b["dz4T"]), L.ptr(d_nrm), L.ptr(b["dz1T"]),
                                           L.ptr(dh0)))
        d_enc = self._buf("d_enc", (S * 640,))
        part = self._buf("sdf_bwd_part", (L.workspace("mli_sdf_bwd", L.SdfBwdArgs(R, N))[3] // 4,))
        L.call("mli_sdf_bwd", L.SdfBwdArgs(
            R, N, L.ptr(rays["center"]), L.ptr(rays["ray_unit"]), L.ptr(dists), L.ptr(rays["outside"]),
            L.ptr(fld["grad"]), L.ptr(fld["hess"]), L.ptr(d_sdf), L.ptr(d_grad), L.ptr(d_nrm), L.ptr(dh0),
            L.ptr(fld["enc"]), L.ptr(self.wsdf), L.ptr(self.wsdf_t), self.eps, self.grad_den, self.hess_den,
            float(w_eikonal), float(w_curvature), scale, L.ptr(d_enc), L.ptr(b["dz0_frag"]), L.ptr(b["p_frag"]),
            L.ptr(b["dws"][:256]), L.ptr(b["dws"][256:]), L.ptr(d_grad_ext), L.ptr(d_hess_ext), L.ptr(part)))
        det = 1 if self.deterministic else 0
        target = self._table_grad_target(grad_table)
        hws = target if det else None
        if det or self.table_grad_clean != grad_table.data_ptr():
            target.zero_()
        self.table_grad_clean = None
        L.call("mli_hash_bwd", L.HashBwdArgs(R, N, L.ptr(rays["center"]), L.ptr(rays["ray_unit"]), L.ptr(dists),
                                             L.ptr(d_enc), self.levels, self.eps, int(self.active_levels),
                                             L.ptr(grad_table), det, L.ptr(hws), grad_table.numel()))
        b["dw"] = self._buf("dw_a", (_dw_numel(_head_dw_sizes(3) + [(256, 256), (256, layout.SDF_K0)]),))
        js, j5, ad, n_desc, _, _ = self._plan_a(b, flat, grad_flat, S)
        zero_dw = 0 if self.deterministic else 1
        if zero_dw:
            self._zero_once(b["dw"])
            self._dw_zero = None
        self._wgrad(S, js, (7,))
        self._wgrad(5 * S, j5, (7,))
        L.call("mli_grad_assemble", L.AssembleArgs(n_desc, L.ptr(ad), 1.0 / scale, zero_dw))
        self._dw_zero = b["dw"].data_ptr() if zero_dw else None
        return grad_flat, grad_table
```

### mli_nerf_amd/model.py

```python
import math

import numpy as np
import torch
import torch.nn.functional as F

from . import layout
from .engine import SWITCHES, PathConfig, RenderEngine
from .hashgrid import GRID_DEFAULTS, level_table


def _cfg_get(node, path, default=None):
    cur = node
    for key in path.split("."):
        if cur is None or not hasattr(cur, key) and not (isinstance(cur, dict) and key in cur):
            return default
        cur = cur[key] if isinstance(cur, dict) else getattr(cur, key)
    return cur


def path_config_from(cfg_model, cfg_data):
    ns = cfg_model.render.num_samples
    hg = cfg_model.object.sdf.encoding.hashgrid
    box = _cfg_get(cfg_data, "bounding_type", "unit_sphere") == "box"
    inside_out = bool(_cfg_get(cfg_model, "object.sdf.mlp.inside_out", False))
    lv = _cfg_get(cfg_model, "light_visibility", None)
    vis = None
    if lv is not None and _cfg_get(lv, "enabled", False):
        vis = dict(camera_ray_type=_cfg_get(lv, "camera_ray_type", None), type=_cfg_get(lv, "type", None),
                   bounding=_cfg_get(lv, "visibility_bounding_type", "sphere"),
                   radius=float(_cfg_get(lv, "visibility_sphere_radius", 1.0)),
                   gamma=float(_cfg_get(lv, "gamma_correlation", 0.0) or 0.0))
    return PathConfig(light_visibility=vis, n_coarse=ns.coarse, n_fine=ns.fine, n_hier=cfg_model.render.num_sample_hierarchy,
                      white_bg=bool(cfg_model.background.white), bounding="box" if box else "sphere",
                      aabb=tuple(_cfg_get(cfg_data, "bounding_box_aabb", (-1, -1, -1, 1, 1, 1))),
                      outside_val=1000.0 * (-1 if inside_out else 1),
                      anneal_end=float(cfg_model.object.s_var.anneal_end),
                      log2T=int(hg.dict_size), levels=int(cfg_model.object.sdf.encoding.levels),
                      min_logres=int(hg.min_logres), max_logres=int(hg.max_logres),
                      scale_rule=str(_cfg_get(hg, "scale_rule", "fp32")))


class WNLinear(torch.nn.Module):

    def __init__(self, v, g, b):
        super().__init__()
        self.bias = v_param(b)
        self.weight_g = v_param(g)
        self.weight_v = v_param(v)


class PlainLinear(torch.nn.Module):
    def __init__(self, w, b):
        super().__init__()
        self.weight, self.bias = v_param(w), v_param(b)


def v_param(t, requires_grad=False):
    return torch.nn.Parameter(t, requires_grad=requires_grad)


class _MLP(torch.nn.Module):
    def __init__(self, linears):
        super().__init__()
        self.linears = torch.nn.ModuleList(linears)


class _Encoding(torch.nn.Module):
    def __init__(self, n_params):
        super().__init__()
        self.params = torch.nn.Parameter(torch.zeros(n_params), requires_grad=False)


class NeuralSDF(torch.nn.Module):

    def __init__(self, pcfg, c2f=None, view=None):
        super().__init__()
        _, total = level_table(pcfg.levels, pcfg.log2T, pcfg.min_logres, pcfg.max_logres, pcfg.scale_rule)
        self.tcnn_encoding = _Encoding(total * 8)
        k0 = 3 + pcfg.levels * 8
        if view is None:
            mlp = _MLP([WNLinear(torch.zeros(256, k0), torch.ones(256, 1), torch.zeros(256)),
                        WNLinear(torch.zeros(256, 256), torch.ones(256, 1), torch.zeros(256))])
            mlp.linear_sdf = PlainLinear(torch.zeros(1, 256), torch.zeros(1))
        else:
            pre = "neural_sdf.mlp."
            mlp = _MLP([WNLinear(*(view(pre + "linears.%d.%s" % (li, n)) for n in ("weight_v", "weight_g", "bias")))
                        for li in range(2)])
            mlp.linear_sdf = PlainLinear(view(pre + "linear_sdf.weight"), view(pre + "linear_sdf.bias"))
            for p in list(mlp.parameters()) + [self.tcnn_encoding.params]:
                p.requires_grad_(True)
        self.mlp = mlp
        self.levels = pcfg.levels
        g = np.exp((np.log(2 ** pcfg.max_logres) - np.log(2 ** pcfg.min_logres)) / (pcfg.levels - 1))
        self.growth_rate = g
        self.resolutions = [int(np.floor(2 ** pcfg.min_logres * g ** lv)) + 1 for lv in range(pcfg.levels)]
        self.normal_eps = 1.0 / self.resolutions[-1]
        self.active_levels = self.anneal_levels = pcfg.levels
        self.warm_up_end = 0
        self.c2f = c2f if c2f is not None and c2f.get("enabled", False) else None

    def set_normal_epsilon(self):
        res = self.resolutions[self.anneal_levels - 1] if self.c2f else self.resolutions[-1]
        self.normal_eps = 1.0 / res

    def set_active_levels(self, current_iter=None):
        if self.c2f is None or current_iter is None:
            self.active_levels = self.anneal_levels = len(self.resolutions)
            return
        anneal = max((current_iter - self.warm_up_end) // self.c2f["step"], 1)
        self.anneal_levels = min(self.levels, anneal)
        self.active_levels = max(self.c2f["init_active_level"], self.anneal_levels)


class LumenRGB(torch.nn.Module):

    def __init__(self, view, heads=layout.HEADS):
        super().__init__()
        self.network_mode = "rgb" if len(heads) == 1 else "rgb_r_s"
        for head, _, _ in heads:
            lins = []
            for li in range(5):
                pre = layout.param_prefix(head, li)
                lins.append(WNLinear(view(pre + ".weight_v"), view(pre + ".weight_g"), view(pre + ".bias")))
                for p in lins[-1].parameters():
                    p.requires_grad_(True)
            setattr(self, head, _MLP(lins))


class _RenderHeads(torch.autograd.Function):

    @staticmethod
    def forward(ctx, table, model, data, u, progress, training, *params):
        eng = model.engine
        st = eng.render(data, model.s_var.detach(), progress, training, u=u, W=model.image_width)
        ctx.state = st
        ctx.stamp = eng.stamp()
        ctx.model = model
        ctx.progress = progress
        model._last_state = st
        comp, fld = st[4], st[2]
        if model.stage != "a":
            return comp["rgb"], comp["o_r"], comp["o_s"], comp["o_re"]
        hess = fld["hess"].clone() if fld["hess"] is not None else torch.zeros_like(fld["grad"])
        return comp["rgb"], comp["o_r"], comp["o_s"], comp["o_re"], fld["grad"].clone(), hess

    @staticmethod
    def backward(ctx, d_rgb, d_o_r, d_o_s, d_o_re, d_grads=None, d_hess=None):
        model = ctx.model
        if ctx.state is None:
            raise RuntimeError("_RenderHeads: backward through the same render twice")
        model.engine.check_stamp(ctx.stamp)
        grad = torch.zeros_like(model.flat)
        gt = None
        if model.stage == "a":
            st = ctx.state
            N, R = st[1].shape
            d_rgb = torch.zeros(R, 3, device=grad.device) if d_rgb is None else d_rgb.contiguous()
            gt = torch.empty_like(model.neural_sdf.tcnn_encoding.params)
            c = lambda t: None if t is None else t.contiguous()
            model.engine.backward_a(st, d_rgb, model.flat.detach(), grad, gt, 0.0, 0.0, ctx.progress,
                                    d_grad_ext=c(d_grads), d_hess_ext=c(d_hess))
        else:
            model.engine.backward(ctx.state, d_rgb, d_o_r, d_o_s, d_o_re, model.flat, model._sdf_l1(), grad)
        ctx.state = None
        views = [grad[off:off + n].view(shape) if need else None
                 for (_, shape, off, n), need in zip(model._trainable_items(), ctx.needs_input_grad[6:])]
        return (gt if ctx.needs_input_grad[0] else None, None, None, None, None, None, *views)


class Model(torch.nn.Module):
    def __init__(self, cfg_model, cfg_data):
        super().__init__()
        self.cfg_model, self.cfg_data = cfg_model, cfg_data
        self.pcfg = path_config_from(cfg_model, cfg_data)
        self.image_size_train = list(cfg_data.train.image_size)
        self.image_size_val = list(cfg_data.val.image_size)
        self.rand_rays_val = int(_cfg_get(cfg_model, "render.rand_rays_val", cfg_model.render.rand_rays))
        self.white_background = self.pcfg.white_bg
        self.outside_val = self.pcfg.outside_val
        self.anneal_end = self.pcfg.anneal_end
        self.progress = 0.0
        self.stratified = bool(cfg_model.render.stratified)
        mode = _cfg_get(cfg_model, "object.rgb.network_mode", None)
        if mode not in (None, "rgb", "rgb_r_s"):
            raise NotImplementedError("LumenRGB network_mode %r is outside the built hot path" % mode)
        self.stage = "b" if mode == "rgb_r_s" else "a"
        self._layout = {name: (shape, off) for name, shape, off in layout.trainable_layout(self.stage)[0]}
        n_train = layout.trainable_layout(self.stage)[1]
        self.register_buffer("flat", torch.zeros(n_train), persistent=False)
        c2f = _cfg_get(cfg_model, "object.sdf.encoding.coarse2fine", None)
        c2f = None if c2f is None else {k: c2f[k] for k in ("enabled", "init_active_level", "step") if k in c2f}
        if self.stage == "a":
            self.neural_sdf = NeuralSDF(self.pcfg, c2f, view=self._view)
            self.neural_rgb = LumenRGB(self._view, layout.HEADS_A)
            self.s_var = torch.nn.Parameter(self._view("s_var"), requires_grad=True)
            with torch.no_grad():
                self.s_var.fill_(float(cfg_model.object.s_var.init_val))
        else:
            self.neural_sdf = NeuralSDF(self.pcfg, c2f)
            self.neural_rgb = LumenRGB(self._view)
            self.s_var = torch.nn.Parameter(torch.tensor(float(cfg_model.object.s_var.init_val)),
                                            requires_grad=False)
        if self.pcfg.bounding == "box":
            self.bounding_box_aabb = torch.tensor(self.pcfg.aabb)
        self.engine = None
        self._streams = None
        self.pipeline_chunks = True
        self._sdf_version = None
        self.image_width = self.image_size_train[1]
        self.deterministic = False
        self.pq = True
        for name, _, _, _ in SWITCHES:
            setattr(self, name, None)

    def _view(self, name, flat=None):
        shape, off = self._layout[name]
        flat = self.flat if flat is None else flat
        return flat.data[off:off + int(np.prod(shape))].view(shape)

    def _layout_items(self):
        return layout.trainable_layout(self.stage)[0]

    def _trainable_items(self):
        return [(n, shape, off, int(np.prod(shape))) for n, shape, off in layout.trainable_layout(self.stage)[0]]

    def trainable_parameters(self):
        named = dict(self.named_parameters())
        return [named[n] for n, _, _, _ in self._trainable_items()]

    def device(self):
        return self.flat.device

    def set_flat_grad(self, grad):
        self.flat.grad = grad
        for p, (_, shape, off, n) in zip(self.trainable_parameters(), self._trainable_items()):
            p.grad = grad[off:off + n].view(shape)

    def flat_grad_from_params(self):
        ps = self.trainable_parameters()
        if all(p.grad is None for p in ps):
            return None
        out = torch.zeros_like(self.flat)
        for p, (_, _, off, n) in zip(ps, self._trainable_items()):
            if p.grad is not None:
                out[off:off + n].copy_(p.grad.reshape(-1))
        return out

    @torch.no_grad()
    def init_weights(self, seed=0):
        from . import synthetic
        pc = self.pcfg
        sd = synthetic.make_state_dict(
            log2T=pc.log2T, seed=seed, s_var=float(self.cfg_model.object.s_var.init_val), enc_std=0.0,
            table_amp=1e-4, heads="rgb" if self.stage == "a" else "rgb_r_s",
            out_bias=float(_cfg_get(self.cfg_model, "object.sdf.mlp.out_bias", 0.5)), scale_rule=pc.scale_rule)
        self.load_state_dict(sd)

    TABLE_KEY = "neural_sdf.tcnn_encoding.params"

    def load_state_dict(self, state_dict, strict=True, assign=False):
        src = state_dict.get(self.TABLE_KEY)
        if src is not None and src.numel() != self.neural_sdf.tcnn_encoding.params.numel():
            self._adopt_table_size(src.numel())
        res = super().load_state_dict(state_dict, strict=strict, assign=assign)
        if src is not None:
            self.table_sharded_stale = False
        return res

    def _adopt_table_size(self, numel):
        from .hashgrid import SCALE_RULES
        pc = self.pcfg
        sizes = {}
        for rule in SCALE_RULES:
            table, total = level_table(pc.levels, pc.log2T, pc.min_logres, pc.max_logres, rule)
            sizes[rule] = (total * 8, [r for _, r, _, _ in table])
        match = [r for r, (n, _) in sizes.items() if n == numel]
        if not match:
            raise ValueError(
                "%s has %d elements; this hash-grid config expects %s" % (
                    self.TABLE_KEY, numel, ", ".join("%d (%d entries x 8; %s scale rule, level resolutions %s)"
                                                     % (n, n // 8, r, res[:7]) for r, (n, res) in sizes.items())))
        rule = match[0]
        import warnings
        warnings.warn("checkpoint hash table has %d elements: level-5 resolution %d (%s scale rule); the level "
                      "table follows it" % (numel, sizes[rule][1][5], rule))
        pc.scale_rule = rule
        p = self.neural_sdf.tcnn_encoding.params
        p.data = torch.zeros(numel, dtype=p.dtype, device=p.device)
        self.engine = None
        self._sdf_version = None

    def _apply(self, fn, recurse=True):
        super()._apply(fn, recurse)
        flat = self.flat.detach()
        self._buffers["flat"] = flat
        for name, p in self.named_parameters():
            if name in self._layout:
                p.data = self._view(name, flat)
        self.engine = None
        self._sdf_version = None
        return self

    def _sdf_l1(self):
        if self.stage == "a":
            return None
        l1 = self.neural_sdf.mlp.linears[1]
        return (l1.weight_v.detach(), l1.weight_g.detach().reshape(-1), l1.bias.detach())

    def prepare(self):
        if self.engine is None:
            self.engine = RenderEngine(self.pcfg, self.flat.device, self.stage)
        sdf = self.neural_sdf
        eng = self.engine
        eng.deterministic = self.deterministic
        eng.pq = self.pq
        for name, _, _, _ in SWITCHES:
            if getattr(self, name) is not None:
                setattr(eng, name, getattr(self, name))
        eng.set_normal_eps(sdf.normal_eps)
        eng.active_levels = int(sdf.active_levels)
        l0 = sdf.mlp.linears[0]
        pack_args = (l0.weight_v.detach(), l0.weight_g.detach().reshape(-1), l0.bias.detach(),
                     sdf.mlp.linear_sdf.weight.detach().reshape(-1), sdf.mlp.linear_sdf.bias.detach())
        if self.stage == "a":
            table = sdf.tcnn_encoding.params
            ver = (table._version, table.data_ptr())
            if ver != self._sdf_version:
                if getattr(self, "table_sharded_stale", False):
                    raise RuntimeError("the hash table is ZeRO-sharded and not gathered: call "
                                       "trainer.sync_table() on every rank before rebuilding the engine")
                eng.load_table(table.detach())
                self._sdf_version = ver
            eng.pack_sdf(*pack_args)
        else:
            ver = tuple(p._version for p in sdf.parameters()) + tuple(p.data_ptr() for p in sdf.parameters())
            if ver != self._sdf_version:
                eng.load_sdf(sdf.tcnn_encoding.params.detach(), *pack_args)
                self._sdf_version = ver
        eng.pack_heads(self.flat.detach(), self._sdf_l1())

    def get_param_groups(self, cfg_optim):
        keywords = _cfg_get(cfg_optim, "partial_training", None)
        if keywords is None:
            return self.parameters()
        return [p for n, p in self.named_parameters() if any(k in n for k in keywords)]

    def forward(self, data, u=None):
        self.prepare()
        u = self.stratified_uniforms(data, u)
        self.image_width = self.image_size_train[1]
        table = self.neural_sdf.tcnn_encoding.params
        res = _RenderHeads.apply(table, self, data, u, self.progress, self.training, *self.trainable_parameters())
        return self.outputs(self._last_state, res)

    def stratified_uniforms(self, data, u=None):
        if not (self.stratified and self.training):
            return None
        if u is None:
            u = torch.rand(1, data["ray_idx"].shape[-1], self.pcfg.n_coarse, device=self.flat.device)
        return u

    def outputs(self, st, heads=None):
        if st[2].get("elided"):
            self.engine.densify(st)
        rays, dists, fld, hd, comp = st
        heads = heads if heads is not None else (comp["rgb"], comp["o_r"], comp["o_s"], comp["o_re"])
        rgb, o_r, o_s, o_re = heads[:4]
        grads, hess = (heads[4], heads[5]) if len(heads) == 6 else (fld["grad"], fld["hess"])
        if len(heads) == 6 and fld["hess"] is None:
            hess = None
        N, R = dists.shape
        out = dict(rgb=rgb[None], o_r=o_r[None], o_s=o_s[None], o_re=o_re[None],
                   outside=rays["outside"].bool().view(1, R, 1),
                   dists=dists.t().reshape(1, R, N, 1),
                   weights=comp["weights"].t().reshape(1, R, N, 1),
                   gradients=grads.permute(1, 0, 2).reshape(1, R, N, 3),
                   hessians=None if hess is None else hess.permute(1, 0, 2).reshape(1, R, N, 3),
                   opacity=None, gradient=None)
        if self.stage == "a":
            for k in ("o_r", "o_s", "o_re"):
                out.pop(k)
        if not self.training:
            out["opacity"] = comp["opacity"][None]
            out["gradient"] = comp["gradient"][None]
            out["depth"] = comp["depth"][None]
            if "visibility" in comp:
                for k in ("visibility", "normal_x_light", "pseudo_shading", "inter_dist", "inter_mask"):
                    out[k] = comp[k][None]
        return out

    @torch.no_grad()
    def inference(self, data, shard=True):
        return self._inference(data, shard, None)[0]

    @torch.no_grad()
    def inference_lights(self, data, pose_lights, shard=True):
        if not torch.is_tensor(pose_lights) or pose_lights.dim() != 3 or tuple(pose_lights.shape[1:]) != (3, 4):
            raise ValueError("inference_lights: pose_lights must be a [L,3,4] tensor, got %s" % (
                tuple(pose_lights.shape) if torch.is_tensor(pose_lights) else type(pose_lights).__name__,))
        if pose_lights.shape[0] == 0:
            raise ValueError("inference_lights: pose_lights holds no light (L == 0)")
        return self._inference(data, shard, pose_lights)

    def _inference(self, data, shard, pose_lights):
        from . import shard as sh
        self.eval()
        self.prepare()
        H, W = self.image_size_val
        n_pix = H * W
        self.image_width = W
        world, rank, group = 1, 0, None
        if shard:
            import torch.distributed as dist
            if dist.is_available() and dist.is_initialized() and dist.get_world_size() > 1:
                world, rank = dist.get_world_size(), dist.get_rank()
        lo, hi, _ = sh.shard_range(n_pix, rank, world)
        N = self.pcfg.n_samples
        vis = self.pcfg.light_visibility is not None
        step = 256 // math.gcd(N, 256)
        dev = self.flat.device
        n_lights = 1 if pose_lights is None else pose_lights.shape[0]
        if pose_lights is not None:
            pose_lights = pose_lights.to(dev, torch.float32).contiguous()
        parts = []
        main = torch.cuda.current_stream(dev)
        if self._streams is None or self._streams[0].device != dev:
            self._streams = [torch.cuda.Stream(device=dev) for _ in range(2)]
        for s in self._streams:
            s.wait_stream(main)
        try:
            for i, start in enumerate(range(lo, hi, self.rand_rays_val)):
                R = min(self.rand_rays_val, hi - start)
                Rp = -(-R // step) * step
                lane = i % 2 if self.pipeline_chunks else 0
                with torch.cuda.stream(self._streams[lane]), self.engine.lane(lane):
                    ridx = torch.arange(start, start + Rp, device=dev).clamp_(max=start + R - 1)[None]
                    if pose_lights is None:
                        d = dict(pose=data["pose"], intr=data["intr"], pose_light=data["pose_light"], ray_idx=ridx)
                        st = self.engine.render(d, self.s_var.detach(), self.progress, False, u=None, W=W)
                        parts.append(sh.pack(st[4], vis)[:R])
                    else:
                        d = dict(pose=data["pose"], intr=data["intr"], ray_idx=ridx)
                        comps = self.engine.render_lights(d, pose_lights, self.s_var.detach(), self.progress, W)[3]
                        parts.append(sh.pack_lights(comps, vis)[:R])
        finally:
            for s in self._streams:
                main.wait_stream(s)
        for p in parts:
            p.record_stream(main)
        local = torch.cat(parts, 0) if parts else torch.zeros(0, n_lights * sh.n_channels(vis), device=dev)
        packed = sh.gather_tiles(local, n_pix, world, group) if world > 1 else local
        rot = data["pose"][..., :3, :3]

        def full(x):
            return x.unflatten(1, (H, W)).moveaxis(-1, 1)
        outs = []
        for unpacked in sh.unpack_lights(packed, n_lights, vis):
            out = {k: v.contiguous()[None] for k, v in unpacked.items()}
            normal_cam = -out["gradient"] @ rot.transpose(-1, -2)
            out.update(rgb_map=full(out["rgb"]), opacity_map=full(out["opacity"]), depth_map=full(out["depth"]),
                       normal_map=full(normal_cam))
            for k in ("o_r", "o_s", "o_re"):
                out[k + "_map"] = full(out[k])
            if vis:
                for k in ("visibility", "normal_x_light", "pseudo_shading", "inter_dist", "inter_mask"):
                    out[k + "_map"] = full(out[k]).float()
                out["visibility"] = out["visibility"] > 0.5
                out["inter_mask"] = out["inter_mask"] > 0.5
            outs.append(out)
        return outs
```

Before: 2.370 million rays/s.

## Skip zero-weight tiles in RGB head forward/backward via padded weighted-tile list

Adds a compacted list of tiles with nonzero compositing weight, padded to a multiple of 8 with dead tiles, and uses it to drive the PQ RGB-head forward and backward kernels instead of the full live-tile list. q4 partials are stored per weighted tile, and dw4 sums them over each ray's tile range. The point is to avoid MLP head work on tiles whose weights are all zero, at the cost of extra indirection, gathered mask loads, and an explicit zeroing of y for skipped tiles. It is enabled by default through a new switch.

```diff
diff --git a/include/mli_hip.h b/include/mli_hip.h
--- a/include/mli_hip.h
+++ b/include/mli_hip.h
@@ -139,6 +139,8 @@
   float* q4;
   const int32_t* tile_list;
   const int32_t* n_live_tiles;
+  const int32_t* wtile_list;
+  const int32_t* n_wtiles_pad;
 } mli_rgb_fwd_args;
 #define MLI_Q4_SCALE 65536.0f
 #define MLI_Q4_SEGS(N) ((256 % (N)) == 0 ? 256 / (N) : ((N) % 256 == 0 ? 1 : 256 / (N) + 2))
@@ -180,6 +182,8 @@
   int skip_dz3;
   const int32_t* tile_list;
   const int32_t* n_live_tiles;
+  const int32_t* wtile_list;
+  const int32_t* n_wtiles_pad;
 } mli_rgb_bwd_args;
 int mli_rgb_bwd(const mli_rgb_bwd_args* a, mli_stream_t s);
 int mli_rgb_bwd_workspace(const mli_rgb_bwd_args* a, int64_t* bytes);
@@ -233,6 +237,7 @@
   int k_out[3];
   float* workspace;
   const int32_t* tile_rank;
+  const int32_t* wtile_rank;
 } mli_dw4_args;
 int mli_dw4(const mli_dw4_args* a, mli_stream_t s);
 int mli_dw4_workspace(const mli_dw4_args* a, int64_t* bytes);
@@ -255,6 +260,7 @@
   int32_t* wtile_list; int32_t* wtile_rank;
   int32_t* ticket;
   int scan_launch;
+  int32_t* n_wtiles_pad;
 };
 typedef struct mli_live_tiles_args_s mli_live_tiles_args;
 int mli_live_tiles(const mli_live_tiles_args* a, mli_stream_t s);
diff --git a/mli_nerf_amd/_lib.py b/mli_nerf_amd/_lib.py
--- a/mli_nerf_amd/_lib.py
+++ b/mli_nerf_amd/_lib.py
@@ -55,7 +55,7 @@
     _fields_ = [("R", I32), ("N", I32), ("center", P), ("ray_unit", P), ("pts_light", P),
                 ("dists", P), ("grad", P), ("h0", P), ("wfwd", P), ("y", P), ("feat_frag", P),
                 ("xT", P), ("masks", P), ("n_heads", I32), ("weights", P), ("q4", P),
-                ("tile_list", P), ("n_live_tiles", P)]
+                ("tile_list", P), ("n_live_tiles", P), ("wtile_list", P), ("n_wtiles_pad", P)]
 
 
 class CompositeArgs(C.Structure):
@@ -73,7 +73,8 @@
 
 class RgbBwdArgs(C.Structure):
     _fields_ = [("R", I32), ("N", I32), ("dz4", P), ("wbwd", P), ("masks", P), ("dzT", P),
-                ("dz4T", P), ("skip_dz3", I32), ("tile_list", P), ("n_live_tiles", P)]
+                ("dz4T", P), ("skip_dz3", I32), ("tile_list", P), ("n_live_tiles", P),
+                ("wtile_list", P), ("n_wtiles_pad", P)]
 
 
 class WgradJob(C.Structure):
@@ -99,7 +100,7 @@
 class Dw4Args(C.Structure):
     _fields_ = [("R", I32), ("N", I32), ("n_heads", I32), ("q4", P), ("dray", P), ("scale", F32),
                 ("dw", P * 3), ("db", P * 3), ("k_out", I32 * 3), ("workspace", P),
-                ("tile_rank", P)]
+                ("tile_rank", P), ("wtile_rank", P)]
 
 
 class LiveRaysArgs(C.Structure):
@@ -109,7 +110,8 @@
 
 class LiveTilesArgs(C.Structure):
     _fields_ = [("comp", CompositeArgs), ("y", P), ("flags", P), ("tile_list", P), ("tile_rank", P),
-                ("n_live_tiles", P), ("wtile_list", P), ("wtile_rank", P), ("ticket", P), ("scan_launch", I32)]
+                ("n_live_tiles", P), ("wtile_list", P), ("wtile_rank", P), ("ticket", P), ("scan_launch", I32),
+                ("n_wtiles_pad", P)]
 
 
 Q4_SCALE = 65536.0
diff --git a/mli_nerf_amd/csrc/mlp_bwd.hip b/mli_nerf_amd/csrc/mlp_bwd.hip
--- a/mli_nerf_amd/csrc/mlp_bwd.hip
+++ b/mli_nerf_amd/csrc/mlp_bwd.hip
@@ -5,7 +5,7 @@
 template <bool NODZ3>
 __global__ __launch_bounds__(GBwd::THREADS) void rgb_bwd_kernel(mli_rgb_bwd_args a) {
   extern __shared__ __attribute__((aligned(16))) uint8_t lds[];
-  if (a.n_live_tiles && (int)(blockIdx.x * GBwd::NW) >= *a.n_live_tiles) return;
+  if (a.n_live_tiles && (int)(blockIdx.x * GBwd::NW) >= *(a.wtile_list ? a.n_wtiles_pad : a.n_live_tiles)) return;
   if (__builtin_amdgcn_readfirstlane(threadIdx.x >> 6) >= GBwd::NW / 2) rgb_bwd_body<GBwd, STORE, NODZ3>(a, lds);
   else rgb_bwd_body<GBwd, DMA, NODZ3>(a, lds);
 }
@@ -18,6 +18,8 @@
   if (S % 256 != 0) return (int)hipErrorInvalidValue;
   if ((a->tile_list != nullptr) != (a->n_live_tiles != nullptr)) return (int)hipErrorInvalidValue;
   if (a->tile_list && (a->N <= 0 || 256 % a->N != 0 || a->N % 32 != 0)) return (int)hipErrorInvalidValue;
+  if ((a->wtile_list != nullptr) != (a->n_wtiles_pad != nullptr)) return (int)hipErrorInvalidValue;
+  if (a->wtile_list && !a->tile_list) return (int)hipErrorInvalidValue;
   if (a->skip_dz3)
     hipLaunchKernelGGL(rgb_bwd_kernel<true>, dim3(S / GBwd::SAMPLES), dim3(GBwd::THREADS), GBwd::LDS_BWD,
                        (hipStream_t)s, *a);
diff --git a/mli_nerf_amd/csrc/mlp_core.h b/mli_nerf_amd/csrc/mlp_core.h
--- a/mli_nerf_amd/csrc/mlp_core.h
+++ b/mli_nerf_amd/csrc/mlp_core.h
@@ -338,7 +338,12 @@
     const int nthr = ROLE == STORE ? G::THREADS / 2 : G::THREADS;
     const int tid = ROLE == STORE ? threadIdx.x - G::THREADS / 2 : threadIdx.x;
     f32x4* qb = reinterpret_cast<f32x4*>(a.q4);
-    for (int it = tid; it < nseg * 257; it += nthr) {
+    for (int it = tid; it < (a.wtile_list ? G::NW * 257 : 0); it += nthr) {
+      const int w = it / 257, row = it - w * 257;
+      gstore_nt(qb + ((size_t)(t0 + w) * a.n_heads + hd) * 257 + row,
+                *reinterpret_cast<const f32x4*>(q4_park(w) + row * 16));
+    }
+    for (int it = tid; it < (a.wtile_list ? 0 : nseg * 257); it += nthr) {
       const int seg = it / 257, row = it - seg * 257;
       size_t item = (size_t)blockIdx.x * segs + seg;
       if (a.tile_list) item = (size_t)(a.tile_list[t0 + seg * (N / 32)] * 32 / N);
@@ -353,6 +358,12 @@
   block_sync();
 }
 
+template <class G>
+MLI_FI int heads_tile(const int32_t* list, int w) {
+  const int j = blockIdx.x * G::NW + w;
+  return list ? __builtin_amdgcn_readfirstlane(list[j]) : j;
+}
+
 MLI_FI int fwd_bytes(int c) { return (c >= 8 && (c - 8) % 33 < 8) ? CH(19) : CH(16); }
 
 template <class G, bool TRAIN, bool PQ, int ROLE>
@@ -360,7 +371,7 @@
   const int lane = threadIdx.x & 63, wave = threadIdx.x >> 6;
   const int c = lane & 31, h = lane >> 5;
   const int S = a.R * a.N;
-  const int tile = blockIdx.x * G::NW + wave;
+  const int tile = heads_tile<G>(PQ ? a.wtile_list : nullptr, wave);
   const int tile_o = (PQ && a.tile_list) ? __builtin_amdgcn_readfirstlane(a.tile_list[tile]) : tile;
   const int m = tile_o * 32 + c;
   const int r = m / a.N, k = m - r * a.N;
@@ -370,6 +381,7 @@
   constexpr int FKS = PQ ? G::FEAT_KS : (!TRAIN ? G::FEAT_KS_EVAL : 0);
   constexpr int FOFF = PQ ? G::LDS_FWD_PQ : G::LDS_FWD;
   const float wgt = PQ ? a.weights[slot] : 0.f;
+  const bool pad = PQ && a.wtile_list && __ballot((__builtin_bit_cast(uint32_t, wgt) & 0x7fffffffu) != 0) == 0;
 
   Ring rg;
   ring_start(rg, a.wfwd, 8 + a.n_heads * 33, bytes);
@@ -520,7 +532,7 @@
         for (int i = 0; i < 3; ++i)
           if (i < no) {
             const float y = sigmoidf_acc(acc[i]);
-            gstore_f32(a.y + 8 * slot + off + i, y);
+            gstore_f32(a.y + 8 * slot + off + i, pad ? 0.f : y);
             if (PQ) gq[i] = Q4_SCALE * wgt * (y * (1.0f - y));
           }
       }
@@ -542,7 +554,7 @@
 __global__ __launch_bounds__(GFwd::THREADS) void rgb_fwd_kernel(mli_rgb_fwd_args a) {
   extern __shared__ __attribute__((aligned(16))) uint8_t lds[];
   typedef typename std::conditional<TRAIN, GFwdT, GFwd>::type G;
-  if (PQ && a.n_live_tiles && (int)(blockIdx.x * G::NW) >= *a.n_live_tiles) return;
+  if (PQ && a.n_live_tiles && (int)(blockIdx.x * G::NW) >= *(a.wtile_list ? a.n_wtiles_pad : a.n_live_tiles)) return;
   if (__builtin_amdgcn_readfirstlane(threadIdx.x >> 6) >= G::NW / 2) rgb_fwd_body<G, TRAIN, PQ, STORE>(a, lds);
   else rgb_fwd_body<G, TRAIN, PQ, DMA>(a, lds);
 }
@@ -556,21 +568,23 @@
   const int c = lane & 31, h = lane >> 5;
   const int S = a.R * a.N;
   const int tiles = S / 32;
-  const int tile = blockIdx.x * G::NW + wave;
+  const int tile = heads_tile<G>(a.wtile_list, wave);
   const int tile_o = a.tile_list ? __builtin_amdgcn_readfirstlane(a.tile_list[tile]) : tile;
   const int m = tile_o * 32 + c;
   const int r = m / a.N, k = m - r * a.N;
   const size_t slot = (size_t)k * a.R + r;
   auto bytes = [](int cc) MLI_LAMBDA_FI { return bwd_bytes(cc); };
   constexpr int MASK_OPS = ROLE == DMA ? 2 : ROLE == ALL ? 1 : 0;
+  int mtile[MASK_OPS > 0 ? MASK_OPS : 1];
+#pragma unroll
+  for (int u = 0; u < MASK_OPS; ++u) mtile[u] = heads_tile<G>(a.wtile_list, u * G::ND + wave);
   auto mask_dma = [&](int L) MLI_LAMBDA_FI {
     const int Lc = min(L, 11);
     const int hd = Lc >> 2, ml = 3 - (Lc & 3);
-    const uint8_t* src = reinterpret_cast<const uint8_t*>(a.masks) +
-                         (((size_t)(hd * 4 + ml) * tiles + (size_t)blockIdx.x * G::NW) * 64) * 16;
 #pragma unroll
     for (int u = 0; u < MASK_OPS; ++u)
-      glds16(src + u * (G::MASKB / 2) + threadIdx.x * 16,
+      glds16(reinterpret_cast<const uint8_t*>(a.masks) +
+                 (((size_t)(hd * 4 + ml) * tiles + (size_t)mtile[u]) * 64 + lane) * 16,
              lds + G::MASK_OFF + (L & 1) * G::MASKB + u * (G::MASKB / 2) + wave * 1024);
   };
 
diff --git a/mli_nerf_amd/csrc/mlp_fwd.hip b/mli_nerf_amd/csrc/mlp_fwd.hip
--- a/mli_nerf_amd/csrc/mlp_fwd.hip
+++ b/mli_nerf_amd/csrc/mlp_fwd.hip
@@ -11,6 +11,8 @@
   if (!pq && a->q4 != nullptr) return (int)hipErrorInvalidValue;
   if ((a->tile_list != nullptr) != (a->n_live_tiles != nullptr)) return (int)hipErrorInvalidValue;
   if (a->tile_list && (!pq || 256 % a->N != 0)) return (int)hipErrorInvalidValue;
+  if ((a->wtile_list != nullptr) != (a->n_wtiles_pad != nullptr)) return (int)hipErrorInvalidValue;
+  if (a->wtile_list && !a->tile_list) return (int)hipErrorInvalidValue;
   const dim3 grid(S / GFwd::SAMPLES), block(GFwd::THREADS);
   if (pq) return mli_launch_rgb_fwd_pq(a, (hipStream_t)s);
   if (train) return mli_launch_rgb_fwd_train(a, (hipStream_t)s);
@@ -29,6 +31,6 @@
   bytes[2] = 0;
   bytes[3] = (int64_t)a->n_heads * (pq ? 3 : 4) * 256 * S * 2;
   bytes[4] = (int64_t)a->n_heads * 4 * (S / 32) * 64 * 16;
-  bytes[5] = pq ? (S / 256) * MLI_Q4_SEGS(a->N) * a->n_heads * 257 * 4 * 4 : 0;
+  bytes[5] = pq ? (a->wtile_list ? S / 32 : (S / 256) * MLI_Q4_SEGS(a->N)) * a->n_heads * 257 * 4 * 4 : 0;
   return 0;
 }
diff --git a/mli_nerf_amd/csrc/rays.hip b/mli_nerf_amd/csrc/rays.hip
--- a/mli_nerf_amd/csrc/rays.hip
+++ b/mli_nerf_amd/csrc/rays.hip
@@ -936,7 +936,12 @@
           a.tile_list[pos * T + i] = r * T + i;
           a.tile_rank[r * T + i] = before * T + (f != 0 ? i : 0);
           a.wtile_rank[pos * T + i] = f != 0 ? below : W;
-          if ((f >> i) & 1u) a.wtile_list[below] = pos * T + i;
+          if ((f >> i) & 1u) {
+            a.wtile_list[below] = pos * T + i;
+          } else if (a.n_wtiles_pad != nullptr) {
+            const int z = pos * T + i - (f != 0 ? below : W);
+            if (z < ((8 - (W & 7)) & 7)) a.wtile_list[W + z] = pos * T + i;
+          }
         }
       },
       L, W);
@@ -944,6 +949,7 @@
     a.tile_rank[R * T] = L * T;
     a.wtile_rank[R * T] = W;
     a.n_live_tiles[0] = (L + G - 1) / G * G * T;
+    if (a.n_wtiles_pad != nullptr) a.n_wtiles_pad[0] = (W + 7) & ~7;
   }
 }
 
@@ -967,12 +973,12 @@
     for (int j = 0; j < L * CE / 32; ++j)
       if (j * 32 < N && ((seg >> (j * (32 / CE))) & ((1u << (32 / CE)) - 1u)) != 0) f |= 1u << j;
     if (sub == 0) a.flags[r] = (int)f;
-    if (f == 0 && a.y != nullptr) {
+    if (a.y != nullptr && (f == 0 || a.n_wtiles_pad != nullptr)) {
       const f32x4 z = {0.f, 0.f, 0.f, 0.f};
 #pragma unroll
       for (int e = 0; e < CE; ++e) {
         const int k = CE * sub + e;
-        if (k < N) {
+        if (k < N && ((f >> (k >> 5)) & 1u) == 0) {
           f32x4* row = reinterpret_cast<f32x4*>(a.y + ((size_t)k * R + r) * 8);
           row[0] = z;
           row[1] = z;
diff --git a/mli_nerf_amd/csrc/wgrad.hip b/mli_nerf_amd/csrc/wgrad.hip
--- a/mli_nerf_amd/csrc/wgrad.hip
+++ b/mli_nerf_amd/csrc/wgrad.hip
@@ -698,14 +698,32 @@
       if (a.tile_rank != nullptr && a.tile_rank[(r0 + sg + 1) * (N / 32)] == a.tile_rank[(r0 + sg) * (N / 32)]) continue;
       const float* d = a.dray + 8 * (r0 + sg);
       const f32x4* q = reinterpret_cast<const f32x4*>(a.q4) + ((size_t)g * segs + sg) * nh * 257;
+      int i0 = 0, i1 = 0;
+      if (a.wtile_rank != nullptr) {
+        const int p0 = a.tile_rank[(r0 + sg) * (N / 32)];
+        i0 = a.wtile_rank[p0];
+        i1 = a.wtile_rank[p0 + N / 32];
+        q = reinterpret_cast<const f32x4*>(a.q4);
+      }
 #pragma unroll
       for (int h = 0; h < 3; ++h) {
         if (h >= nh) break;
         f32x4 dv;
 #pragma unroll
         for (int c = 0; c < 4; ++c) dv[c] = c < a.k_out[h] ? d[3 * h + c] : 0.f;
-        acc[h] += dv * __builtin_nontemporal_load(q + h * 257 + f);
-        if (f == 0) accb[h] += dv * __builtin_nontemporal_load(q + h * 257 + 256);
+        if (a.wtile_rank == nullptr) {
+          acc[h] += dv * __builtin_nontemporal_load(q + h * 257 + f);
+          if (f == 0) accb[h] += dv * __builtin_nontemporal_load(q + h * 257 + 256);
+          continue;
+        }
+        f32x4 v = {0.f, 0.f, 0.f, 0.f}, vb = {0.f, 0.f, 0.f, 0.f};
+        for (int i = i0; i < i1; ++i) {
+          const f32x4* qi = q + ((size_t)i * nh + h) * 257;
+          v += __builtin_nontemporal_load(qi + f);
+          if (f == 0) vb += __builtin_nontemporal_load(qi + 256);
+        }
+        acc[h] += dv * v;
+        if (f == 0) accb[h] += dv * vb;
       }
     }
   }
@@ -932,6 +950,7 @@
 extern "C" int mli_dw4(const mli_dw4_args* a, mli_stream_t s) {
   if (!dw4_valid(a) || !a->q4 || !a->dray || !a->workspace) return (int)hipErrorInvalidValue;
   if (a->tile_rank && 256 % a->N != 0) return (int)hipErrorInvalidValue;
+  if (a->wtile_rank && !a->tile_rank) return (int)hipErrorInvalidValue;
   for (int h = 0; h < a->n_heads; ++h)
     if (!a->dw[h] || !a->db[h]) return (int)hipErrorInvalidValue;
   const int slices = dw4_slices(a);
diff --git a/mli_nerf_amd/engine.py b/mli_nerf_amd/engine.py
--- a/mli_nerf_amd/engine.py
+++ b/mli_nerf_amd/engine.py
@@ -102,6 +102,9 @@
     ("skip_zero_tiles", "MLI_SKIP_ZERO_TILES", True, bool),
     ("elide_outside", "MLI_ELIDE_OUTSIDE", True, bool),
     ("elide_outside_sampling", "MLI_ELIDE_OUTSIDE_SAMPLING", True, bool),
+)
+MORE_SWITCHES = (
+    ("skip_zero_tiles_heads", "MLI_SKIP_ZERO_TILES_HEADS", True, bool),
 )
 
 
@@ -155,7 +158,7 @@
         self._pack_descs = None
         self.trace = None
         self.deterministic = False
-        for name, env, default, kind in SWITCHES:
+        for name, env, default, kind in SWITCHES + MORE_SWITCHES:
             v = os.environ.get(env)
             setattr(self, name, default if v is None else int(v) if kind is int else v != "0")
         self.pq = True
@@ -367,7 +370,7 @@
             y.zero_()
             self._y_zeroed = y.data_ptr()
         feat = self._buf("feat", (S * layout.K0,), torch.float16)
-        xT = masks = w = tl = tr = nl = wl = wr = None
+        xT = masks = w = tl = tr = nl = wl = wr = npad = None
         pq = s_var is not None and self.pq_mode(N, training)
         if training and self.stage == "b" and not self.deterministic:
             self._zero_once(self._buf("dw", (_dw_numel(self._dw_sizes()),)))
@@ -375,18 +378,20 @@
             xT = self._buf("xT", (nh, 3 if pq else 4, S * 256), torch.float16)
             masks = self._buf("masks", (nh, 4, S // 32, 64, 4), torch.int32)
         if pq and elide and self.elides(N, training):
-            w, tl, tr, nl, wl, wr = self._live_lists(rays, dists, fld, y, s_var, progress)
+            w, tl, tr, nl, wl, wr, npad = self._live_lists(rays, dists, fld, y, s_var, progress)
         else:
             self.densify((rays, dists, fld))
             if pq:
                 w = self.weights(rays, dists, fld, s_var, progress)
-        q4 = self._buf("q4", (S // 256, layout.q4_segs(N), nh, 257, 4)) if pq else None
+        q4 = None if not pq else (self._buf("q4", (S // 256, layout.q4_segs(N), nh, 257, 4)) if npad is None
+                                  else self._buf("q4", (S // 32, nh, 257, 4)))
         L.call("mli_rgb_fwd", L.RgbFwdArgs(R, N, L.ptr(rays["center"]), L.ptr(rays["ray_unit"]),
                                            L.ptr(rays["pts_light"]), L.ptr(dists), L.ptr(fld["grad"]),
                                            L.ptr(fld["h0"]), L.ptr(self.wfwd), L.ptr(y), L.ptr(feat),
-                                           L.ptr(xT), L.ptr(masks), nh, L.ptr(w), L.ptr(q4), L.ptr(tl), L.ptr(nl)))
+                                           L.ptr(xT), L.ptr(masks), nh, L.ptr(w), L.ptr(q4), L.ptr(tl), L.ptr(nl),
+                                           L.ptr(wl if npad is not None else None), L.ptr(npad)))
         return dict(y=y, x0T=feat if training else None, xT=xT, masks=masks, feat=feat, q4=q4,
-                    tile_list=tl, tile_rank=tr, n_live_tiles=nl, wtile_list=wl, wtile_rank=wr)
+                    tile_list=tl, tile_rank=tr, n_live_tiles=nl, wtile_list=wl, wtile_rank=wr, n_wtiles_pad=npad)
 
     def _live_lists(self, rays, dists, fld, y, s_var, progress):
         N, R = dists.shape
@@ -399,7 +404,7 @@
             w = self.weights(rays, dists, fld, s_var, progress)
             L.call("mli_live_rays", L.LiveRaysArgs(R, N, L.ptr(w), L.ptr(y), L.ptr(flags), L.ptr(tl), L.ptr(tr),
                                                    L.ptr(nl)))
-            return w, tl, tr, nl, None, None
+            return w, tl, tr, nl, None, None, None
         out = self._composite_out(dists, outputs=False)
         w, comp = out["weights"], self._composite_args(rays, dists, fld, dict(y=None), s_var, progress, out)
         wl = self._buf("wtile_list", (T,), torch.int32)
@@ -407,10 +412,13 @@
         step = self._lane.step
         if "live_ticket" not in step:
             step["live_ticket"] = torch.zeros(1, dtype=torch.int32, device=self.device)
+        npad = None
+        if self.skip_zero_tiles and self.skip_zero_tiles_heads:
+            npad = self._buf("n_wtiles_pad", (1,), torch.int32)
         L.call("mli_live_tiles", L.LiveTilesArgs(comp, L.ptr(y), L.ptr(flags), L.ptr(tl), L.ptr(tr), L.ptr(nl),
                                                  L.ptr(wl), L.ptr(wr), L.ptr(step["live_ticket"]),
-                                                 0 if self.live_tiles_pass == 2 else 1))
-        return (w, tl, tr, nl, wl, wr) if self.skip_zero_tiles else (w, tl, tr, nl, None, None)
+                                                 0 if self.live_tiles_pass == 2 else 1, L.ptr(npad)))
+        return (w, tl, tr, nl, wl, wr, npad) if self.skip_zero_tiles else (w, tl, tr, nl, None, None, None)
 
     def _composite_out(self, dists, outputs=True, extras=False):
         N, R = dists.shape
@@ -672,7 +680,9 @@
         dzT = self._buf("dzT", (3, 4, S * 256), torch.float16)
         L.call("mli_rgb_bwd", L.RgbBwdArgs(R, N, L.ptr(dz4), L.ptr(self.wbwd), L.ptr(hd["masks"]), L.ptr(dzT),
                                            L.ptr(dz4T), 1 if rebuild else 0, L.ptr(hd.get("tile_list")),
-                                           L.ptr(hd.get("n_live_tiles"))))
+                                           L.ptr(hd.get("n_live_tiles")),
+                                           L.ptr(hd.get("wtile_list") if hd.get("n_wtiles_pad") is not None else None),
+                                           L.ptr(hd.get("n_wtiles_pad"))))
         jobs, ad, (dw4, db4, k4) = self._wgrad_plan(dzT, dz4T, hd, dwbuf, flat, grad_out, S,
                                                     (dz4, R, N) if rebuild else None)
         if self.gate_wgrad:
@@ -712,7 +722,8 @@
     def _dw4(self, R, N, hd, scale, dw4, db4, k4):
         args = L.Dw4Args(R, N, 3, L.ptr(hd["q4"]), L.ptr(self._lane.step["dray"]), scale / L.Q4_SCALE,
                          (C.c_void_p * 3)(*dw4), (C.c_void_p * 3)(*db4), (C.c_int * 3)(*k4), None,
-                         L.ptr(hd.get("tile_rank")))
+                         L.ptr(hd.get("tile_rank")),
+                         L.ptr(hd.get("wtile_rank") if hd.get("n_wtiles_pad") is not None else None))
         args.workspace = L.ptr(self._buf("dw4_ws", (L.workspace("mli_dw4", args)[0] // 4,)))
         L.call("mli_dw4", args)
 
diff --git a/mli_nerf_amd/model.py b/mli_nerf_amd/model.py
--- a/mli_nerf_amd/model.py
+++ b/mli_nerf_amd/model.py
@@ -5,7 +5,7 @@
 import torch.nn.functional as F
 
 from . import layout
-from .engine import SWITCHES, PathConfig, RenderEngine
+from .engine import MORE_SWITCHES, SWITCHES, PathConfig, RenderEngine
 from .hashgrid import GRID_DEFAULTS, level_table
 
 
@@ -210,7 +210,7 @@
         self.image_width = self.image_size_train[1]
         self.deterministic = False
         self.pq = True
-        for name, _, _, _ in SWITCHES:
+        for name, _, _, _ in SWITCHES + MORE_SWITCHES:
             setattr(self, name, None)
 
     def _view(self, name, flat=None):
@@ -314,7 +314,7 @@
         eng = self.engine
         eng.deterministic = self.deterministic
         eng.pq = self.pq
-        for name, _, _, _ in SWITCHES:
+        for name, _, _, _ in SWITCHES + MORE_SWITCHES:
             if getattr(self, name) is not None:
                 setattr(eng, name, getattr(self, name))
         eng.set_normal_eps(sdf.normal_eps)
```

After: 2.495 million rays/s (median of 6 runs). 5.3% higher.
